# microsoft/OmniParser

Measured on AMD Instinct MI355X. Metric: screenshots/sec end-to-end (detect+caption) @1920x1080, higher is better.
Workload: dtype f32 (split-f16x3 MFMA)

## Files before the change

omniparser_amd/csrc/capi.hip:

```cpp
#include "omni_internal.h"

#include <math.h>
#include <stdarg.h>
#include <stdlib.h>
#include <string.h>
#include <vector>

static thread_local char g_err[512] = "";

void omni_set_error(const char* fmt, ...) {
  va_list ap;
  va_start(ap, fmt);
  vsnprintf(g_err, sizeof(g_err), fmt, ap);
  va_end(ap);
}

extern "C" const char* omni_last_error(void) { return g_err; }
extern "C" int omni_abi_version(void) { return OMNI_ABI_VERSION; }

static omni_ovf_reader_t g_ovf_readers[8];
static int g_ovf_n = 0;
void omni_register_overflow_reader(omni_ovf_reader_t fn) {
  if (g_ovf_n < 8) g_ovf_readers[g_ovf_n++] = fn;
}
extern "C" int omni_overflow_count(int reset, unsigned long long* count) {
  OMNI_REQUIRE(count != nullptr, "omni_overflow_count: null result pointer");
  unsigned long long total = 0;
  for (int k = 0; k < g_ovf_n; ++k) {
    unsigned int v = 0;
    if (g_ovf_readers[k](&v, reset)) {
      omni_set_error("omni_overflow_count: reading the device counter failed");
      return OMNI_E_HIP;
    }
    total += v;
  }
  *count = total;
  return OMNI_OK;
}

extern "C" int omni_device_count(void) {
  int n = 0;
  hipError_t e = hipGetDeviceCount(&n);
  if (e != hipSuccess) {
    omni_set_error("hipGetDeviceCount: %s", hipGetErrorString(e));
    return OMNI_E_NODEV;
  }
  return n;
}

static int dispatch(const omni_op_t* op, hipStream_t s) {
  switch (op->kind) {
    case OMNI_OP_CONV: return op->i[20] == 2 ? omni_launch_gemm_dma(op, s) : omni_launch_conv(op, s);
    case OMNI_OP_SPLIT_CONVERT: return omni_launch_split_convert(op, s);
    case OMNI_OP_MLP_FUSED: return omni_launch_mlp_fused(op, s);
    case OMNI_OP_GLUE: return omni_launch_glue(op, s);
    case OMNI_OP_OVERLAY: return omni_launch_overlay(op, s);
    case OMNI_OP_PNG_PACK: return omni_launch_png_pack(op, s);
    case OMNI_OP_PNG_DEFLATE: return omni_launch_png_deflate(op, s);
    case OMNI_OP_AVGPOOL2: return omni_launch_avgpool2(op, s);
    case OMNI_OP_MAXPOOL: return omni_launch_maxpool(op, s);
    case OMNI_OP_RESIZE_NEAREST: return omni_launch_resize_nearest(op, s);
    case OMNI_OP_LETTERBOX: return omni_launch_letterbox(op, s);
    case OMNI_OP_DETECT_DECODE: return omni_launch_detect_decode(op, s);
    case OMNI_OP_NMS: return omni_launch_nms(op, s);
    case OMNI_OP_DWCONV3: return omni_launch_dwconv3(op, s);
    case OMNI_OP_LAYERNORM: return omni_launch_layernorm(op, s);
    case OMNI_OP_DWCONV3_LN: return omni_launch_dwconv3_ln(op, s);
    case OMNI_OP_ATTN_ROWS: case OMNI_OP_CHAN_ATTN: case OMNI_OP_ATTN_DECODE: return omni_launch_attention(op, s);
    case OMNI_OP_PROJ_PREP: case OMNI_OP_ASSEMBLE: case OMNI_OP_EMBED_STEP: case OMNI_OP_GREEDY_STEP:
    case OMNI_OP_BEAM_STEP: case OMNI_OP_GREEDY_CTRL_STEP: case OMNI_OP_CROP_RESIZE: return omni_launch_misc(op, s);
    case OMNI_OP_GREEDY_VOCAB_STEP: return omni_launch_vocab_step(op, s);
    case OMNI_OP_VISUAL_MATCH: return omni_launch_visual_match(op, s);
    case OMNI_OP_REGION_OCR: return omni_launch_region_ocr(op, s);
    default:
      omni_set_error("unknown op kind %d", op->kind);
      return OMNI_E_ARG;
  }
}

static bool check_ptrs_enabled() {
  const char* e = getenv("OMNI_CHECK_PTRS");
  if (e && e[0] == '0') return false;
  static const int ndev = [] { int n = 0; const bool ok = hipGetDeviceCount(&n) == hipSuccess; if (!ok) (void)hipGetLastError(); return ok ? n : 0; }();
  return ndev > 0;
}

static void op_extents(const omni_op_t* op, long long ext[8]) {
  for (int k = 0; k < 8; ++k) ext[k] = 1;
  const long long esz = op->dtype == OMNI_F32 ? 4 : 2;
  const int* i = op->i;
  auto span = [&](long long rows, long long ld, long long coff, long long c) { return rows > 0 ? ((rows - 1) * ld + coff + c) * esz : 1; };
  switch (op->kind) {
    case OMNI_OP_CONV: {
      const long long B = i[0], H = i[1], W = i[2], Cin = i[3], Cout = i[12], M = B * i[10] * i[11], K = (long long)i[6] * i[7] * Cin;
      ext[0] = span(B * H * W, i[4], i[5], i[25] ? i[4] : Cin);
      ext[1] = Cout * K * (i[20] ? 4 : esz);
      ext[2] = Cout * 4;
      ext[3] = span(M, i[16], i[17], Cout);
      ext[4] = span(M, i[13], i[14], Cout);
      ext[5] = i[19] > 0 ? (long long)i[19] * 1024 : 1;
      if (i[24] > 0) ext[6] = (long long)i[24] * 4;
      if (i[20] == 2 && i[26] > 0) {
        const long long nimg = (M + i[26] - 1) / i[26];
        ext[1] += (nimg - 1) * (long long)i[27];
        ext[6] = nimg * 4;
      }
      if (i[20] == 2 && i[28] == 1) {
        ext[7] = (M / 256) * (Cout / 64) * 4096;
        ext[4] = 1;
      }
      break;
    }
    case OMNI_OP_CHAN_ATTN: {
      const long long B = i[0], N = i[1], C = i[3], G = i[4], ct = i[10] > 0 ? i[10] : (i[5] > 0 ? i[5] : 1);
      ext[0] = B * N * 3 * C * esz; ext[4] = B * N * C * esz; ext[5] = B * G * ((N + ct - 1) / ct) * 1024 * 4;
      if (i[8] == 1) { ext[1] = C * C * 4; ext[2] = ext[3] = B * C * C * 4; ext[6] = B * 4; ext[7] = B * (C / 64) * G * 4; }
      break;
    }
    case OMNI_OP_BEAM_STEP: {
      const long long rows = (long long)i[0] * i[6], T = i[3];
      ext[0] = rows > 0 ? ((rows - 1) * i[2] + i[1]) * esz : 1;
      ext[1] = (long long)i[1] * 4;
      ext[2] = ext[4] = ext[5] = rows * T * 4;
      ext[3] = rows * 4;
      ext[7] = (long long)i[0] * (3LL * i[6] + 2) * 4;
      break;
    }
    case OMNI_OP_GREEDY_STEP:
      if (op->p[5] || op->p[7]) {
        const long long rows = i[0], T = i[3];
        ext[0] = rows > 0 ? ((rows - 1) * i[2] + i[1]) * esz : 1;
        ext[1] = (long long)i[1] * 4;
        ext[2] = ext[4] = ext[7] = rows * T * 4;
        ext[5] = rows * 4;
        ext[6] = 4;
      }
      break;
    case OMNI_OP_GREEDY_CTRL_STEP: {
      const long long rows = i[0], T = i[3];
      ext[0] = rows > 0 ? ((rows - 1) * i[2] + i[1]) * esz : 1;
      ext[1] = (long long)i[1] * 4;
      ext[2] = ext[4] = rows * T * 4;
      ext[3] = rows * 4;
      ext[6] = 4;
      ext[7] = i[12];
      break;
    }
    case OMNI_OP_GREEDY_VOCAB_STEP: {
      const long long rows = i[0], T = i[3];
      ext[0] = rows > 0 ? ((rows - 1) * i[2] + i[1]) * esz : 1;
      ext[1] = (long long)i[1] * 4;
      ext[2] = ext[4] = rows * T * 4;
      ext[3] = ext[5] = rows * 4;
      ext[6] = 4;
      ext[7] = i[12];
      break;
    }
    case OMNI_OP_VISUAL_MATCH: {
      const long long D = i[3];
      if (i[0] == 0) {
        ext[0] = i[1] > 0 ? (((long long)i[1] - 1) * i[2] + D) * esz : 1; ext[4] = (long long)i[1] * D * 4; ext[5] = (long long)i[1] * 4;
      } else if (const long long part = omni_visual_match_part_bytes(op)) {
        ext[5] = part;
        if (i[0] == 1) { ext[0] = (long long)i[1] * D * 4; ext[1] = (long long)i[2] * D * 4; }
        else { ext[4] = ext[6] = (long long)i[1] * i[4] * 4; }
      }
      break;
    }
    case OMNI_OP_REGION_OCR:
      if (i[0] == 0) {
        if (i[1] > 0 && i[2] > 0 && i[3] > 0 && i[4] > 0 && i[13] > 0) {
          ext[0] = (long long)i[2] * i[3] * 3; ext[1] = (long long)i[1] * 8; ext[4] = (long long)i[1] * i[4] * i[4] * i[13] * esz; ext[7] = 1024;
        }
      } else if (i[0] == 1) {
        omni_region_ocr_extents(op, ext);
      }
      break;
    case OMNI_OP_MLP_FUSED: {
      const long long rows = (long long)i[0] * i[1], C = i[3], hid = i[12];
      ext[0] = span(rows, i[4], i[5], C); ext[1] = hid * C * 4; ext[2] = hid * 4; ext[3] = span(rows, i[16], i[17], C);
      ext[4] = span(rows, i[13], i[14], C); ext[5] = hid * C * 4; ext[6] = C * 4;
      break;
    }
    case OMNI_OP_SPLIT_CONVERT: {
      const long long rows = (long long)i[0] * i[1];
      ext[0] = span(rows, i[4], i[5], i[3]); ext[4] = span(rows, i[13], i[14], i[3]);
      break;
    }
    case OMNI_OP_AVGPOOL2: case OMNI_OP_MAXPOOL: case OMNI_OP_RESIZE_NEAREST: {
      const long long B = i[0], Ho = op->kind == OMNI_OP_AVGPOOL2 ? i[1] - 1 : i[10], Wo = op->kind == OMNI_OP_AVGPOOL2 ? i[2] - 1 : i[11];
      ext[0] = span(B * i[1] * i[2], i[4], i[5], i[3]); ext[4] = span(B * Ho * Wo, i[13], i[14], i[3]);
      if (op->kind == OMNI_OP_RESIZE_NEAREST && i[17] > 1) {
        static const int pidx[4] = {1, 2, 3, 5};
        static const int base[4][4] = {{19, 20, 21, 22}, {23, 24, 25, 26}, {27, 28, 29, 30}, {7, 12, 15, 16}};
        for (int k = 0; k + 1 < i[17] && k < 4; ++k)
          ext[pidx[k]] = span(B * i[base[k][0]] * i[base[k][1]], i[base[k][2]], i[base[k][3]], i[3]);
      }
      break;
    }
    case OMNI_OP_NMS: {
      const long long cap = i[0], md = i[1], fr = i[4] > 0 ? i[4] : 1;
      ext[0] = fr * cap * 32; ext[1] = fr * 4; ext[2] = fr * (cap + 1) * 32; ext[3] = cap * ((cap + 63) / 64) * 8;
      ext[4] = fr * md * 16; ext[5] = fr * md * 4; ext[6] = fr * md * 4; ext[7] = fr * 4;
      break;
    }
    case OMNI_OP_DETECT_DECODE: {
      for (int l = 0; l < 3; ++l) {
        const long long hw = (long long)(i[1] / (8 << l)) * (i[2] / (8 << l));
        ext[l] = span(hw, i[3 + l], i[13 + l], i[0]);
        ext[3 + l] = span(hw, i[6 + l], i[16 + l], i[12] ? 4 : 64);
      }
      ext[6] = (long long)i[9] * 32; ext[7] = 4;
      break;
    }
    case OMNI_OP_LAYERNORM: {
      const long long rows = (long long)i[0] * i[1], C = i[3];
      ext[0] = rows * C * esz; ext[1] = (long long)(i[5] > 0 ? i[5] : 1) * C * esz; ext[2] = C * 4; ext[3] = C * 4;
      ext[4] = rows * C * esz; ext[5] = rows * C * esz;
      break;
    }
    case OMNI_OP_DWCONV3: case OMNI_OP_DWCONV3_LN: {
      const long long n = (long long)i[0] * i[1] * i[2] * i[3] * esz, C = i[3];
      ext[0] = n; ext[1] = 9 * C * esz; ext[2] = C * 4; ext[4] = n;
      if (op->kind == OMNI_OP_DWCONV3_LN) { ext[3] = n; ext[5] = C * 4; ext[6] = C * 4; }
      break;
    }
    case OMNI_OP_ASSEMBLE: {
      const long long B = i[0], n_img = i[1], n_txt = i[2], C = i[3];
      ext[0] = B * n_img * C * esz; ext[1] = n_txt * C * esz; ext[2] = B * n_txt * 4; ext[3] = (long long)i[4] * C * esz;
      ext[4] = B * (n_img + n_txt) * C * esz;
      break;
    }
    case OMNI_OP_ATTN_ROWS:
      ext[7] = (long long)i[11] * 4;
      break;
    case OMNI_OP_ATTN_DECODE:
      ext[7] = i[7] > 0 ? (long long)((i[10] + (i[12] > 1 ? i[12] : 1) - 1) / (i[12] > 1 ? i[12] : 1)) * 4 : (long long)i[10] * i[8] * 4;
      break;
    case OMNI_OP_OVERLAY:
      if (op->p[3] || op->p[4] || i[3]) {
        const long long B = i[3] > 0 ? i[3] : 1;
        ext[0] = B * i[0] * i[1] * 3; ext[1] = (long long)i[2] * 32; ext[3] = B * 8; ext[4] = (B + 1) * 4;
      }
      break;
    case OMNI_OP_PNG_DEFLATE:
      if (i[5] == 2 && i[6] > 0 && i[0] > 0 && i[1] > 0) {
        const long long B = i[6], U = (long long)i[0] * (3LL * i[1] + 1), units = (U + 32767) / 32768;
        ext[0] = B * i[0] * i[1] * 3; ext[1] = B * i[2]; ext[2] = B * U; ext[3] = B * units * 33792; ext[4] = B * i[3] * 4;
        ext[5] = B * i[4] * 4; ext[6] = B * 4 * (((long long)i[2] + 2) / 3); ext[7] = B * units * 32768 * 4;
      }
      break;
    default: break;
  }
  for (int k = 0; k < 8; ++k) if (ext[k] < 1) ext[k] = 1;
}

static int check_op_ptrs(const omni_op_t* op, int index) {
  long long ext[8];
  op_extents(op, ext);
  for (int k = 0; k < 8; ++k) {
    const void* ptr = op->p[k];
    if (!ptr) continue;
    hipDeviceptr_t base = nullptr;
    size_t size = 0;
    hipError_t e = hipMemGetAddressRange(&base, &size, (hipDeviceptr_t)ptr);
    if (e != hipSuccess || !base) {
      (void)hipGetLastError();
      omni_set_error("op %d (kind %d): p[%d] = %p is not inside any device allocation (%s)", index, op->kind, k, ptr,
                     e != hipSuccess ? hipGetErrorString(e) : "no base");
      return OMNI_E_ARG;
    }
    const long long off = (const char*)ptr - (const char*)base;
    if (off < 0 || off + ext[k] > (long long)size) {
      omni_set_error("op %d (kind %d): p[%d] = %p + %lld bytes runs past its allocation [%p, +%zu)", index, op->kind, k, ptr, ext[k],
                     (void*)base, size);
      return OMNI_E_ARG;
    }
  }
  return OMNI_OK;
}

static int check_ctrl_block(const omni_op_t* op, int index) {
  if (op->kind != OMNI_OP_GREEDY_CTRL_STEP) return OMNI_OK;
  const long long bytes = op->i[12], nw = ((long long)op->i[1] + 31) >> 5, fixed = OMNI_GEN_CTRL_HEADER_BYTES + 8 * nw;
  if (!op->p[7] || op->i[1] <= 0 || bytes < fixed) {
    omni_set_error("op %d (greedy_ctrl_step): a control block of %lld bytes (i12) at p7 = %p cannot hold the header and two bitmaps over a "
                   "vocabulary of %d (%lld bytes)", index, bytes, op->p[7], op->i[1], fixed);
    return OMNI_E_ARG;
  }
  omni_gen_ctrl_t h;
  hipError_t e = hipMemcpy(&h, op->p[7], sizeof h, hipMemcpyDeviceToHost);
  if (e != hipSuccess) {
    (void)hipGetLastError();
    omni_set_error("op %d (greedy_ctrl_step): the header of the control block p7 = %p cannot be read (%s)", index, op->p[7], hipGetErrorString(e));
    return OMNI_E_ARG;
  }
  if (h.n_bad < 0 || h.n_bad > OMNI_GEN_CTRL_MAX_BAD || (h.n_bad > 0 && (h.bad_stride < 3 || h.bad_stride > OMNI_GEN_CTRL_MAX_BAD_LEN + 1))) {
    omni_set_error("op %d (greedy_ctrl_step): the control block claims %d bad-word sequences of stride %d (at most %d of 2..%d tokens)", index,
                   h.n_bad, h.bad_stride, OMNI_GEN_CTRL_MAX_BAD, OMNI_GEN_CTRL_MAX_BAD_LEN);
    return OMNI_E_ARG;
  }
  const long long need = fixed + 4LL * h.n_bad * h.bad_stride;
  if (bytes < need) {
    omni_set_error("op %d (greedy_ctrl_step): the control block's header claims %d bad-word sequences of stride %d = %lld bytes, i12 says %lld",
                   index, h.n_bad, h.bad_stride, need, bytes);
    return OMNI_E_ARG;
  }
  return OMNI_OK;
}

static int check_trie_block(const omni_op_t* op, int index) {
  if (op->kind != OMNI_OP_GREEDY_VOCAB_STEP) return OMNI_OK;
  const long long bytes = op->i[12];
  if (!op->p[7] || bytes < OMNI_VOCAB_HEADER_BYTES + 4) {
    omni_set_error("op %d (greedy_vocab_step): a trie block of %lld bytes (i12) at p7 = %p cannot hold the header and one node (%d bytes)",
                   index, bytes, op->p[7], OMNI_VOCAB_HEADER_BYTES + 4);
    return OMNI_E_ARG;
  }
  omni_vocab_trie_t h;
  hipError_t e = hipMemcpy(&h, op->p[7], sizeof h, hipMemcpyDeviceToHost);
  if (e != hipSuccess) {
    (void)hipGetLastError();
    omni_set_error("op %d (greedy_vocab_step): the header of the trie block p7 = %p cannot be read (%s)", index, op->p[7], hipGetErrorString(e));
    return OMNI_E_ARG;
  }
  if (h.n_nodes < 1 || h.n_nodes > OMNI_VOCAB_MAX_NODES || h.n_edges < 0 || h.n_edges >= h.n_nodes) {
    omni_set_error("op %d (greedy_vocab_step): the trie block claims %d nodes and %d edges (1..%d nodes, fewer edges than nodes)", index,
                   h.n_nodes, h.n_edges, OMNI_VOCAB_MAX_NODES);
    return OMNI_E_ARG;
  }
  const long long need = OMNI_VOCAB_HEADER_BYTES + 4LL * (h.n_nodes + 1 + 2LL * h.n_edges);
  if (bytes < need) {
    omni_set_error("op %d (greedy_vocab_step): the trie block's header claims %d nodes and %d edges = %lld bytes, i12 says %lld",
                   index, h.n_nodes, h.n_edges, need, bytes);
    return OMNI_E_ARG;
  }
  return OMNI_OK;
}

// ... 184 lines not shown
```

omniparser_amd/csrc/caption_ops.hip:

```cpp
#include "omni_internal.h"
#include <stdlib.h>

#pragma clang fp contract(off)

OMNI_RANGE_GUARD_TU()

namespace {

template <typename T> __device__ __forceinline__ float ldf(const T* p) { return ElemTraits<T>::to_f32(*p); }
template <typename T> __device__ __forceinline__ void stf(T* p, float v) { *p = ElemTraits<T>::from_f32(v); }

__device__ __forceinline__ float wave_sum(float v) {
#pragma unroll
  for (int o = 32; o > 0; o >>= 1) v += __shfl_xor(v, o);
  return v;
}
__device__ __forceinline__ float wave_max(float v) {
#pragma unroll
  for (int o = 32; o > 0; o >>= 1) v = fmaxf(v, __shfl_xor(v, o));
  return v;
}

struct DwArgs { const void* x; const void* w; const float* bias; void* y; int B, H, W, C; long long total; };

// ... 1335 lines not shown
}

__global__ __launch_bounds__(256) void chan_scores_mfma_kernel(ChanArgs a) {
  __shared__ float red[4][1024];
  const int chunk = blockIdx.x, g = blockIdx.y, b = blockIdx.z;
  const int lane = threadIdx.x & 63, wave = threadIdx.x >> 6;
  const int n0c = chunk * a.chunk_tokens;
  const int n1 = n0c + a.chunk_tokens < a.N ? n0c + a.chunk_tokens : a.N;
  const int per = a.chunk_tokens / 4;
  const int nw0 = n0c + wave * per, nw1 = min(nw0 + per, n1);
  const float* __restrict__ base = (const float*)a.qkv + (long long)b * a.N * 3 * a.C + g * 32 + (lane & 31);
  const long long ld = 3ll * a.C;
  f32x16 acc;
#pragma unroll
  for (int e = 0; e < 16; ++e) acc[e] = 0.0f;
  const int tsel = lane >> 5;
  int n = nw0;
  for (; n + 32 <= nw1; n += 32) {
    const float* r = base + (long long)(n + tsel) * ld;
    float qv[16], kv[16];
#pragma unroll
    for (int u = 0; u < 16; ++u) { qv[u] = r[2 * u * ld]; kv[u] = r[2 * u * ld + a.C]; }
#pragma unroll
    for (int u = 0; u < 16; ++u) acc = __builtin_amdgcn_mfma_f32_32x32x2f32(qv[u], kv[u], acc, 0, 0, 0);
  }
  for (; n < nw1; n += 2) {
    const int tok = n + tsel;
    const bool ok = tok < nw1;
    const float* r = base + (long long)(ok ? tok : nw0) * ld;
    const float qv = ok ? r[0] : 0.0f, kv = ok ? r[a.C] : 0.0f;
    acc = __builtin_amdgcn_mfma_f32_32x32x2f32(qv, kv, acc, 0, 0, 0);
  }
#pragma unroll
  for (int e = 0; e < 16; ++e) red[wave][((e & 3) + 8 * (e >> 2) + 4 * (lane >> 5)) * 32 + (lane & 31)] = acc[e];
  __syncthreads();
  float* out = a.ws + (((long long)b * a.G + g) * a.chunks + chunk) * 1024;
  for (int e = threadIdx.x; e < 1024; e += 256) out[e] = ((red[0][e] + red[1][e]) + red[2][e]) + red[3][e];
}

__global__ __launch_bounds__(256) void chan_softmax_kernel(ChanArgs a) {
  __shared__ float sa[32][33];
  const int g = blockIdx.x, b = blockIdx.y;
  float* p0 = a.ws + ((long long)b * a.G + g) * a.chunks * 1024;
  const int i = threadIdx.x >> 3, j0 = (threadIdx.x & 7) * 4;
  {
    const float* p = p0 + i * 32 + j0;
    float s[4] = {0.f, 0.f, 0.f, 0.f};
    int c = 0;
    for (; c + 8 <= a.chunks; c += 8) {
      f32x4 v[8];
#pragma unroll
      for (int u = 0; u < 8; ++u) v[u] = *reinterpret_cast<const f32x4*>(p + (long long)(c + u) * 1024);
#pragma unroll
      for (int u = 0; u < 8; ++u)
#pragma unroll
        for (int e = 0; e < 4; ++e) s[e] += v[u][e];
    }
    for (; c < a.chunks; ++c) {
      const f32x4 v = *reinterpret_cast<const f32x4*>(p + (long long)c * 1024);
#pragma unroll
      for (int e = 0; e < 4; ++e) s[e] += v[e];
    }
#pragma unroll
    for (int e = 0; e < 4; ++e) sa[i][j0 + e] = s[e] * a.scale;
  }
  __syncthreads();
  if (threadIdx.x < 32) {
    const int r = threadIdx.x;
    float mx = -INFINITY;
    for (int j = 0; j < 32; ++j) mx = fmaxf(mx, sa[r][j]);
    float sum = 0.f;
    for (int j = 0; j < 32; ++j) { float e = expf(sa[r][j] - mx); sa[r][j] = e; sum += e; }
    const float inv = 1.0f / sum;
    for (int j = 0; j < 32; ++j) sa[r][j] *= inv;
  }
  __syncthreads();
#pragma unroll
  for (int e = 0; e < 4; ++e) p0[i * 32 + j0 + e] = sa[i][j0 + e];
}

__global__ __launch_bounds__(256, 2) void chan_apply_mfma_split_kernel(ChanArgs a) {
  const int g = blockIdx.y, b = blockIdx.z;
  const int lane = threadIdx.x & 63, wave = threadIdx.x >> 6;
  const int col = lane & 31, kg = lane >> 5;
  const float inv2048 = 1.0f / 2048.0f;
  const int n00 = blockIdx.x * 256 + wave * 64;
  if (n00 >= a.N) return;
  const float* V = (const float*)a.qkv + (long long)b * a.N * 3 * a.C + 2 * a.C + g * 32 + kg * 8;
  f32x4 vraw[2][4];
#pragma unroll
  for (int t = 0; t < 2; ++t) {
    const int nl = min(n00 + t * 32 + col, a.N - 1);
    const float* vp = V + (long long)nl * 3 * a.C;
#pragma unroll
    for (int ks = 0; ks < 2; ++ks) {
      vraw[t][2 * ks] = *reinterpret_cast<const f32x4*>(vp + 16 * ks);
      vraw[t][2 * ks + 1] = *reinterpret_cast<const f32x4*>(vp + 16 * ks + 4);
    }
  }
  const float* A = a.ws + ((long long)b * a.G + g) * a.chunks * 1024 + col * 32 + kg * 8;
  h16x8 Ah[2], Al[2];
#pragma unroll
  for (int ks = 0; ks < 2; ++ks) {
    uint2 h0, l0, h1, l1;
    split4m(*reinterpret_cast<const f32x4*>(A + 16 * ks), h0, l0);
    split4m(*reinterpret_cast<const f32x4*>(A + 16 * ks + 4), h1, l1);
    Ah[ks] = __builtin_bit_cast(h16x8, u32x4{h0.x, h0.y, h1.x, h1.y});
    Al[ks] = __builtin_bit_cast(h16x8, u32x4{l0.x, l0.y, l1.x, l1.y});
  }
  float* const O = (float*)a.o + (long long)b * a.N * a.C + g * 32 + 4 * kg;
  unsigned char* const S = (unsigned char*)a.o + (long long)b * a.N * a.C * 4;
#pragma unroll
  for (int t = 0; t < 2; ++t) {
    const int n = n00 + t * 32 + col;
    if (n00 + t * 32 >= a.N) break;
    f32x16 accM, accC;
#pragma unroll
    for (int e = 0; e < 16; ++e) { accM[e] = 0.f; accC[e] = 0.f; }
#pragma unroll
    for (int ks = 0; ks < 2; ++ks) {
      uint2 h0, l0, h1, l1;
      split4m(vraw[t][2 * ks], h0, l0);
      split4m(vraw[t][2 * ks + 1], h1, l1);
      const h16x8 vh = __builtin_bit_cast(h16x8, u32x4{h0.x, h0.y, h1.x, h1.y});
      const h16x8 vl = __builtin_bit_cast(h16x8, u32x4{l0.x, l0.y, l1.x, l1.y});
      accM = __builtin_amdgcn_mfma_f32_32x32x16_f16(Ah[ks], vh, accM, 0, 0, 0);
      accC = __builtin_amdgcn_mfma_f32_32x32x16_f16(Ah[ks], vl, accC, 0, 0, 0);
      accC = __builtin_amdgcn_mfma_f32_32x32x16_f16(Al[ks], vh, accC, 0, 0, 0);
    }
    if (n < a.N) {
#pragma unroll
      for (int q = 0; q < 4; ++q) {
        const f32x4 o = f32x4{accC[4 * q], accC[4 * q + 1], accC[4 * q + 2], accC[4 * q + 3]} * inv2048 +
                        f32x4{accM[4 * q], accM[4 * q + 1], accM[4 * q + 2], accM[4 * q + 3]};
        if (a.osplit) {
          const float v[4] = {o[0], o[1], o[2], o[3]};
          uint2 hi, lo;
          omni_split4(v, hi, lo);
          unsigned char* p = S + (long long)n * a.C * 4 + omni_split_off(g * 32 + 8 * q + 4 * kg);
          *reinterpret_cast<uint2*>(p) = hi;
          *reinterpret_cast<uint2*>(p + 32) = lo;
        } else {
          *reinterpret_cast<f32x4*>(O + (long long)n * a.C + 8 * q) = o;
        }
      }
    }
  }
}


struct FoldArgs {
  const float* ws; const float* wp; float* wf; float* bmax; unsigned char* wb; float* osc;
  int C, G, chunks, nblk;
};

__global__ __launch_bounds__(256) void chan_fold_kernel(FoldArgs a) {
  __shared__ float sA[32][32];
  __shared__ float sW[64][33];
  __shared__ float smax[4];
  const int ob = blockIdx.x, g = blockIdx.y, b = blockIdx.z, tid = threadIdx.x;
  const float* A = a.ws + ((long long)b * a.G + g) * a.chunks * 1024;
  for (int e = tid; e < 1024; e += 256) sA[e >> 5][e & 31] = A[e];
  for (int e = tid; e < 64 * 32; e += 256) sW[e >> 5][e & 31] = a.wp[(long long)(ob * 64 + (e >> 5)) * a.C + g * 32 + (e & 31)];
  __syncthreads();
  const int r = tid >> 2, j0 = (tid & 3) * 8;
  float acc[8];
#pragma unroll
  for (int e = 0; e < 8; ++e) acc[e] = 0.0f;
#pragma unroll 8
  for (int i = 0; i < 32; ++i) {
    const float w = sW[r][i];
#pragma unroll
    for (int e = 0; e < 8; ++e) acc[e] = fmaf(w, sA[i][j0 + e], acc[e]);
  }
  float* out = a.wf + ((long long)b * a.C + ob * 64 + r) * a.C + g * 32 + j0;
  *reinterpret_cast<f32x4*>(out) = f32x4{acc[0], acc[1], acc[2], acc[3]};
  *reinterpret_cast<f32x4*>(out + 4) = f32x4{acc[4], acc[5], acc[6], acc[7]};
  float m = 0.0f;
#pragma unroll
  for (int e = 0; e < 8; ++e) m = fmaxf(m, fabsf(acc[e]));
#pragma unroll
  for (int o = 32; o >= 1; o >>= 1) m = fmaxf(m, __shfl_xor(m, o));
  if ((tid & 63) == 0) smax[tid >> 6] = m;
  __syncthreads();
  if (tid == 0) a.bmax[(long long)b * a.nblk + ob * a.G + g] = fmaxf(fmaxf(smax[0], smax[1]), fmaxf(smax[2], smax[3]));
}

__global__ __launch_bounds__(256) void chan_fold_pack_kernel(FoldArgs a) {
  __shared__ float red[256];
  const int b = blockIdx.y, tid = threadIdx.x;
  float m = 0.0f;
  for (int e = tid; e < a.nblk; e += 256) m = fmaxf(m, a.bmax[(long long)b * a.nblk + e]);
  red[tid] = m;
  __syncthreads();
  for (int o = 128; o >= 1; o >>= 1) {
    if (tid < o) red[tid] = fmaxf(red[tid], red[tid + o]);
    __syncthreads();
  }
  const float amax = red[0];
  int k = 0;
  if (amax > 0.0f) {
    k = 12 - ((int)((__builtin_bit_cast(unsigned, amax) >> 23) & 0xffu) - 127);
    k = max(-24, min(24, k));
  }
  const float up = __builtin_bit_cast(float, (unsigned)(127 + k) << 23);
  if (blockIdx.x == 0 && tid == 0) a.osc[b] = __builtin_bit_cast(float, (unsigned)(127 - k) << 23);
  const int gpr = a.C / 16;
  const int idx = blockIdx.x * 256 + tid;
  if (idx >= a.C * gpr) return;
  const float* src = a.wf + (long long)b * a.C * a.C + (long long)idx * 16;
  half_t h[32];
#pragma unroll
  for (int q = 0; q < 4; ++q) {
    const f32x4 v = *reinterpret_cast<const f32x4*>(src + 4 * q) * up;
#pragma unroll
    for (int e = 0; e < 4; ++e) {
      const half_t hi = (half_t)v[e];
      h[4 * q + e] = hi;
      h[16 + 4 * q + e] = (half_t)(v[e] - (float)hi);
    }
  }
  unsigned char* dst = a.wb + ((long long)b * a.C * a.C + (long long)idx * 16) * 4;
#pragma unroll
  for (int q = 0; q < 4; ++q) {
    f16x8 o;
#pragma unroll
    for (int e = 0; e < 8; ++e) o[e] = h[8 * q + e];
    *reinterpret_cast<f16x8*>(dst + 16 * q) = o;
  }
}


struct PrepArgs { const void* x; const float* pos; const float* temporal; void* y; int B, N, C; };

template <typename T>
__global__ __launch_bounds__(256) void proj_prep_kernel(PrepArgs a) {
  int c = blockIdx.x * 256 + threadIdx.x, b = blockIdx.y;
  if (c >= a.C) return;
  const T* x = (const T*)a.x + (long long)b * a.N * a.C + c;
  T* y = (T*)a.y + (long long)b * (a.N + 1) * a.C + c;
  float s = 0.f;
  for (int n = 0; n < a.N; ++n) {
    float v = (ldf(x + (long long)n * a.C) + a.pos[(long long)n * a.C + c]) + a.temporal[c];
    s += v;
    stf(y + (long long)(n + 1) * a.C, v);
  }
  stf(y, s / (float)a.N);
}

struct AsmArgs {
  const void* img; const void* txt; void* y; int B, n_img, n_txt, C;
  const void* table; const int* ids; int vocab; float scale;
};

template <typename T>
__global__ __launch_bounds__(256) void assemble_kernel(AsmArgs a) {
  long long total = (long long)a.B * (a.n_img + a.n_txt) * a.C;
  long long idx = (long long)blockIdx.x * 256 + threadIdx.x;
  if (idx >= total) return;
  int c = (int)(idx % a.C);
  long long r = idx / a.C;
  int t = (int)(r % (a.n_img + a.n_txt));
  long long b = r / (a.n_img + a.n_txt);
  if (a.ids && t >= a.n_img) {
    const int tok = min(max(a.ids[b * a.n_txt + (t - a.n_img)], 0), a.vocab - 1);
    float v = ldf((const T*)a.table + (long long)tok * a.C + c);
    if (a.scale != 1.0f) v *= a.scale;
    stf((T*)a.y + idx, v);
    return;
  }
  const T* src = t < a.n_img ? (const T*)a.img + (b * a.n_img + t) * a.C + c : (const T*)a.txt + (long long)(t - a.n_img) * a.C + c;
  ((T*)a.y)[idx] = *src;
}

struct EmbArgs { const void* table; const void* pos; const int* ids; const int* step; void* y; int B, C, T, pos_offset; float scale; };

template <typename T>
__global__ __launch_bounds__(256) void embed_step_kernel(EmbArgs a) {
  int c = blockIdx.x * 256 + threadIdx.x, b = blockIdx.y;
  if (c >= a.C) return;
  int st = *a.step;
  int tok = a.ids[b * a.T + st];
  float v = ldf((const T*)a.table + (long long)tok * a.C + c);
  if (a.scale != 1.0f) v *= a.scale;
  v += ldf((const T*)a.pos + (long long)(st + a.pos_offset) * a.C + c);
  stf((T*)a.y + (long long)b * a.C + c, v);
}

constexpr int ATTN_SELF_SPLIT_MIN_CAP = 64;
struct DecArgs {
  const void* q; const void* knew; const void* vnew; void* kc; void* vc; void* o; const int* step;
  int ldq, qoff, ldn, koff, voff, ldo;
  int heads, nk_fixed, cap, C, ldc;
  float scale;
  const int* nkeys;
};

__device__ __forceinline__ int decode_cross_keys(const DecArgs& a, int bkv) {
  return a.nkeys ? min(max(a.nkeys[bkv], 1), a.nk_fixed) : a.nk_fixed;
}

template <typename T, bool BEAM>
__device__ __forceinline__ void attn_decode_body(DecArgs a, const int* table, int kv_div) {
  OMNI_DYN_LDS(float, sp);
  const int h = blockIdx.x, b = blockIdx.y, lane = threadIdx.x;
  const int C = a.ldc;
  int nk;
  const int bkv = BEAM && a.nk_fixed > 0 ? b / kv_div : b;
  T* Kc = (T*)a.kc + (long long)bkv * a.cap * C + h * 64;
  T* Vc = (T*)a.vc + (long long)bkv * a.cap * C + h * 64;
  const int* trow = BEAM && a.nk_fixed <= 0 ? table + (long long)b * a.cap : nullptr;
  auto krow = [&](int k) -> long long {
    if constexpr (BEAM) {
      if (trow) return ((long long)(trow[k] - b) * a.cap + k) * C;
    }
    return (long long)k * C;
  };
  if (a.nk_fixed > 0) {
    nk = decode_cross_keys(a, bkv);
  } else {
    int st = *a.step;
    nk = st + 1;
    Kc[(long long)st * C + lane] = ((const T*)a.knew)[(long long)b * a.ldn + a.koff + h * 64 + lane];
    Vc[(long long)st * C + lane] = ((const T*)a.vnew)[(long long)b * a.ldn + a.voff + h * 64 + lane];
    __syncthreads();
  }
  float qd = ldf((const T*)a.q + (long long)b * a.ldq + a.qoff + h * 64 + lane);
  __shared__ float sq[64];
  sq[lane] = qd;
  __syncthreads();
  float mx = -INFINITY;
  for (int k = lane; k < nk; k += 64) {
    const T* kr = Kc + krow(k);
    float s = 0.f;
#pragma unroll 16
    for (int d = 0; d < 64; ++d) s += sq[d] * ldf(kr + d);
    s *= a.scale;
    sp[k] = s;
    mx = fmaxf(mx, s);
  }
  mx = wave_max(mx);
  float sum = 0.f;
  for (int k = lane; k < nk; k += 64) { float e = expf(sp[k] - mx); sp[k] = e; sum += e; }
  sum = wave_sum(sum);
  __syncthreads();
  float acc = 0.f;
  for (int k = 0; k < nk; ++k) acc += sp[k] * ldf(Vc + krow(k) + lane);
  stf((T*)a.o + (long long)b * a.ldo + h * 64 + lane, acc / sum);
}

template <typename T>
__global__ __launch_bounds__(64) void attn_decode_kernel(DecArgs a) { attn_decode_body<T, false>(a, nullptr, 1); }

template <typename T>
__global__ __launch_bounds__(64) void attn_decode_beam_kernel(DecArgs a, const int* table, int kv_div) {
  attn_decode_body<T, true>(a, table, kv_div);
}

template <bool BEAM>
// ... 800 lines not shown
      int kk = k[y]; s0 += s[0] * kk; s1 += s[1] * kk; s2 += s[2] * kk;
    }
    p[0] = clip8b(s0); p[1] = clip8b(s1); p[2] = clip8b(s2);
  }
  T* out = (T*)a.y + ((long long)crop * a.R * a.R + idx) * a.ldo;
#pragma unroll
  for (int c = 0; c < 3; ++c) {
    float v = a.lut[p[c]];
    stf(out + c, (v - a.mean[c]) / a.stdv[c]);
  }
  for (int c = 3; c < a.ldo; ++c) stf(out + c, 0.0f);
}

template <typename F32, typename F16>
int by_dtype(int dtype, const char* name, F32 f32, F16 f16) {
  if (dtype == OMNI_F32) f32();
  else if (dtype == OMNI_F16) f16();
  else { omni_set_error("%s: bad dtype %d", name, dtype); return OMNI_E_ARG; }
  return OMNI_OK;
}

template <typename L>
int by_dtype_scores(int dtype, bool scores, const char* name, L launch) {
  return scores ? by_dtype(dtype, name, [&] { launch(float{}, std::true_type{}); }, [&] { launch(half_t{}, std::true_type{}); })
                : by_dtype(dtype, name, [&] { launch(float{}, std::false_type{}); }, [&] { launch(half_t{}, std::false_type{}); });
}

}

int omni_launch_dwconv3(const omni_op_t* op, hipStream_t s) {
  DwArgs a{};
  a.x = op->p[0]; a.w = op->p[1]; a.bias = (const float*)op->p[2]; a.y = op->p[4];
  a.B = op->i[0]; a.H = op->i[1]; a.W = op->i[2]; a.C = op->i[3];
  OMNI_REQUIRE(a.x && a.w && a.bias && a.y && a.B > 0 && a.H > 0 && a.W > 0 && a.C > 0, "dwconv3: bad arguments");
  OMNI_REQUIRE(a.C % (op->dtype == OMNI_F32 ? 4 : 8) == 0, "dwconv3: C must be a multiple of the 16-byte vector width");
  a.total = (long long)a.B * a.H * a.W * a.C;
  const int V = op->dtype == OMNI_F32 ? 4 : 8;
  const DwStripGrid g = dwconv3_strip_grid(a, V);
  int rc;
  if (g.ok) {
    rc = by_dtype(op->dtype, "dwconv3",
        [&] { hipLaunchKernelGGL(dwconv3_strip_kernel<float>, dim3(g.gx, g.gy, g.gz), dim3(256), 0, s, a, g.cv_log2); },
        [&] { hipLaunchKernelGGL(dwconv3_strip_kernel<half_t>, dim3(g.gx, g.gy, g.gz), dim3(256), 0, s, a, g.cv_log2); });
  } else {
    long long blocks = (a.total / V + 255) / 256; if (blocks > 65536) blocks = 65536;
    rc = by_dtype(op->dtype, "dwconv3",
        [&] { hipLaunchKernelGGL(dwconv3_kernel<float>, dim3((unsigned)blocks), dim3(256), 0, s, a); },
        [&] { hipLaunchKernelGGL(dwconv3_kernel<half_t>, dim3((unsigned)blocks), dim3(256), 0, s, a); });
  }
  if (rc) return rc;
  OMNI_HIP_CHECK(hipGetLastError());
  return OMNI_OK;
}

int omni_launch_dwconv3_ln(const omni_op_t* op, hipStream_t s) {
  DwLnArgs a{};
  a.x = op->p[0]; a.w = op->p[1]; a.bias = (const float*)op->p[2]; a.h = op->p[3]; a.y1 = op->p[4];
  a.g = (const float*)op->p[5]; a.b = (const float*)op->p[6];
  a.B = op->i[0]; a.H = op->i[1]; a.W = op->i[2]; a.C = op->i[3]; a.eps = op->f[0]; a.osplit = op->i[6];
  const int V = op->dtype == OMNI_F32 ? 4 : 8;
  OMNI_REQUIRE(a.x && a.w && a.bias && a.h && a.y1 && a.g && a.b, "dwconv3_ln: null pointer");
  OMNI_REQUIRE(!a.osplit || (op->dtype == OMNI_F32 && a.C % 16 == 0), "dwconv3_ln: split output needs an f32 plan and C %% 16 == 0");
  OMNI_REQUIRE(a.B > 0 && a.H > 0 && a.W > 0 && a.C > 0 && a.C <= 1024 && a.C % V == 0, "dwconv3_ln: bad shape (C <= 1024, C %% %d == 0)", V);
  a.pixels = (long long)a.B * a.H * a.W;
  if (op->dtype == OMNI_F32 && (a.C == 128 || a.C == 256 || a.C == 512) && (long long)a.B * a.H * a.W < (1ll << 31)) {
    if (a.C == 128) launch_dwln_strip<1, 32>(a, s);
    else if (a.C == 256) launch_dwln_strip<1, 64>(a, s);
    else launch_dwln_strip<2, 64>(a, s);
    OMNI_HIP_CHECK(hipGetLastError());
    return OMNI_OK;
  }
  unsigned blocks = (unsigned)((a.pixels + 3) / 4);
  int rc = by_dtype(op->dtype, "dwconv3_ln",
      [&] { hipLaunchKernelGGL(dwconv3_ln_kernel<float>, dim3(blocks), dim3(256), 0, s, a); },
      [&] { hipLaunchKernelGGL(dwconv3_ln_kernel<half_t>, dim3(blocks), dim3(256), 0, s, a); });
  if (rc) return rc;
  OMNI_HIP_CHECK(hipGetLastError());
  return OMNI_OK;
}

int omni_launch_layernorm(const omni_op_t* op, hipStream_t s) {
  LnArgs a{};
  a.x = op->p[0]; a.add = op->p[1]; a.g = (const float*)op->p[2]; a.b = (const float*)op->p[3]; a.y = op->p[4];
  a.rows = ((long long)op->i[0]) * (op->i[1] > 0 ? op->i[1] : 1); a.C = op->i[3]; a.period = op->i[5] > 0 ? op->i[5] : 1;
  a.eps = op->f[0];
  a.omode = op->i[6]; a.y2 = op->p[5];
  OMNI_REQUIRE(a.x && a.g && a.b && a.y && a.rows > 0 && a.C > 0 && a.C <= 1024, "layernorm: bad arguments (C <= 1024)");
  OMNI_REQUIRE(a.omode >= 0 && a.omode <= 2 && (a.omode != 2 || a.y2), "layernorm: bad output mode %d", a.omode);
  OMNI_REQUIRE(a.omode == 0 || (op->dtype == OMNI_F32 && a.C % 16 == 0), "layernorm: split output needs an f32 plan and C %% 16 == 0");
  if (op->dtype == OMNI_F32 && launch_layernorm_v4(a, s)) {
    OMNI_HIP_CHECK(hipGetLastError());
    return OMNI_OK;
  }
  unsigned blocks = (unsigned)((a.rows + 3) / 4);
  int rc = by_dtype(op->dtype, "layernorm",
      [&] { launch_layernorm_typed<float>(a, blocks, s); },
      [&] { launch_layernorm_typed<half_t>(a, blocks, s); });
  if (rc) return rc;
  OMNI_HIP_CHECK(hipGetLastError());
  return OMNI_OK;
}

static int launch_attn_rows(const omni_op_t* op, hipStream_t s) {
  AttnArgs a{};
  a.q = op->p[0]; a.k = op->p[1]; a.v = op->p[2]; a.o = op->p[4];
  a.kbias = (const float*)op->p[5]; a.vbias = (const float*)op->p[6];
  a.ldq = op->i[0]; a.ldk = op->i[1]; a.ldv = op->i[2]; a.ldo = op->i[3];
  a.qoff = op->i[4]; a.koff = op->i[5]; a.voff = op->i[6]; a.ooff = op->i[7];
  a.heads = op->i[8]; a.nq = op->i[9]; a.nk = op->i[10]; a.groups = op->i[11];
  a.mode = op->i[12]; a.H = op->i[13]; a.W = op->i[14];
  int D = op->i[15];
  a.scale = op->f[0];
  a.osplit = op->i[16];
  a.nkeys = (const int*)op->p[7];
  OMNI_REQUIRE(a.q && a.k && a.v && a.o && a.heads > 0 && a.nq > 0 && a.nk > 0 && a.groups > 0, "attn_rows: bad arguments");
  OMNI_REQUIRE(!a.nkeys || a.mode == 0, "attn_rows: the per-group key count (p7) is for mode 0");
  OMNI_REQUIRE(!a.osplit || (op->dtype == OMNI_F32 && a.ldo % 16 == 0 && a.ooff % 16 == 0), "attn_rows: split output needs an f32 plan, 16-channel aligned");
  OMNI_REQUIRE(D == 32 || D == 64, "attn_rows: head_dim %d unsupported", D);
  if (a.mode == 1) {
    OMNI_REQUIRE(a.nq == 144 && a.nk == 144 && a.H > 0 && a.W > 0, "attn_rows: window mode needs 12x12 windows");
    a.wy = (a.H + 11) / 12; a.wx = (a.W + 11) / 12;
    OMNI_REQUIRE(a.groups % (a.wy * a.wx) == 0, "attn_rows: groups must be B * windows");
  } else { a.wy = a.wx = 0; }
  int rc;
  const bool aligned4 = a.ldq % 4 == 0 && a.ldk % 4 == 0 && a.ldv % 4 == 0 && a.ldo % 4 == 0 &&
                        a.qoff % 4 == 0 && a.koff % 4 == 0 && a.voff % 4 == 0 && a.ooff % 4 == 0;
  OMNI_REQUIRE(!a.osplit || (a.mode == 1 && D == 32) || (a.mode == 0 && D == 64), "attn_rows: split output exists on the MFMA kernels only");
  if (a.mode == 1 && D == 32) {
    dim3 grid(1, a.heads, a.groups);
    OMNI_REQUIRE(op->dtype != OMNI_F32 || aligned4, "attn_rows: the f32 window kernel reads 16-byte rows (pitches and channel offsets %% 4 == 0)");
    rc = by_dtype(op->dtype, "attn_rows",
      [&] { hipLaunchKernelGGL(window_attn_mfma_f32_kernel, grid, dim3(192), 0, s, a); },
      [&] { hipLaunchKernelGGL((window_attn_mfma_kernel<half_t>), grid, dim3(192), 0, s, a); });
  } else if (a.mode == 0 && D == 64) {
    dim3 grid((a.nq + 127) / 128, a.heads, a.groups);
    OMNI_REQUIRE(op->dtype != OMNI_F32 || aligned4, "attn_rows: the f32 MHA kernel reads 16-byte rows (pitches and channel offsets %% 4 == 0)");
    rc = by_dtype(op->dtype, "attn_rows",
      [&] { hipLaunchKernelGGL(mha_mfma_f32_kernel, grid, dim3(256), 0, s, a); },
      [&] { hipLaunchKernelGGL((mha_mfma_kernel<half_t>), grid, dim3(256), 0, s, a); });
  } else {
    dim3 grid((a.nq + 127) / 128, a.heads, a.groups);
    if (D == 32) rc = by_dtype(op->dtype, "attn_rows",
      [&] { hipLaunchKernelGGL((attn_rows_kernel<float, 32, 128>), grid, dim3(128), 0, s, a); },
      [&] { hipLaunchKernelGGL((attn_rows_kernel<half_t, 32, 128>), grid, dim3(128), 0, s, a); });
    else rc = by_dtype(op->dtype, "attn_rows",
      [&] { hipLaunchKernelGGL((attn_rows_kernel<float, 64, 128>), grid, dim3(128), 0, s, a); },
      [&] { hipLaunchKernelGGL((attn_rows_kernel<half_t, 64, 128>), grid, dim3(128), 0, s, a); });
  }
  if (rc) return rc;
  OMNI_HIP_CHECK(hipGetLastError());
  return OMNI_OK;
}

static int launch_chan_attn(const omni_op_t* op, hipStream_t s) {
  ChanArgs a{};
  a.qkv = op->p[0]; a.o = op->p[4]; a.ws = (float*)op->p[5];
  a.B = op->i[0]; a.N = op->i[1]; a.C = op->i[3]; a.G = op->i[4]; a.chunk_tokens = op->i[5]; a.osplit = op->i[6];
  const bool fold = op->i[8] == 1;
  OMNI_REQUIRE(a.qkv && (a.o || fold) && a.ws && a.B > 0 && a.N > 0 && a.C == a.G * 32 && a.chunk_tokens > 0, "chan_attn: bad arguments");
  OMNI_REQUIRE(op->i[8] == 0 || fold, "chan_attn: unknown mode %d", op->i[8]);
  OMNI_REQUIRE(!fold || (op->dtype == OMNI_F32 && a.chunk_tokens % 8 == 0 && a.C % 64 == 0 && op->p[1] && op->p[2] && op->p[3] && op->p[6] && op->p[7]),
               "chan_attn: fold mode needs an f32 plan, C %% 64 == 0, chunk_tokens %% 8 == 0 and p1 / p2 / p3 / p6 / p7");
  OMNI_REQUIRE(!a.osplit || op->dtype == OMNI_F32, "chan_attn: split output needs an f32 plan");
  const bool have_scores = op->i[9] == 1;
  if (op->i[10] != 0) {
    OMNI_REQUIRE(op->i[10] > 0 && op->i[10] % 8 == 0 && a.chunk_tokens % op->i[10] == 0 && op->dtype == OMNI_F32 && a.C % 4 == 0,
                 "chan_attn: i10 = %d (tokens per partial) needs an f32 plan, i10 %% 8 == 0 and i5 %% i10 == 0", op->i[10]);
    a.chunk_tokens = op->i[10];
  }
  OMNI_REQUIRE(op->i[9] == 0 || (have_scores && op->dtype == OMNI_F32 && a.chunk_tokens % 8 == 0 && a.C % 4 == 0),
               "chan_attn: i9 = %d (partials already in the workspace) needs an f32 plan and chunk_tokens %% 8 == 0", op->i[9]);
  a.chunks = (a.N + a.chunk_tokens - 1) / a.chunk_tokens;
  a.scale = 1.0f / sqrtf((float)a.N);
  if (op->f[0] != 0.0f) a.scale = op->f[0];
  dim3 g1(a.chunks, a.G, a.B), g2((a.N + 255) / 256, a.G, a.B);
  if (op->dtype == OMNI_F32 && a.chunk_tokens % 8 == 0 && a.C % 4 == 0) {
    if (!have_scores) hipLaunchKernelGGL(chan_scores_mfma_kernel, g1, dim3(256), 0, s, a);
    hipLaunchKernelGGL(chan_softmax_kernel, dim3(a.G, a.B), dim3(256), 0, s, a);
    if (fold) {
      FoldArgs f{};
      f.ws = a.ws; f.wp = (const float*)op->p[1]; f.wf = (float*)op->p[2]; f.wb = (unsigned char*)op->p[3]; f.osc = (float*)op->p[6];
      f.bmax = (float*)op->p[7];
      f.C = a.C; f.G = a.G; f.chunks = a.chunks; f.nblk = (a.C / 64) * a.G;
      hipLaunchKernelGGL(chan_fold_kernel, dim3(a.C / 64, a.G, a.B), dim3(256), 0, s, f);
      hipLaunchKernelGGL(chan_fold_pack_kernel, dim3((a.C * (a.C / 16) + 255) / 256, a.B), dim3(256), 0, s, f);
      OMNI_HIP_CHECK(hipGetLastError());
      return OMNI_OK;
    }
    hipLaunchKernelGGL(chan_apply_mfma_split_kernel, g2, dim3(256), 0, s, a);
    OMNI_HIP_CHECK(hipGetLastError());
    return OMNI_OK;
  }
  int rc = by_dtype(op->dtype, "chan_attn",
      [&] { hipLaunchKernelGGL(chan_scores_kernel<float>, g1, dim3(256), 0, s, a);
            hipLaunchKernelGGL(chan_apply_kernel<float>, g2, dim3(256), 0, s, a); },
      [&] { hipLaunchKernelGGL(chan_scores_kernel<half_t>, g1, dim3(256), 0, s, a);
            hipLaunchKernelGGL(chan_apply_kernel<half_t>, g2, dim3(256), 0, s, a); });
  if (rc) return rc;
  OMNI_HIP_CHECK(hipGetLastError());
  return OMNI_OK;
}

static int launch_attn_decode(const omni_op_t* op, hipStream_t s) {
  DecArgs a{};
  a.q = op->p[0]; a.knew = op->p[1]; a.vnew = op->p[2]; a.kc = op->p[3]; a.o = op->p[4]; a.vc = op->p[5];
  a.step = (const int*)op->p[6];
  a.ldq = op->i[0]; a.qoff = op->i[1]; a.ldn = op->i[2]; a.koff = op->i[3]; a.voff = op->i[4]; a.ldo = op->i[5];
  a.heads = op->i[6]; a.nk_fixed = op->i[7]; a.cap = op->i[8]; a.C = op->i[9]; a.ldc = op->i[11] > 0 ? op->i[11] : a.C;
  int B = op->i[10];
  a.scale = op->f[0];
  OMNI_REQUIRE(a.q && a.kc && a.vc && a.o && B > 0 && a.heads > 0 && a.C == a.heads * 64, "attn_decode: bad arguments (head_dim 64)");
  OMNI_REQUIRE(a.nk_fixed > 0 || (a.knew && a.vnew && a.step), "attn_decode: self-attention needs new k/v and the step counter");
  const int* table = a.nk_fixed > 0 ? nullptr : (const int*)op->p[7];
  a.nkeys = a.nk_fixed > 0 ? (const int*)op->p[7] : nullptr;
  const int kv_div = op->i[12] > 1 ? op->i[12] : 1;
  const bool beam = table != nullptr || kv_div > 1;
  OMNI_REQUIRE(a.nk_fixed <= 0 || a.nk_fixed <= a.cap, "attn_decode: nk_fixed beyond the cache rows");
  OMNI_REQUIRE(kv_div == 1 || a.nk_fixed > 0, "attn_decode: rows per K/V row > 1 is for cross-attention");
  int nk_max = a.nk_fixed > 0 ? a.nk_fixed : a.cap;
  if (a.nk_fixed > 0 && op->dtype == OMNI_F32 && a.ldc % 4 == 0 && a.ldq % 4 == 0 && a.qoff % 4 == 0) {
    const size_t lds = (size_t)(((a.nk_fixed + 3) & ~3) + 8 + 256) * 4;
    if (beam)
      hipLaunchKernelGGL(attn_decode_cross_kernel<true>, dim3(a.heads, B), dim3(256), lds, s, a, kv_div);
    else
      hipLaunchKernelGGL(attn_decode_cross_kernel<false>, dim3(a.heads, B), dim3(256), lds, s, a, 1);
    OMNI_HIP_CHECK(hipGetLastError());
    return OMNI_OK;
  }
  if (a.nk_fixed <= 0 && !beam && op->dtype == OMNI_F32 && a.cap > ATTN_SELF_SPLIT_MIN_CAP && a.ldc % 4 == 0 && a.ldq % 4 == 0 &&
      a.qoff % 4 == 0 && a.ldn % 4 == 0 && a.koff % 4 == 0 && a.voff % 4 == 0) {
    const size_t lds = (size_t)(((a.cap + 3) & ~3) + 8 + 256) * 4;
    OMNI_REQUIRE(lds <= 48 * 1024, "attn_decode: %d cache rows exceed the score LDS of the split-key kernel", a.cap);
    hipLaunchKernelGGL(attn_decode_self_kernel, dim3(a.heads, B), dim3(256), lds, s, a);
    OMNI_HIP_CHECK(hipGetLastError());
    return OMNI_OK;
  }
  dim3 grid(a.heads, B);
  size_t sh = (size_t)nk_max * 4;
  int rc = beam ? by_dtype(op->dtype, "attn_decode",
      [&] { hipLaunchKernelGGL(attn_decode_beam_kernel<float>, grid, dim3(64), sh, s, a, table, kv_div); },
      [&] { hipLaunchKernelGGL(attn_decode_beam_kernel<half_t>, grid, dim3(64), sh, s, a, table, kv_div); })
                : by_dtype(op->dtype, "attn_decode",
      [&] { hipLaunchKernelGGL(attn_decode_kernel<float>, grid, dim3(64), sh, s, a); },
      [&] { hipLaunchKernelGGL(attn_decode_kernel<half_t>, grid, dim3(64), sh, s, a); });
  if (rc) return rc;
  OMNI_HIP_CHECK(hipGetLastError());
  return OMNI_OK;
}

static int finish_step(const omni_op_t* op, hipStream_t s) {
  if (op->i[11]) hipLaunchKernelGGL(step_inc_kernel, dim3(1), dim3(64), 0, s, (int*)op->p[6]);
  OMNI_HIP_CHECK(hipGetLastError());
  return OMNI_OK;
}

static GreedyArgs greedy_args_from_op(const omni_op_t* op) {
  GreedyArgs a{};
  a.logits = op->p[0]; a.bias = (const float*)op->p[1]; a.ids = (int*)op->p[2]; a.finished = (int*)op->p[3];
  a.step = (const int*)op->p[6];
  a.B = op->i[0]; a.V = op->i[1]; a.ldl = op->i[2]; a.T = op->i[3]; a.max_new = op->i[4]; a.ngram = op->i[5];
  a.bos = op->i[6]; a.eos = op->i[7]; a.pad = op->i[8]; a.forced_bos = op->i[9]; a.forced_eos = op->i[10];
  a.logp = (float*)op->p[4];
  return a;
}

static int launch_score(const omni_op_t* op, hipStream_t s) {
  ScoreArgs a{};
  a.logits = op->p[0]; a.bias = (const float*)op->p[1]; a.ids = (const int*)op->p[2]; a.logp = (float*)op->p[4];
  a.tlen = (const int*)op->p[5]; a.step = (const int*)op->p[6]; a.top1 = (int*)op->p[7];
  a.B = op->i[0]; a.V = op->i[1]; a.ldl = op->i[2]; a.T = op->i[3];
  OMNI_REQUIRE(a.tlen, "greedy_step: p7 (top1) belongs to the target-score form, which p5 (target lengths) selects");
  OMNI_REQUIRE(a.logp, "greedy_step: the target-score form (p5) writes p4, which is NULL");
  OMNI_REQUIRE(a.logits && a.ids && a.step && a.B > 0 && a.V > 0 && a.ldl >= a.V && a.T >= 2, "greedy_step (target scores): bad arguments");
  OMNI_REQUIRE((unsigned long long)a.logits % (op->dtype == OMNI_F32 ? 4 : 2) == 0, "greedy_step (target scores): logits not aligned to their element");
  int rc = by_dtype(op->dtype, "greedy_step",
      [&] { hipLaunchKernelGGL(score_step_kernel<float>, dim3(a.B), dim3(256), 0, s, a); },
      [&] { hipLaunchKernelGGL(score_step_kernel<half_t>, dim3(a.B), dim3(256), 0, s, a); });
  return rc ? rc : finish_step(op, s);
}

static int launch_greedy(const omni_op_t* op, hipStream_t s) {
  if (op->p[5] || op->p[7]) return launch_score(op, s);
  GreedyArgs a = greedy_args_from_op(op);
  OMNI_REQUIRE(a.logits && a.ids && a.finished && a.step && a.B > 0 && a.V > 0 && a.T >= a.max_new + 1, "greedy_step: bad arguments");
  if (a.ngram > 0 && a.max_new - a.ngram + 1 > 32) {
    const size_t lds = ((size_t)((a.V + 31) >> 5) + (size_t)a.T) * 4;
    OMNI_REQUIRE(lds <= 48 * 1024, "greedy_step: a vocabulary of %d and %d positions exceed the ban LDS", a.V, a.T);
    int rl = by_dtype_scores(op->dtype, a.logp != nullptr, "greedy_step", [&](auto t, auto sc) {
      hipLaunchKernelGGL((greedy_step_long_kernel<decltype(t), decltype(sc)::value>), dim3(a.B), dim3(256), lds, s, a); });
    return rl ? rl : finish_step(op, s);
  }
  int rc = by_dtype_scores(op->dtype, a.logp != nullptr, "greedy_step", [&](auto t, auto sc) {
    hipLaunchKernelGGL((greedy_step_kernel<decltype(t), decltype(sc)::value>), dim3(a.B), dim3(256), 0, s, a); });
  return rc ? rc : finish_step(op, s);
}

static int launch_greedy_ctrl(const omni_op_t* op, hipStream_t s) {
  GreedyCtrlArgs c{};
  c.g = greedy_args_from_op(op);
  const GreedyArgs& a = c.g;
  c.ctrl = (const unsigned*)op->p[7]; c.ctrl_bytes = op->i[12];
  OMNI_REQUIRE(a.logits && a.ids && a.finished && a.step && a.B > 0 && a.V > 0 && a.ldl >= a.V && a.T >= a.max_new + 1 && a.max_new >= 1,
               "greedy_ctrl_step: bad arguments");
  OMNI_REQUIRE(!op->p[5], "greedy_ctrl_step: p5 (target lengths) belongs to OMNI_OP_GREEDY_STEP; the controls have no target-score form");
  OMNI_REQUIRE(c.ctrl && (unsigned long long)c.ctrl % 4 == 0, "greedy_ctrl_step: p7 (control block) is NULL or not 4-byte aligned");
  const long long nw = ((long long)a.V + 31) >> 5;
  OMNI_REQUIRE(c.ctrl_bytes >= OMNI_GEN_CTRL_HEADER_BYTES + 8 * nw, "greedy_ctrl_step: a control block of %d bytes (i12) cannot hold the header and "
               "two bitmaps over a vocabulary of %d (%lld bytes)", c.ctrl_bytes, a.V, OMNI_GEN_CTRL_HEADER_BYTES + 8 * nw);
  const size_t lds = ((size_t)2 * nw + (size_t)a.T + OMNI_GEN_CTRL_MAX_BAD) * 4;
  OMNI_REQUIRE(lds <= 48 * 1024, "greedy_ctrl_step: a vocabulary of %d and %d positions exceed the bitmap LDS", a.V, a.T);
  int rc = by_dtype_scores(op->dtype, a.logp != nullptr, "greedy_ctrl_step", [&](auto t, auto sc) {
    hipLaunchKernelGGL((greedy_ctrl_step_kernel<decltype(t), decltype(sc)::value>), dim3(a.B), dim3(256), lds, s, c); });
  return rc ? rc : finish_step(op, s);
}

static int launch_beam(const omni_op_t* op, hipStream_t s) {
  BeamArgs a{};
  a.logits = op->p[0]; a.bias = (const float*)op->p[1]; a.ids = (int*)op->p[2]; a.run_score = (float*)op->p[3];
  a.table = (int*)op->p[4]; a.fin_ids = (int*)op->p[5]; a.step = (const int*)op->p[6]; a.state = (int*)op->p[7];
  a.B = op->i[0]; a.V = op->i[1]; a.ldl = op->i[2]; a.T = op->i[3]; a.max_new = op->i[4]; a.ngram = op->i[5]; a.k = op->i[6];
  a.eos = op->i[7]; a.pad = op->i[8]; a.forced_bos = op->i[9]; a.forced_eos = op->i[10]; a.early_stopping = op->i[12];
  a.length_penalty = op->f[0];
  OMNI_REQUIRE(a.logits && a.ids && a.run_score && a.table && a.fin_ids && a.step && a.state && a.B > 0 && a.V > 0 && a.ldl >= a.V,
               "beam_step: bad arguments");
  OMNI_REQUIRE(a.k >= 2 && a.k <= BEAM_MAX, "beam_step: 2 <= beams <= %d (got %d)", BEAM_MAX, a.k);
  OMNI_REQUIRE(a.T >= a.max_new + 1 && a.max_new >= 1 && a.early_stopping >= 0 && a.early_stopping <= 2, "beam_step: bad arguments");
  const size_t lds = (size_t)3 * a.k * a.T * 4;
  OMNI_REQUIRE(lds <= 48 * 1024, "beam_step: %d beams x %d positions exceed the staging LDS", a.k, a.T);
  int rc = by_dtype(op->dtype, "beam_step",
      [&] { hipLaunchKernelGGL(beam_step_kernel<float>, dim3(a.B), dim3(256), lds, s, a); },
      [&] { hipLaunchKernelGGL(beam_step_kernel<half_t>, dim3(a.B), dim3(256), lds, s, a); });
  return rc ? rc : finish_step(op, s);
}

static int launch_crop_resize(const omni_op_t* op, hipStream_t s) {
  CropArgs a{};
  a.img = (const unsigned char*)op->p[0]; a.boxes = (const int*)op->p[1]; a.c64 = (unsigned char*)op->p[2];
// ... 71 lines not shown
```

omniparser_amd/csrc/gemm_dma.hip:

```cpp
#include "omni_internal.h"
#include "gemm_common.h"
#include <string.h>
#include <type_traits>

OMNI_RANGE_GUARD_TU()

namespace {

typedef __attribute__((address_space(3))) void lds_void;

struct GemmArgs {
  const unsigned char* x; const unsigned char* w; const float* bias; const float* res; unsigned char* y;
  int M, N, K, nk;
  int ldi, in_coff, ldo, out_coff, ldr, res_coff;
  int mtiles, ntiles, xcd_order, xcd_n;
  float oscale;
  int img_tiles; unsigned w_img_stride; const float* img_oscale;
};

constexpr int GEMM_EPI_SCORES = 3;

#if defined(__AMDGCN__)
struct RowBuf {
  __amdgpu_buffer_rsrc_t r;
  __device__ __forceinline__ RowBuf(const void* base, unsigned bytes) : r(__builtin_amdgcn_make_buffer_rsrc((void*)base, 0, (int)bytes, 0x00020000)) {}
  __device__ __forceinline__ void store16(unsigned off, f32x4 v) const { __builtin_amdgcn_raw_buffer_store_b128(__builtin_bit_cast(u32x4, v), r, (int)off, 0, 0); }
  __device__ __forceinline__ f32x4 load16(unsigned off) const { return __builtin_bit_cast(f32x4, __builtin_amdgcn_raw_buffer_load_b128(r, (int)off, 0, 0)); }
};
#else
struct RowBuf {
  unsigned char* base; unsigned bytes;
  RowBuf(const void* b, unsigned n) : base((unsigned char*)b), bytes(n) {}
  void store16(unsigned off, f32x4 v) const { if (off + 16u <= bytes) *reinterpret_cast<f32x4*>(base + off) = v; }
  f32x4 load16(unsigned off) const { return off + 16u <= bytes ? *reinterpret_cast<const f32x4*>(base + off) : f32x4{0.f, 0.f, 0.f, 0.f}; }
};
#endif

template <int BM, int BN, int WM, int WN, int TM, int TN, int LDS_BYTES, int ACT, bool OSPLIT, bool RES>
__device__ __forceinline__ void gemm_epilogue(f32x16 (&acc)[TM][TN], const GemmArgs& a, unsigned char* lds, int m0, int n0, int wave, int lane, float osc) {
  constexpr int NW = WM * WN;
  const int wm = wave / WN, wn = wave % WN;
  const int hsel = lane >> 5;
  static_assert(TN % 2 == 0, "epilogue stages 64 channels (256 bytes per row) of a wave at a time");
  constexpr int EP = 272;
  static_assert(NW * 32 * EP <= LDS_BYTES, "epilogue staging must fit the LDS ring");
  __syncthreads();
  unsigned char* stg = lds + wave * (32 * EP);
  float amax = 0.0f;
  const int rrow = lane >> 4, chunk = lane & 15;
  const int trows = min(a.M - m0, BM), wc0 = n0 + wn * (BN / WN);
  const RowBuf ybuf(a.y + ((long long)m0 * a.ldo + a.out_coff + wc0) * 4, (unsigned)(trows - 1) * (unsigned)(a.ldo * 4) + (BN / WN) * 4);
  const RowBuf rbuf(RES ? reinterpret_cast<const unsigned char*>(a.res) + ((long long)m0 * a.ldr + a.res_coff + wc0) * 4 : a.y,
                    RES ? (unsigned)(trows - 1) * (unsigned)(a.ldr * 4) + (BN / WN) * 4 : 0u);
  const unsigned yoff = (unsigned)(wm * (BM / WM) + rrow) * (unsigned)(a.ldo * 4) + chunk * 16;
  const unsigned roff = (unsigned)(wm * (BM / WM) + rrow) * (unsigned)(a.ldr * 4) + chunk * 16;
  static_assert(!(RES && OSPLIT), "residual + format-B output is not a layer of this model");
#pragma unroll
  for (int jh = 0; jh < TN / 2; ++jh) {
    const int nw0 = n0 + wn * (BN / WN) + jh * 64;
    f32x4 bq[2][4];
#pragma unroll
    for (int j = 0; j < 2; ++j)
#pragma unroll
      for (int q = 0; q < 4; ++q)
        bq[j][q] = a.bias ? *reinterpret_cast<const f32x4*>(a.bias + nw0 + 4 * hsel + j * 32 + q * 8) : f32x4{0.f, 0.f, 0.f, 0.f};
    f32x4 rres[8];
    auto load_res = [&](int i) {
#pragma unroll
      for (int it = 0; it < 8; ++it) rres[it] = rbuf.load16(roff + (unsigned)(i * 32 + it * 4) * (unsigned)(a.ldr * 4) + jh * 256);
    };
    if constexpr (RES) load_res(0);
#pragma unroll
    for (int i = 0; i < TM; ++i) {
      unsigned char* wr = stg + (lane & 31) * EP;
#pragma unroll
      for (int j = 0; j < 2; ++j)
#pragma unroll
        for (int q = 0; q < 4; ++q) {
          const f32x16& ac = acc[i][jh * 2 + j];
          float v[4];
          if constexpr (ACT == OMNI_ACT_GELU) {
#pragma unroll
            for (int c = 0; c < 4; c += 2) {
              const f32x2 g = omni_gelu2(__builtin_elementwise_fma(f32x2{ac[q * 4 + c], ac[q * 4 + c + 1]}, (f32x2)osc, f32x2{bq[j][q][c], bq[j][q][c + 1]}));
              v[c] = g[0]; v[c + 1] = g[1];
            }
          } else {
#pragma unroll
            for (int c = 0; c < 4; c += 2) {
              f32x2 t = __builtin_elementwise_fma(f32x2{ac[q * 4 + c], ac[q * 4 + c + 1]}, (f32x2)osc, f32x2{bq[j][q][c], bq[j][q][c + 1]});
              if constexpr (ACT == OMNI_ACT_SILU) t = f32x2{t[0] / (1.0f + expf(-t[0])), t[1] / (1.0f + expf(-t[1]))};
              v[c] = t[0]; v[c + 1] = t[1];
            }
          }
          const int cl = j * 32 + q * 8 + 4 * hsel;
          if constexpr (OSPLIT) {
            uint2 hi, lo;
            omni_split4(v, hi, lo, amax);
            *reinterpret_cast<uint2*>(wr + omni_split_off(cl)) = hi;
            *reinterpret_cast<uint2*>(wr + omni_split_off(cl) + 32) = lo;
          } else {
            *reinterpret_cast<f32x4*>(wr + cl * 4) = f32x4{v[0], v[1], v[2], v[3]};
          }
        }
      OMNI_WAVE_SYNC();
      f32x4 ov[8];
#pragma unroll
      for (int it = 0; it < 8; ++it) {
        ov[it] = *reinterpret_cast<const f32x4*>(stg + (it * 4 + rrow) * EP + chunk * 16);
        if constexpr (RES) ov[it] += rres[it];
      }
      if constexpr (RES) { if (i + 1 < TM) load_res(i + 1); }
#pragma unroll
      for (int it = 0; it < 8; ++it) ybuf.store16(yoff + (unsigned)(i * 32 + it * 4) * (unsigned)(a.ldo * 4) + jh * 256, ov[it]);
      OMNI_WAVE_SYNC();
      __builtin_amdgcn_sched_barrier(0);
    }
  }
  if constexpr (OSPLIT) omni_report_range(amax);
}

template <int BM, int BN, int WM, int WN, int TM, int TN, int LDS_BYTES>
__device__ __forceinline__ void gemm_scores_epilogue(f32x16 (&acc)[TM][TN], const GemmArgs& a, unsigned char* lds, int img, int chunk, int n0, int wave,
                                                     int lane, float osc) {
  static_assert(BM == 256 && BN == 256 && WM == 2 && WN == 4 && TM == 4 && TN == 2, "scores epilogue: 256x256 tile, a wave owns 128 tokens x 64 channels");
  constexpr int NW = WM * WN, EP = 272, HAND = NW * 32 * EP;
  static_assert(HAND + WN * 2 * 4096 <= LDS_BYTES, "hand-over matrices must fit the LDS ring behind the staging slices");
  const int wm = wave / WN, wn = wave % WN;
  const int hsel = lane >> 5;
  __syncthreads();
  unsigned char* stg = lds + wave * (32 * EP);
  const int nw0 = n0 + wn * 64;
  f32x4 bq[2][4];
#pragma unroll
  for (int j = 0; j < 2; ++j)
#pragma unroll
    for (int q = 0; q < 4; ++q)
      bq[j][q] = a.bias ? *reinterpret_cast<const f32x4*>(a.bias + nw0 + 4 * hsel + j * 32 + q * 8) : f32x4{0.f, 0.f, 0.f, 0.f};
  f32x16 sc[2];
#pragma unroll
  for (int e = 0; e < 16; ++e) { sc[0][e] = 0.0f; sc[1][e] = 0.0f; }
#pragma unroll
  for (int i = 0; i < TM; ++i) {
    unsigned char* wr = stg + (lane & 31) * EP;
#pragma unroll
    for (int j = 0; j < 2; ++j)
#pragma unroll
      for (int q = 0; q < 4; ++q) {
        const f32x16& ac = acc[i][j];
        float v[4];
#pragma unroll
        for (int c = 0; c < 4; c += 2) {
          const f32x2 t = __builtin_elementwise_fma(f32x2{ac[q * 4 + c], ac[q * 4 + c + 1]}, (f32x2)osc, f32x2{bq[j][q][c], bq[j][q][c + 1]});
          v[c] = t[0]; v[c + 1] = t[1];
        }
        *reinterpret_cast<f32x4*>(wr + (j * 32 + q * 8 + 4 * hsel) * 4) = f32x4{v[0], v[1], v[2], v[3]};
      }
    OMNI_WAVE_SYNC();
    const unsigned char* rd = stg + hsel * EP + (lane & 31) * 4;
    float qv[16], kv[16];
#pragma unroll
    for (int u = 0; u < 16; ++u) {
      qv[u] = *reinterpret_cast<const float*>(rd + 2 * u * EP);
      kv[u] = *reinterpret_cast<const float*>(rd + 2 * u * EP + 128);
    }
#pragma unroll
    for (int u = 0; u < 16; ++u) sc[i >> 1] = __builtin_amdgcn_mfma_f32_32x32x2f32(qv[u], kv[u], sc[i >> 1], 0, 0, 0);
    OMNI_WAVE_SYNC();
    __builtin_amdgcn_sched_barrier(0);
  }
  float* hand = reinterpret_cast<float*>(lds + HAND) + wn * 2048;
  if (wm == 1) {
#pragma unroll
    for (int r = 0; r < 2; ++r)
#pragma unroll
      for (int e = 0; e < 16; ++e) hand[(r * 16 + e) * 64 + lane] = sc[r][e];
  }
  __syncthreads();
  if (wm == 0) {
    float* out = reinterpret_cast<float*>(a.y) + ((((long long)img * (a.N / 64) + (n0 / 64 + wn)) * a.img_tiles + chunk) * 1024 + (lane & 31));
#pragma unroll
    for (int e = 0; e < 16; ++e)
      out[((e & 3) + 8 * (e >> 2) + 4 * hsel) * 32] = ((sc[0][e] + sc[1][e]) + hand[e * 64 + lane]) + hand[(16 + e) * 64 + lane];
  }
}

template <int BM, int BN, int WM, int WN, int NSTAGE, int ACT, bool OSPLIT, bool RES, int SCHED = 0>
__global__ __launch_bounds__(WM * WN * 64, 2) void gemm_dma_kernel(GemmArgs a) {
#if defined(__HIP_DEVICE_COMPILE__)
  constexpr int NW = WM * WN;
  constexpr int TM = BM / (32 * WM), TN = BN / (32 * WN);
  constexpr int A_DMA = BM / (8 * NW), B_DMA = BN / (8 * NW);
  constexpr int DPS = A_DMA + B_DMA;
  constexpr int STAGE = (BM + BN) * 128;
  constexpr int NP = TM / 2;
  constexpr int NU = 2 * NP;
  constexpr int NM = 6 * TN;
  static_assert(TM % 2 == 0 && TN >= 1 && A_DMA >= 1 && B_DMA >= 1 && NSTAGE >= 2 && NSTAGE <= 4, "tile / wave grid mismatch");
  static_assert(BM * 128 + (TN - 1) * 4096 < 65536 && (TM - 1) * 4096 < 65536, "ds_read immediate offsets");
  __shared__ __attribute__((aligned(16))) unsigned char lds[NSTAGE * STAGE];

  const int tid = threadIdx.x, lane = tid & 63;
  const int wave = __builtin_amdgcn_readfirstlane(tid >> 6);
  const int wm = wave / WN, wn = wave % WN;
  int mt, nt;
  if (!tile_of_block(blockIdx.x, a.mtiles, a.ntiles, a.xcd_order, a.xcd_n, mt, nt)) return;
  const int m0 = __builtin_amdgcn_readfirstlane(mt) * BM, n0 = __builtin_amdgcn_readfirstlane(nt) * BN;
  const int img = a.img_tiles ? __builtin_amdgcn_readfirstlane(mt / a.img_tiles) : 0;
  const float osc = a.img_oscale ? a.img_oscale[img] : a.oscale;

  const int rsub = lane >> 3, slot = lane & 7;
  unsigned voffA[A_DMA], voffB[B_DMA];
  auto pieceA = [&](int i) { return SCHED == 2 ? wave + NW * i : wave * A_DMA + i; };
#pragma unroll
  for (int i = 0; i < A_DMA; ++i) {
    const int rl = pieceA(i) * 8 + rsub;
    const int rr = min(rl, a.M - 1 - m0);
    voffA[i] = (unsigned)rr * (unsigned)(a.ldi * 4) + (unsigned)((slot ^ ((rl >> 1) & 7)) * 16);
// ... 21 lines not shown
    for (int i = 0; i < DPS; ++i) issue_piece(kt, stage, i);
  };

  const int swz = (lane >> 1) & 7, hsel = lane >> 5;
  int offA[4], offW[4];
#pragma unroll
  for (int gp = 0; gp < 4; ++gp) {
    const int c = ((((gp >> 1) * 4 + (gp & 1) * 2 + hsel) ^ swz)) * 16;
    offA[gp] = (wm * (BM / WM) + (lane & 31)) * 128 + c;
    offW[gp] = BM * 128 + (wn * (BN / WN) + (lane & 31)) * 128 + c;
  }
  struct AF { f16x8 h[2], l[2]; };
  struct WF { f16x8 h[TN], l[TN]; };
  auto loadA = [&](const unsigned char* st, int g, int ip, AF& f) {
#pragma unroll
    for (int t = 0; t < 2; ++t) {
      f.h[t] = *reinterpret_cast<const f16x8*>(st + offA[g * 2 + 0] + (ip * 2 + t) * 4096);
      f.l[t] = *reinterpret_cast<const f16x8*>(st + offA[g * 2 + 1] + (ip * 2 + t) * 4096);
    }
  };
  auto loadW = [&](const unsigned char* st, int g, WF& f) {
#pragma unroll
    for (int j = 0; j < TN; ++j) {
      f.h[j] = *reinterpret_cast<const f16x8*>(st + offW[g * 2 + 0] + j * 4096);
      f.l[j] = *reinterpret_cast<const f16x8*>(st + offW[g * 2 + 1] + j * 4096);
    }
  };

  f32x16 acc[TM][TN];
#pragma unroll
  for (int i = 0; i < TM; ++i)
#pragma unroll
    for (int j = 0; j < TN; ++j)
#pragma unroll
      for (int e = 0; e < 16; ++e) acc[i][j][e] = 0.0f;

  auto mma = [&](const AF& af, const WF& wf, int ip) {
#pragma unroll
    for (int t = 0; t < 2; ++t)
#pragma unroll
      for (int j = 0; j < TN; ++j)
        acc[ip * 2 + t][j] = __builtin_amdgcn_mfma_f32_32x32x16_f16(wf.h[j], af.h[t], acc[ip * 2 + t][j], 0, 0, 0);
#pragma unroll
    for (int t = 0; t < 2; ++t)
#pragma unroll
      for (int j = 0; j < TN; ++j)
        acc[ip * 2 + t][j] = __builtin_amdgcn_mfma_f32_32x32x16_f16(wf.l[j], af.h[t], acc[ip * 2 + t][j], 0, 0, 0);
#pragma unroll
    for (int t = 0; t < 2; ++t)
#pragma unroll
      for (int j = 0; j < TN; ++j)
        acc[ip * 2 + t][j] = __builtin_amdgcn_mfma_f32_32x32x16_f16(wf.h[j], af.l[t], acc[ip * 2 + t][j], 0, 0, 0);
  };

  const int nk = a.nk;
#pragma unroll
  for (int s = 0; s < NSTAGE - 1; ++s)
    if (s < nk) issue(s, s);
  int stage = 0, nstage = NSTAGE - 1;
  constexpr int IU = SCHED == 1 ? (NU + 1) / 2 : NU;
  constexpr int PPU = (DPS + IU - 1) / IU;
  AF af[2];
  WF wf[2];
  auto slice = [&](int kt, auto more_tag) {
    constexpr bool MORE = decltype(more_tag)::value;
    if constexpr (NSTAGE > 2 && MORE) OMNI_WAIT_VMCNT((NSTAGE - 2) * DPS);
    else OMNI_WAIT_VMCNT(0);
    __builtin_amdgcn_s_barrier();
    const unsigned char* st = lds + stage * STAGE;
    loadW(st, 0, wf[0]);
    loadA(st, 0, 0, af[0]);
#pragma unroll
    for (int u = 0; u < NU; ++u) {
      const int g = u / NP, ip = u % NP;
      int nds = 0;
      if (u + 1 < NU) {
        const int g2 = (u + 1) / NP, ip2 = (u + 1) % NP;
        if (g2 != g) { loadW(st, g2, wf[g2 & 1]); nds += 2 * TN; }
        loadA(st, g2, ip2, af[(u + 1) & 1]);
        nds += 4;
      }
      if constexpr (MORE) {
#pragma unroll
        for (int i = u * PPU; i < (u + 1) * PPU && i < DPS; ++i) issue_piece(kt + NSTAGE - 1, nstage, i);
      }
      mma(af[u & 1], wf[g & 1], ip);
      {
        const int npc = (MORE && u < IU) ? PPU : 0;
#pragma unroll
        for (int k = 0; k < NM; ++k) {
          __builtin_amdgcn_sched_group_barrier(0x8, 1, 0);
          if (k < nds) __builtin_amdgcn_sched_group_barrier(0x100, 1, 0);
          else if (k < nds + npc) __builtin_amdgcn_sched_group_barrier(0x20, 1, 0);
        }
      }
      __builtin_amdgcn_sched_barrier(0);
    }
    stage = stage + 1 == NSTAGE ? 0 : stage + 1;
    nstage = nstage + 1 == NSTAGE ? 0 : nstage + 1;
  };
  if constexpr (SCHED == 2) {
    static_assert(BM == 256 && BN == 256 && WM == 2 && WN == 4 && NSTAGE == 2 && TM == 4 && TN == 2 && A_DMA == 4 && B_DMA == 4, "ping-pong: 256x256 tile, 8 waves");
    OMNI_WAIT_VMCNT(0);
    __builtin_amdgcn_s_barrier();
    if (wm == 1) __builtin_amdgcn_s_barrier();
    auto phase_barrier = [&]() {
      __builtin_amdgcn_sched_barrier(0);
      __builtin_amdgcn_s_barrier();
      __builtin_amdgcn_sched_barrier(0);
    };
    {
      AF afp;
      auto slice_pp = [&](int kt, auto more_tag) {
        constexpr bool MORE = decltype(more_tag)::value;
        const unsigned char* st = lds + stage * STAGE;
#pragma unroll
        for (int u = 0; u < 4; ++u) {
          const int g = u & 1, ip = u >> 1;
          if (u < 2) loadW(st, g, wf[g]);
          loadA(st, g, ip, afp);
          if constexpr (MORE) {
            if (u == 0) { issue_piece(kt + 1, nstage, 0); issue_piece(kt + 1, nstage, 2); }
            if (u == 1) { issue_piece(kt + 1, nstage, A_DMA + 0); issue_piece(kt + 1, nstage, A_DMA + 1); }
            if (u == 2) { issue_piece(kt + 1, nstage, A_DMA + 2); issue_piece(kt + 1, nstage, A_DMA + 3); }
            if (u == 3) { issue_piece(kt + 1, nstage, 1); issue_piece(kt + 1, nstage, 3); }
            if (u == 1) OMNI_WAIT_VMCNT(4);
            if (u == 3) OMNI_WAIT_VMCNT(2);
          } else {
            if (u == 1) OMNI_WAIT_VMCNT(0);
          }
          phase_barrier();
          __builtin_amdgcn_s_setprio(1);
          mma(afp, wf[g], ip);
          __builtin_amdgcn_s_setprio(0);
          phase_barrier();
        }
        stage ^= 1;
        nstage ^= 1;
      };
      int ktp = 0;
      for (; ktp + 1 < nk; ++ktp) slice_pp(ktp, std::true_type{});
      for (; ktp < nk; ++ktp) slice_pp(ktp, std::false_type{});
    }
    if (wm == 0) __builtin_amdgcn_s_barrier();
  } else {
  int kt = 0;
  for (; kt + NSTAGE - 1 < nk; ++kt) slice(kt, std::true_type{});
  for (; kt < nk; ++kt) slice(kt, std::false_type{});
  }

  if constexpr (ACT == GEMM_EPI_SCORES)
    gemm_scores_epilogue<BM, BN, WM, WN, TM, TN, NSTAGE * STAGE>(acc, a, lds, img, __builtin_amdgcn_readfirstlane(mt) - img * a.img_tiles, n0, wave, lane, osc);
  else
    gemm_epilogue<BM, BN, WM, WN, TM, TN, NSTAGE * STAGE, ACT, OSPLIT, RES>(acc, a, lds, m0, n0, wave, lane, osc);
#endif
}

__global__ __launch_bounds__(256) void split_convert_kernel(const float* __restrict__ x, unsigned char* __restrict__ y, long long rows,
                                                            int C, int ldi, int in_coff, int ldo, int out_coff) {
  const int gpr = C / 16;
  const long long idx = (long long)blockIdx.x * blockDim.x + threadIdx.x;
  if (idx >= rows * gpr) return;
  const long long r = idx / gpr;
  const int g = (int)(idx - r * gpr);
  const float* src = x + r * ldi + in_coff + g * 16;
  f32x4 v[4];
#pragma unroll
  for (int q = 0; q < 4; ++q) v[q] = *reinterpret_cast<const f32x4*>(src + q * 4);
  uint2 hi[4], lo[4];
#pragma unroll
  for (int q = 0; q < 4; ++q) {
    float t[4] = {v[q][0], v[q][1], v[q][2], v[q][3]};
    omni_split4(t, hi[q], lo[q]);
  }
  unsigned char* dst = y + (r * ldo + out_coff + g * 16) * 4;
  *reinterpret_cast<u32x4*>(dst) = u32x4{hi[0].x, hi[0].y, hi[1].x, hi[1].y};
  *reinterpret_cast<u32x4*>(dst + 16) = u32x4{hi[2].x, hi[2].y, hi[3].x, hi[3].y};
  *reinterpret_cast<u32x4*>(dst + 32) = u32x4{lo[0].x, lo[0].y, lo[1].x, lo[1].y};
  *reinterpret_cast<u32x4*>(dst + 48) = u32x4{lo[2].x, lo[2].y, lo[3].x, lo[3].y};
}

struct MlpArgs {
  const unsigned char* x; const unsigned char* w1; const unsigned char* w2; const float* b1;
  GemmArgs ep{};
  int ldi, in_coff;
  float osc1;
};

template <int C, int HID>
__global__ __launch_bounds__(256, 2) void mlp_fused_kernel(MlpArgs a) {
#if defined(__HIP_DEVICE_COMPILE__)
  static_assert(C == 128 && HID % 32 == 0, "written for the C = 128 stage: 8 K groups in registers, 4 output tiles");
  constexpr int NW = 4, KG = C / 16, OB = C / 32, NCH = HID / 32;
  constexpr int W1B = 32 * C * 4, W2B = C * 128, STAGE = W1B + W2B;
  constexpr int P1 = W1B / 1024 / NW, P2 = W2B / 1024 / NW;
  __shared__ __attribute__((aligned(16))) unsigned char lds[2 * STAGE + HID * 4];
  float* lb1 = reinterpret_cast<float*>(lds + 2 * STAGE);

  const int tid = threadIdx.x, lane = tid & 63;
  const int wave = __builtin_amdgcn_readfirstlane(tid >> 6);
  const int m0 = blockIdx.x * (NW * 32);
  const int hsel = lane >> 5, swz = (lane >> 1) & 7;

  for (int e = tid * 4; e < HID; e += 256 * 4) *reinterpret_cast<f32x4*>(lb1 + e) = *reinterpret_cast<const f32x4*>(a.b1 + e);

  const int rsub = lane >> 3, slot = lane & 7;
  unsigned voff1[P1], voff2[P2];
#pragma unroll
  for (int i = 0; i < P1; ++i) {
    const int pc = wave * P1 + i, rl = (pc & 3) * 8 + rsub, sl = pc >> 2;
    voff1[i] = (unsigned)rl * (unsigned)(C * 4) + (unsigned)(sl * 128) + (unsigned)((slot ^ ((rl >> 1) & 7)) * 16);
  }
#pragma unroll
  for (int i = 0; i < P2; ++i) {
    const int rl = (wave * P2 + i) * 8 + rsub;
    voff2[i] = (unsigned)rl * (unsigned)(HID * 4) + (unsigned)((slot ^ ((rl >> 1) & 7)) * 16);
  }
  const __amdgpu_buffer_rsrc_t rsrc1 = __builtin_amdgcn_make_buffer_rsrc((void*)a.w1, 0, 0x7fffffff, 0x00020000);
  const __amdgpu_buffer_rsrc_t rsrc2 = __builtin_amdgcn_make_buffer_rsrc((void*)a.w2, 0, 0x7fffffff, 0x00020000);
  auto issue = [&](int c, int stage) {
#pragma unroll
    for (int i = 0; i < P1; ++i)
      __builtin_amdgcn_raw_ptr_buffer_load_lds(rsrc1, (lds_void*)(lds + stage * STAGE + (wave * P1 + i) * 1024), 16, voff1[i], c * (32 * C * 4), 0, 0);
#pragma unroll
    for (int i = 0; i < P2; ++i)
      __builtin_amdgcn_raw_ptr_buffer_load_lds(rsrc2, (lds_void*)(lds + stage * STAGE + W1B + (wave * P2 + i) * 1024), 16, voff2[i], c * 128, 0, 0);
  };
  issue(0, 0);

  f16x8 xh[KG], xl[KG];
  {
    const int m = min(m0 + wave * 32 + (lane & 31), a.ep.M - 1);
    const unsigned char* xrow = a.x + ((long long)m * a.ldi + a.in_coff) * 4 + hsel * 16;
#pragma unroll
    for (int g = 0; g < KG; ++g) {
      xh[g] = *reinterpret_cast<const f16x8*>(xrow + g * 64);
      xl[g] = *reinterpret_cast<const f16x8*>(xrow + g * 64 + 32);
    }
  }
  int fo[2][2];
#pragma unroll
  for (int gg = 0; gg < 2; ++gg)
#pragma unroll
    for (int pt = 0; pt < 2; ++pt) fo[gg][pt] = (lane & 31) * 128 + (((gg * 4 + pt * 2 + hsel) ^ swz) * 16);

  f32x16 acc2[1][OB];
#pragma unroll
  for (int j = 0; j < OB; ++j)
#pragma unroll
    for (int e = 0; e < 16; ++e) acc2[0][j][e] = 0.0f;
  const float osc1 = a.osc1;
  float amax = 0.0f;
  __syncthreads();

  for (int c = 0; c < NCH; ++c) {
    const int stage = c & 1;
    OMNI_WAIT_VMCNT(0);
    __builtin_amdgcn_s_barrier();
    if (c + 1 < NCH) issue(c + 1, stage ^ 1);
    const unsigned char* st = lds + stage * STAGE;
    f32x16 a1[2];
#pragma unroll
    for (int e = 0; e < 16; ++e) { a1[0][e] = 0.0f; a1[1][e] = 0.0f; }
#pragma unroll
    for (int g = 0; g < KG; g += 2) {
      const unsigned char* sl = st + (g >> 1) * 4096;
      const f16x8 wh0 = *reinterpret_cast<const f16x8*>(sl + fo[0][0]), wl0 = *reinterpret_cast<const f16x8*>(sl + fo[0][1]);
      const f16x8 wh1 = *reinterpret_cast<const f16x8*>(sl + fo[1][0]), wl1 = *reinterpret_cast<const f16x8*>(sl + fo[1][1]);
      a1[0] = __builtin_amdgcn_mfma_f32_32x32x16_f16(wh0, xh[g], a1[0], 0, 0, 0);
      a1[1] = __builtin_amdgcn_mfma_f32_32x32x16_f16(wh1, xh[g + 1], a1[1], 0, 0, 0);
      a1[0] = __builtin_amdgcn_mfma_f32_32x32x16_f16(wl0, xh[g], a1[0], 0, 0, 0);
      a1[1] = __builtin_amdgcn_mfma_f32_32x32x16_f16(wl1, xh[g + 1], a1[1], 0, 0, 0);
      a1[0] = __builtin_amdgcn_mfma_f32_32x32x16_f16(wh0, xl[g], a1[0], 0, 0, 0);
      a1[1] = __builtin_amdgcn_mfma_f32_32x32x16_f16(wh1, xl[g + 1], a1[1], 0, 0, 0);
    }
    f16x8 gh[2], gl[2];
#pragma unroll
    for (int kg = 0; kg < 2; ++kg) {
      uint2 hq[2], lq[2];
#pragma unroll
      for (int qq = 0; qq < 2; ++qq) {
        const int q = kg * 2 + qq;
        const f32x4 bq = *reinterpret_cast<const f32x4*>(lb1 + c * 32 + 8 * q + 4 * hsel);
        float v[4];
#pragma unroll
        for (int r = 0; r < 4; r += 2) {
          const f32x2 t = omni_gelu2(__builtin_elementwise_fma(f32x2{a1[0][q * 4 + r], a1[0][q * 4 + r + 1]} + f32x2{a1[1][q * 4 + r], a1[1][q * 4 + r + 1]},
                                                               (f32x2)osc1, f32x2{bq[r], bq[r + 1]}));
          v[r] = t[0]; v[r + 1] = t[1];
        }
        omni_split4(v, hq[qq], lq[qq], amax);
      }
      gh[kg] = __builtin_bit_cast(f16x8, u32x4{hq[0].x, hq[0].y, hq[1].x, hq[1].y});
      gl[kg] = __builtin_bit_cast(f16x8, u32x4{lq[0].x, lq[0].y, lq[1].x, lq[1].y});
    }
#pragma unroll
    for (int kg = 0; kg < 2; ++kg)
#pragma unroll
      for (int j = 0; j < OB; j += 2) {
        const unsigned char* sw = st + W1B + j * 4096;
        const f16x8 wh0 = *reinterpret_cast<const f16x8*>(sw + fo[kg][0]), wl0 = *reinterpret_cast<const f16x8*>(sw + fo[kg][1]);
        const f16x8 wh1 = *reinterpret_cast<const f16x8*>(sw + 4096 + fo[kg][0]), wl1 = *reinterpret_cast<const f16x8*>(sw + 4096 + fo[kg][1]);
        acc2[0][j] = __builtin_amdgcn_mfma_f32_32x32x16_f16(wh0, gh[kg], acc2[0][j], 0, 0, 0);
        acc2[0][j + 1] = __builtin_amdgcn_mfma_f32_32x32x16_f16(wh1, gh[kg], acc2[0][j + 1], 0, 0, 0);
        acc2[0][j] = __builtin_amdgcn_mfma_f32_32x32x16_f16(wl0, gh[kg], acc2[0][j], 0, 0, 0);
        acc2[0][j + 1] = __builtin_amdgcn_mfma_f32_32x32x16_f16(wl1, gh[kg], acc2[0][j + 1], 0, 0, 0);
        acc2[0][j] = __builtin_amdgcn_mfma_f32_32x32x16_f16(wh0, gl[kg], acc2[0][j], 0, 0, 0);
        acc2[0][j + 1] = __builtin_amdgcn_mfma_f32_32x32x16_f16(wh1, gl[kg], acc2[0][j + 1], 0, 0, 0);
      }
  }
  omni_report_range(amax);
  gemm_epilogue<NW * 32, C, NW, 1, 1, OB, 2 * STAGE, OMNI_ACT_NONE, false, true>(acc2, a.ep, lds, m0, 0, wave, lane, a.ep.oscale);
#endif
}

template <int BM, int BN, int WM, int WN, int NSTAGE>
int launch_tile(GemmArgs& a, int rows_per_img, int act, int osplit, bool scores, hipStream_t s) {
  if (rows_per_img % BM != 0) {
    omni_set_error("gemm_dma: per-image weights need whole %d-row tiles per image (rows per image %d)", BM, rows_per_img);
    return OMNI_E_ARG;
  }
  a.img_tiles = rows_per_img / BM;
  a.mtiles = (a.M + BM - 1) / BM;
  a.ntiles = a.N / BN;
  a.xcd_order = (a.mtiles >= 64 && a.ntiles > 1) ? 1 : 0;
  a.xcd_n = a.xcd_order ? choose_xcd_n(a.ntiles, 4ll * a.N * a.K) : 1;
  dim3 grid(tile_grid(a.mtiles, a.ntiles, a.xcd_order, a.xcd_n)), block(WM * WN * 64);
  const bool res = a.res != nullptr;
  constexpr int SCHED1 = (BM == 256 && BN == 256) ? 1 : 0;
  const char* sched_e = getenv("OMNI_GEMM_SCHED");
  const bool lockstep = sched_e && atoi(sched_e) == 1;
#define OMNI_GD(ACT_, OS_, RES_)                                                                                                   \
  do {                                                                                                                             \
    if constexpr (BM == 256 && BN == 256) {                                                                                        \
      if (!lockstep) { hipLaunchKernelGGL((gemm_dma_kernel<BM, BN, WM, WN, NSTAGE, ACT_, OS_, RES_, 2>), grid, block, 0, s, a); break; }  \
    }                                                                                                                              \
    hipLaunchKernelGGL((gemm_dma_kernel<BM, BN, WM, WN, NSTAGE, ACT_, OS_, RES_, SCHED1>), grid, block, 0, s, a);                  \
  } while (0)
  if (scores) {
    if constexpr (BM == 256 && BN == 256) OMNI_GD(GEMM_EPI_SCORES, false, false);
    else { omni_set_error("gemm_dma: the scores epilogue is built for the 256x256 tile"); return OMNI_E_ARG; }
  }
  else if (act == OMNI_ACT_NONE && !osplit && !res) OMNI_GD(OMNI_ACT_NONE, false, false);
  else if (act == OMNI_ACT_NONE && !osplit && res) OMNI_GD(OMNI_ACT_NONE, false, true);
  else if (act == OMNI_ACT_NONE && osplit && !res) OMNI_GD(OMNI_ACT_NONE, true, false);
  else if (act == OMNI_ACT_GELU && osplit && !res) OMNI_GD(OMNI_ACT_GELU, true, false);
  else if (act == OMNI_ACT_GELU && !osplit && !res) OMNI_GD(OMNI_ACT_GELU, false, false);
#undef OMNI_GD
  else {
    omni_set_error("gemm_dma: unsupported epilogue (act %d, split out %d, residual %d)", act, osplit, (int)res);
    return OMNI_E_ARG;
  }
  return OMNI_OK;
}

}

int omni_launch_gemm_dma(const omni_op_t* op, hipStream_t s) {
  GemmArgs a{};
  a.x = (const unsigned char*)op->p[0]; a.w = (const unsigned char*)op->p[1]; a.bias = (const float*)op->p[2];
  a.res = (const float*)op->p[3]; a.y = (unsigned char*)op->p[4];
  const int B = op->i[0], H = op->i[1], W = op->i[2];
  a.K = op->i[3]; a.ldi = op->i[4]; a.in_coff = op->i[5];
  a.N = op->i[12]; a.ldo = op->i[13]; a.out_coff = op->i[14];
  const int act = op->i[15];
  a.ldr = op->i[16]; a.res_coff = op->i[17];
  const int osplit = op->i[21];
  a.oscale = op->f[1] != 0.0f ? op->f[1] : 1.0f;
  OMNI_REQUIRE(op->dtype == OMNI_F32, "gemm_dma: f32 plans only");
  OMNI_REQUIRE(op->i[28] == 0 || op->i[28] == 1, "gemm_dma: unknown epilogue mode %d (i28)", op->i[28]);
  const bool scores = op->i[28] == 1;
  OMNI_REQUIRE(a.x && a.w && (a.y || scores), "gemm_dma: null pointer");
  if (scores) a.y = (unsigned char*)op->p[7];
  OMNI_REQUIRE(op->i[6] == 1 && op->i[7] == 1 && op->i[8] == 1 && op->i[9] == 0 && op->i[10] == H && op->i[11] == W,
               "gemm_dma: pointwise layers only");
  OMNI_REQUIRE(op->f[0] == 0.0f, "gemm_dma: output scale is not supported");
  const long long M = (long long)B * H * W;
  OMNI_REQUIRE(M > 0 && M < (1ll << 31), "gemm_dma: bad M");
  a.M = (int)M;
  OMNI_REQUIRE(a.K >= 32 && a.K % 32 == 0 && a.N % 128 == 0, "gemm_dma: needs K %% 32 == 0 and N %% 128 == 0 (K %d, N %d)", a.K, a.N);
  OMNI_REQUIRE(a.ldi % 16 == 0 && a.in_coff % 16 == 0, "gemm_dma: split input needs 16-channel aligned ld / offset (%d, %d)", a.ldi, a.in_coff);
  OMNI_REQUIRE(a.ldo % 4 == 0 && a.out_coff % 4 == 0 && (!osplit || (a.ldo % 16 == 0 && a.out_coff % 16 == 0)), "gemm_dma: output alignment");
  OMNI_REQUIRE(!a.res || (a.ldr % 4 == 0 && a.res_coff % 4 == 0), "gemm_dma: residual alignment");
  OMNI_REQUIRE((long long)a.ldi * 4 * 256 < (1ll << 31) && (long long)a.K * 4 * 256 < (1ll << 31) && (long long)a.ldo * 4 * 256 < (1ll << 31) &&
               (long long)a.ldr * 4 * 256 < (1ll << 31), "gemm_dma: row stride too large");
  a.nk = a.K / 32;
  const int rows_per_img = op->i[26];
  OMNI_REQUIRE(rows_per_img >= 0 && op->i[27] >= 0, "gemm_dma: bad per-image weight arguments (%d rows, stride %d)", rows_per_img, op->i[27]);
  if (rows_per_img > 0) {
    OMNI_REQUIRE(a.M % rows_per_img == 0, "gemm_dma: %d rows are no whole number of images of %d rows", a.M, rows_per_img);
    OMNI_REQUIRE(op->i[27] % 16 == 0 && (op->i[27] == 0 || op->i[27] >= a.N * a.K * 4), "gemm_dma: per-image weight stride %d (N %d, K %d)", op->i[27], a.N, a.K);
    a.w_img_stride = (unsigned)op->i[27];
    a.img_oscale = (const float*)op->p[6];
  }
  if (scores) {
    OMNI_REQUIRE(a.y, "gemm_dma: the scores epilogue needs its workspace (p7)");
    OMNI_REQUIRE(rows_per_img > 0 && rows_per_img % 256 == 0, "gemm_dma: the scores epilogue needs whole 256-row chunks per image (i26 = %d)", rows_per_img);
    OMNI_REQUIRE(a.N % 256 == 0, "gemm_dma: the scores epilogue needs N %% 256 == 0 (N %d)", a.N);
    OMNI_REQUIRE(act == OMNI_ACT_NONE && !a.res && !osplit, "gemm_dma: the scores epilogue takes no activation, residual or format-B output");
  }
  int tile = (a.N % 256 == 0) ? 0 : 1;
  {
    const long long mt256 = (a.M + 255) / 256;
    if (mt256 * (a.N / (tile == 0 ? 256 : 128)) < 256) tile = (tile == 0 && mt256 * (a.N / 128) >= 256) ? 1 : 2;
  }
  if (const char* e = getenv("OMNI_GEMM_TILE")) {
    if (!strcmp(e, "256x128")) tile = 1;
    else if (!strcmp(e, "128x128")) tile = 2;
    else if (!strcmp(e, "256x256") && a.N % 256 == 0) tile = 0;
  }
  if (scores) tile = 0;
  int rc;
  if (tile == 0) rc = launch_tile<256, 256, 2, 4, 2>(a, rows_per_img, act, osplit, scores, s);
  else if (tile == 1) rc = launch_tile<256, 128, 4, 2, 3>(a, rows_per_img, act, osplit, false, s);
  else rc = launch_tile<128, 128, 2, 2, 2>(a, rows_per_img, act, osplit, false, s);
  if (rc) return rc;
  OMNI_HIP_CHECK(hipGetLastError());
  return OMNI_OK;
}

int omni_launch_split_convert(const omni_op_t* op, hipStream_t s) {
  const long long rows = (long long)op->i[0] * (op->i[1] > 0 ? op->i[1] : 1);
  const int C = op->i[3], ldi = op->i[4], in_coff = op->i[5], ldo = op->i[13], out_coff = op->i[14];
  OMNI_REQUIRE(op->dtype == OMNI_F32 && op->p[0] && op->p[4], "split_convert: f32 plans, non-null pointers");
  OMNI_REQUIRE(rows > 0 && C > 0 && C % 16 == 0 && ldi % 16 == 0 && in_coff % 16 == 0 && ldo % 16 == 0 && out_coff % 16 == 0,
               "split_convert: 16-channel alignment (C %d, ld %d/%d, off %d/%d)", C, ldi, ldo, in_coff, out_coff);
  const long long total = rows * (C / 16);
  hipLaunchKernelGGL(split_convert_kernel, dim3((unsigned)((total + 255) / 256)), dim3(256), 0, s, (const float*)op->p[0],
                     (unsigned char*)op->p[4], rows, C, ldi, in_coff, ldo, out_coff);
  OMNI_HIP_CHECK(hipGetLastError());
  return OMNI_OK;
}

int omni_launch_mlp_fused(const omni_op_t* op, hipStream_t s) {
  MlpArgs a{};
  a.x = (const unsigned char*)op->p[0]; a.w1 = (const unsigned char*)op->p[1]; a.b1 = (const float*)op->p[2];
  a.w2 = (const unsigned char*)op->p[5];
  a.ep.x = nullptr; a.ep.w = nullptr; a.ep.bias = (const float*)op->p[6]; a.ep.res = (const float*)op->p[3]; a.ep.y = (unsigned char*)op->p[4];
  const long long M = (long long)op->i[0] * (op->i[1] > 0 ? op->i[1] : 1);
  const int C = op->i[3], HID = op->i[12];
  a.ldi = op->i[4]; a.in_coff = op->i[5];
  a.ep.ldo = op->i[13]; a.ep.out_coff = op->i[14]; a.ep.ldr = op->i[16]; a.ep.res_coff = op->i[17];
  a.osc1 = op->f[1] != 0.0f ? op->f[1] : 1.0f;
  a.ep.oscale = op->f[2] != 0.0f ? op->f[2] : 1.0f;
  OMNI_REQUIRE(op->dtype == OMNI_F32, "mlp_fused: f32 plans only");
  OMNI_REQUIRE(a.x && a.w1 && a.w2 && a.b1 && a.ep.bias && a.ep.res && a.ep.y, "mlp_fused: null pointer (both biases and the residual are required)");
  OMNI_REQUIRE(C == 128 && HID == 512, "mlp_fused: built for C = 128, hidden = 512 (got %d, %d)", C, HID);
  OMNI_REQUIRE(M > 0 && M < (1ll << 31), "mlp_fused: bad row count");
  OMNI_REQUIRE(a.ldi % 16 == 0 && a.in_coff % 16 == 0, "mlp_fused: split input needs 16-channel aligned ld / offset");
  OMNI_REQUIRE(a.ep.ldo % 4 == 0 && a.ep.out_coff % 4 == 0 && a.ep.ldr % 4 == 0 && a.ep.res_coff % 4 == 0, "mlp_fused: output / residual alignment");
  OMNI_REQUIRE((long long)a.ep.ldo * 4 * 128 < (1ll << 31) && (long long)a.ep.ldr * 4 * 128 < (1ll << 31), "mlp_fused: row stride too large");
  a.ep.M = (int)M; a.ep.N = C; a.ep.K = HID; a.ep.nk = 0; a.ep.ldi = 0; a.ep.in_coff = 0;
  a.ep.mtiles = a.ep.ntiles = a.ep.xcd_order = a.ep.xcd_n = 0;
  hipLaunchKernelGGL((mlp_fused_kernel<128, 512>), dim3((unsigned)((M + 127) / 128)), dim3(256), 0, s, a);
  OMNI_HIP_CHECK(hipGetLastError());
  return OMNI_OK;
}
```

omniparser_amd/csrc/omni_internal.h:

```cpp
#pragma once
#include <hip/hip_runtime.h>
#include <hip/hip_fp16.h>
#include <stdint.h>
#include <stdio.h>
#include <string>
#include "../../include/omni_amd.h"

void omni_set_error(const char* fmt, ...);

#define OMNI_HIP_CHECK(expr)                                                        \
  do {                                                                              \
    hipError_t _e = (expr);                                                         \
    if (_e != hipSuccess) {                                                         \
      omni_set_error("%s failed: %s (%s:%d)", #expr, hipGetErrorString(_e), __FILE__, __LINE__); \
      return OMNI_E_HIP;                                                            \
    }                                                                               \
  } while (0)

#define OMNI_REQUIRE(cond, ...)                 \
  do {                                          \
    if (!(cond)) {                              \
      omni_set_error(__VA_ARGS__);              \
      return OMNI_E_ARG;                        \
    }                                           \
  } while (0)

#ifndef OMNI_WAIT_VMCNT
#define OMNI_WAIT_VMCNT(n) asm volatile("s_waitcnt vmcnt(%0)" ::"n"(n) : "memory")
#endif

#ifndef OMNI_WAIT_LGKM0
#define OMNI_WAIT_LGKM0() asm volatile("s_waitcnt lgkmcnt(0)" ::: "memory")
#endif

#ifndef OMNI_DYN_LDS
#define OMNI_DYN_LDS(type, name) extern __shared__ type name[]
#endif

#ifndef OMNI_WAVE_SYNC
#define OMNI_WAVE_SYNC() __builtin_amdgcn_wave_barrier()
#endif

typedef _Float16 half_t;
typedef float f32x4 __attribute__((ext_vector_type(4)));
typedef float f32x16 __attribute__((ext_vector_type(16)));
typedef _Float16 f16x8 __attribute__((ext_vector_type(8)));
typedef _Float16 f16x4 __attribute__((ext_vector_type(4)));
typedef uint32_t u32x4 __attribute__((ext_vector_type(4)));

template <typename T> struct ElemTraits;
template <> struct ElemTraits<float> {
  static constexpr int kVec = 4;
  static __host__ __device__ __forceinline__ float to_f32(float v) { return v; }
  static __host__ __device__ __forceinline__ float from_f32(float v) { return v; }
};
template <> struct ElemTraits<half_t> {
  static constexpr int kVec = 8;
  static __host__ __device__ __forceinline__ float to_f32(half_t v) { return (float)v; }
  static __host__ __device__ __forceinline__ half_t from_f32(float v) { return (half_t)v; }
};

static __device__ unsigned int omni_ovf_count_tu;
#define OMNI_F16_MAX 65504.0f
__device__ __forceinline__ float omni_amax4(const float* v, float amax) {
  amax = __builtin_fmaxf(__builtin_fmaxf(__builtin_fabsf(v[0]), __builtin_fabsf(v[1])), amax);
  return __builtin_fmaxf(__builtin_fmaxf(__builtin_fabsf(v[2]), __builtin_fabsf(v[3])), amax);
}
__device__ __forceinline__ void omni_report_range(float amax) {
  if (__builtin_expect(amax > OMNI_F16_MAX, 0)) atomicAdd(&omni_ovf_count_tu, 1u);
}
typedef int (*omni_ovf_reader_t)(unsigned int* count, int reset);
void omni_register_overflow_reader(omni_ovf_reader_t fn);
#define OMNI_RANGE_GUARD_TU()                                                                                               \
  namespace {                                                                                                               \
  int omni_ovf_read_tu(unsigned int* count, int reset) {                                                                    \
    unsigned int v = 0;                                                                                                     \
    if (hipMemcpyFromSymbol(&v, HIP_SYMBOL(omni_ovf_count_tu), sizeof v, 0, hipMemcpyDeviceToHost) != hipSuccess) return 1; \
    if (reset && v) {                                                                                                       \
      const unsigned int z = 0;                                                                                             \
      if (hipMemcpyToSymbol(HIP_SYMBOL(omni_ovf_count_tu), &z, sizeof z, 0, hipMemcpyHostToDevice) != hipSuccess) return 1; \
    }                                                                                                                       \
    *count = v;                                                                                                             \
    return 0;                                                                                                               \
  }                                                                                                                         \
  struct OmniOvfReg { OmniOvfReg() { omni_register_overflow_reader(&omni_ovf_read_tu); } } omni_ovf_reg;                   \
  }

__device__ __forceinline__ void omni_split4_raw(const float* v, uint2& hi, uint2& lo) {
  typedef __fp16 hv2 __attribute__((ext_vector_type(2)));
  float c[4];
#pragma unroll
  for (int e = 0; e < 4; ++e) c[e] = __builtin_fminf(__builtin_fmaxf(v[e], -OMNI_F16_MAX), OMNI_F16_MAX);
  hv2 h01 = __builtin_amdgcn_cvt_pkrtz(c[0], c[1]);
  hv2 h23 = __builtin_amdgcn_cvt_pkrtz(c[2], c[3]);
  float m1 = -1.0f;
  asm("" : "+r"(m1));
  hv2 l01 = __builtin_amdgcn_cvt_pkrtz(__builtin_fmaf((float)h01[0], m1, c[0]), __builtin_fmaf((float)h01[1], m1, c[1]));
  hv2 l23 = __builtin_amdgcn_cvt_pkrtz(__builtin_fmaf((float)h23[0], m1, c[2]), __builtin_fmaf((float)h23[1], m1, c[3]));
  hi.x = __builtin_bit_cast(unsigned, h01); hi.y = __builtin_bit_cast(unsigned, h23);
  lo.x = __builtin_bit_cast(unsigned, l01); lo.y = __builtin_bit_cast(unsigned, l23);
}
__device__ __forceinline__ void omni_split4(const float* v, uint2& hi, uint2& lo, float& amax) {
  amax = omni_amax4(v, amax);
  omni_split4_raw(v, hi, lo);
}
__device__ __forceinline__ void omni_split4(const float* v, uint2& hi, uint2& lo) {
  omni_report_range(omni_amax4(v, 0.0f));
  omni_split4_raw(v, hi, lo);
}
__device__ __forceinline__ void omni_split1(float v, unsigned short& hi, unsigned short& lo) {
  typedef __fp16 hv2 __attribute__((ext_vector_type(2)));
  omni_report_range(__builtin_fabsf(v));
  v = __builtin_fminf(__builtin_fmaxf(v, -OMNI_F16_MAX), OMNI_F16_MAX);
  hv2 h = __builtin_amdgcn_cvt_pkrtz(v, 0.0f);
  hv2 l = __builtin_amdgcn_cvt_pkrtz(v - (float)h[0], 0.0f);
  hi = (unsigned short)(__builtin_bit_cast(unsigned, h) & 0xffffu);
  lo = (unsigned short)(__builtin_bit_cast(unsigned, l) & 0xffffu);
}
__device__ __forceinline__ int omni_split_half_index(int c) { return (c >> 4) * 32 + (c & 15); }
__device__ __forceinline__ int omni_split_off(int c) { return (c >> 4) * 64 + (c & 15) * 2; }

__device__ __forceinline__ float omni_erff(float a) {
  const float t = __builtin_fminf(__builtin_fabsf(a), 6.0f), s = t * t;
  float r = __builtin_fmaf(-1.72853470e-5f, t, 3.83197126e-4f);
  const float u = __builtin_fmaf(-3.88396438e-3f, t, 2.42546219e-2f);
  r = __builtin_fmaf(r, s, u);
  r = __builtin_fmaf(r, t, -1.06777847e-1f);
  r = __builtin_fmaf(r, t, -6.34846687e-1f);
  r = __builtin_fmaf(r, t, -1.28717512e-1f);
  r = __builtin_fmaf(r, t, -t);
  const float big = __builtin_copysignf(1.0f - __expf(r), a);
  float q = -5.96761703e-4f;
  q = __builtin_fmaf(q, s, 4.99119423e-3f);
  q = __builtin_fmaf(q, s, -2.67681349e-2f);
  q = __builtin_fmaf(q, s, 1.12819925e-1f);
  q = __builtin_fmaf(q, s, -3.76125336e-1f);
  q = __builtin_fmaf(q, s, 1.28379166e-1f);
  const float small = __builtin_fmaf(q, a, a);
  return t > 0.927734375f ? big : small;
}
__device__ __forceinline__ float omni_gelu(float v) { return 0.5f * v * (1.0f + omni_erff(v * 0.70710678118654752440f)); }
typedef float f32x2 __attribute__((ext_vector_type(2)));
#if defined(__AMDGCN__)
#define OMNI_EXP2(x) __builtin_amdgcn_exp2f(x)
#else
#define OMNI_EXP2(x) __builtin_exp2f(x)
#endif
__device__ __forceinline__ f32x2 omni_gelu2(f32x2 v) {
  const f32x2 t = __builtin_elementwise_min(__builtin_elementwise_abs(v), (f32x2)8.48528137423857f);
  f32x2 p = __builtin_elementwise_fma((f32x2)1.137868688e-09f, t, (f32x2)-5.171069262e-08f);
  p = __builtin_elementwise_fma(p, t, (f32x2)1.014483701e-06f);
  p = __builtin_elementwise_fma(p, t, (f32x2)-1.117507963e-05f);
  p = __builtin_elementwise_fma(p, t, (f32x2)7.388171798e-05f);
  p = __builtin_elementwise_fma(p, t, (f32x2)-2.645340865e-04f);
  p = __builtin_elementwise_fma(p, t, (f32x2)-3.723767077e-05f);
  p = __builtin_elementwise_fma(p, t, (f32x2)6.994847674e-03f);
  p = __builtin_elementwise_fma(p, t, (f32x2)-5.247364566e-02f);
  p = __builtin_elementwise_fma(p, t, (f32x2)-4.592104554e-01f);
  p = __builtin_elementwise_fma(p, t, (f32x2)-1.151105404e+00f);
  p = __builtin_elementwise_fma(p, t, (f32x2)1.941864447e-08f);
  const f32x2 E = {OMNI_EXP2(p[0]), OMNI_EXP2(p[1])};
  const f32x2 c1 = __builtin_elementwise_copysign((f32x2)0.5f, v);
  return v * __builtin_elementwise_fma(-c1, E, 0.5f + c1);
}

int omni_launch_conv(const omni_op_t* op, hipStream_t s);
int omni_launch_gemm_dma(const omni_op_t* op, hipStream_t s);
int omni_launch_split_convert(const omni_op_t* op, hipStream_t s);
int omni_launch_mlp_fused(const omni_op_t* op, hipStream_t s);
int omni_launch_avgpool2(const omni_op_t* op, hipStream_t s);
int omni_launch_maxpool(const omni_op_t* op, hipStream_t s);
int omni_launch_resize_nearest(const omni_op_t* op, hipStream_t s);
int omni_launch_letterbox(const omni_op_t* op, hipStream_t s);
int omni_launch_detect_decode(const omni_op_t* op, hipStream_t s);
int omni_launch_nms(const omni_op_t* op, hipStream_t s);
int omni_launch_dwconv3(const omni_op_t* op, hipStream_t s);
int omni_launch_layernorm(const omni_op_t* op, hipStream_t s);
int omni_launch_dwconv3_ln(const omni_op_t* op, hipStream_t s);
int omni_launch_attention(const omni_op_t* op, hipStream_t s);
int omni_launch_misc(const omni_op_t* op, hipStream_t s);
int omni_launch_vocab_step(const omni_op_t* op, hipStream_t s);
int omni_launch_visual_match(const omni_op_t* op, hipStream_t s);
long long omni_visual_match_part_bytes(const omni_op_t* op);
int omni_launch_region_ocr(const omni_op_t* op, hipStream_t s);
bool omni_region_ocr_extents(const omni_op_t* op, long long ext[8]);
int omni_launch_glue(const omni_op_t* op, hipStream_t s);
int omni_launch_overlay(const omni_op_t* op, hipStream_t s);
int omni_launch_png_pack(const omni_op_t* op, hipStream_t s);
int omni_launch_png_deflate(const omni_op_t* op, hipStream_t s);
```

omniparser_amd/florence.py:

```python
import contextlib
import json
import math
import os
from pathlib import Path
from types import SimpleNamespace
from typing import Dict, List, Optional

import numpy as np
import torch

from . import _lib as L
from .planner import PlanBuilder, View, torch_dtype

PROMPT_IDS = [0, 2264, 473, 5, 2274, 6190, 116, 2]
TEXT_CAPACITIES = (8, 16, 32, 64)


def text_capacity(n_tokens: int) -> int:
    for c in TEXT_CAPACITIES:
        if n_tokens <= c:
            return c
    raise ValueError(f"a prompt of {n_tokens} tokens exceeds the captioner's limit of {TEXT_CAPACITIES[-1]} prompt tokens "
                     "(bos and eos included)")

# ... 863 lines not shown
        if cap.use_graph:
            self.reset()
            for p in plans:
                p.run(cap.stream)
            cap.stream.synchronize()
            for p in plans:
                p.capture(cap.stream)
            cap.stream.synchronize()


class _DecodePlans(_StepPlans):

    def __init__(self, cap: "Florence2Captioner", B: int, R: int, max_new: int, beam=None, n_txt=None, scores=False, vocab=False):
        w, dev, dt = cap.w, cap.device, cap.dtype
        self.B, self.R = B, R
        S = (R // 32) ** 2 + 1 + (len(PROMPT_IDS) if n_txt is None else n_txt)
        self.S = S
        self.n_txt = n_txt
        pk = PlanBuilder(dev, dt)
        self.nkeys = None
        if n_txt is not None:
            self.nkeys = pk.raw((B,), torch.int32)
            self.nkeys.fill_(S)
        self.cross_kv = [pk.alloc(B, S, 1, 2 * w.d_model, zero=True) for _ in range(w.dec_layers)]
        self._keep = pk.keep
        self._build_step(cap, B, max_new, S, self.cross_kv, beam=beam, nkeys=self.nkeys, scores=scores, vocab=vocab)
        self.free_evt = None
        self._warm_up_and_capture(cap, self.step_plan)


class _CaptionPlans(_StepPlans):

    def __init__(self, cap: "Florence2Captioner", B: int, R: int, max_new: int, arena: Optional["_CaptionPlans"] = None, stream=None,
                 beam=None, n_txt=None, scores=False, force=None, controls=False, vocab=False, embed=False):
        w, dev, dt = cap.w, cap.device, cap.dtype
        if arena is not None:
            n_txt = arena.n_txt
        self.embed = bool(embed)
        self.n_txt = n_txt
        sd = w.sd
        self.B, self.R, self.T = B, R, max_new + 1
        pb = PlanBuilder(dev, dt)
        pb.reuse = bool(cap.reuse_activations)
        if arena is not None:
            assert arena.R == R and arena.B >= B and arena.arena is None
            pb.arena = iter(arena.pb.alloc_log)
        self.arena = arena
        self._row_plans = {}
        self.pb = pb
        V = pb.V
        W = _Weights(cap, pb)

        use_dma = dt == L.F32 and pb.split and os.environ.get("OMNI_GEMM_DMA", "1") != "0"
        self.use_dma = use_dma
        grp = {"dma": use_dma}

        def tokens(v: View) -> View:
            return View(v.t.view(v.B, v.H * v.W, 1, v.ld), v.coff, v.C, v.fmt)

        def linear(key, x: View, out: View, act=L.ACT_NONE, res=None, bias=True, keys=None, out_split=False):
            keys = keys or [key]
            n_out, k_in = out.C, x.C
            dma = grp["dma"] and n_out % 128 == 0 and k_in % 32 == 0 and x.ld % 16 == 0 and x.coff % 16 == 0
            assert dma or x.fmt != "split", f"{keys}: split input for a layer that cannot take the LDS-DMA GEMM"
            wp, bp = W.linear(keys, bias, dma)
            if dma and x.fmt != "split":
                pb.split_convert(x)
            xt, ot = tokens(x), tokens(out)
            pb.conv(xt, wp, bp, ot, 1, act=act, res=tokens(res) if res is not None else None, out_split=dma and out_split)
            out.fmt = ot.fmt
            return out

        def layernorm(key, x: View, out: View, add=None, period=0, eps=1e-5, split=None):
            rows = x.B * x.H * x.W
            omode, y2 = 0, None
            if grp["dma"] and split is not None and x.C % 16 == 0:
                omode, y2 = (1, None) if split is out else (2, split)
            pb.add_op(W.layernorm(key, x.ptr, out.ptr, rows, x.C, add=add.data_ptr() if add is not None else None,
                                  y2=y2.ptr if y2 is not None else None, period=period, omode=omode, eps=eps))
            out.fmt = "split" if omode == 1 else "f32"
            if y2 is not None:
                y2.fmt = "split"
            return out

        def dwconv(key, x: View, out: View):
            wp, bp = W.dwconv(key)
            pb.keep += [wp, bp]
            pb.add_op(L.make_op(L.OP_DWCONV3, dt, p=[x.ptr, wp.data_ptr(), bp.data_ptr(), None, out.ptr],
                                i={0: x.B, 1: x.H, 2: x.W, 3: x.C}))
            return out

        fuse_env = cap.fuse_dwln
        attn_split = use_dma and cap.attn_split_out

        def dwconv_ln(conv_key, norm_key, x: View, y1: View, hout: View):
            if not (fuse_env and dt == L.F32 and x.C in (128, 256, 512)):
                dwconv(conv_key, x, y1)
                return layernorm(norm_key, y1, hout, split=hout)
            wp, bp = W.dwconv(conv_key)
            pb.keep += [wp, bp]
            pb.add_op(L.make_op(L.OP_DWCONV3_LN, dt,
                                p=[x.ptr, wp.data_ptr(), bp.data_ptr(), hout.ptr, y1.ptr,
                                   W.f32(norm_key + ".weight").data_ptr(), W.f32(norm_key + ".bias").data_ptr()],
                                i={0: x.B, 1: x.H, 2: x.W, 3: x.C, 6: 1 if grp["dma"] else 0}, f={0: 1e-5}))
            hout.fmt = "split" if grp["dma"] else "f32"
            return hout

        self.x_in = pb.alloc(B, R, R, V, zero=True)
        x = self.x_in
        vt = "model.vision_tower."
        self.chan_ws = None
        self.fold_stages = []
        self.stage_out = []
        for s in range(4):
            C = w.embed_dim[s]
            grp["dma"] = use_dma and C % 128 == 0
            k, st, pd = w.patch[s]
            Ho = (x.H + 2 * pd - k) // st + 1
            conv_key = f"{vt}convs.{s}.conv"
            if w.prenorm[s]:
                xn = pb.alloc(B, x.H, x.W, x.C)
                layernorm(f"{vt}convs.{s}.norm", x, xn)
                cur = pb.alloc(B, Ho, Ho, C)
                wp, bp = W.packed(conv_key, lambda: (sd[conv_key + ".weight"], sd[conv_key + ".bias"]))
                pb.conv(xn, wp, bp, cur, k, st, pd)
                pb.release(xn, *([] if x is self.x_in else [x]))
            else:
                t0 = pb.alloc(B, Ho, Ho, C)
                if cap.patch_rows and dt == L.F32 and pb.split and V == 4 and k <= 8 and x is self.x_in:
                    wp, bp = W.cached((conv_key, dt, "patch"), lambda: (pb.pack_weight_patch(sd[conv_key + ".weight"], V),
                                                                         pb.upload(sd[conv_key + ".bias"].float())))
                    pb.conv_patch(x, wp, bp, t0, k, st, pd)
                else:
                    wp, bp = W.cached((conv_key, dt, "pad"), lambda: (pb.pack_weight(sd[conv_key + ".weight"], cin_pad=V),
                                                                       pb.upload(sd[conv_key + ".bias"].float())))
                    pb.conv(x, wp, bp, t0, k, st, pd)
                cur = pb.alloc(B, Ho, Ho, C)
                layernorm(f"{vt}convs.{s}.norm", t0, cur)
                pb.release(t0)
            H = Ho
            N = H * H
            A_, B_ = cur, pb.alloc(B, H, H, C)
            hbuf = pb.alloc(B, H, H, C)
            qkv = pb.alloc(B, H, H, 3 * C)
            att = pb.alloc(B, H, H, C)
            mlp_one = grp["dma"] and cap.fuse_mlp and C == 128 and sd[f"{vt}blocks.{s}.0.spatial_block.ffn.fc1.weight"].shape[0] == 512
            ffn = None if mlp_one else pb.alloc(B, H, H, 4 * C)
            fold = bool(cap.fold_chan_proj) and grp["dma"] and dt == L.F32 and C % 128 == 0 and N % 256 == 0 and N >= 4 * C
            chunk_tokens = 1024
            partial_tokens = 256 if fold else 0
            chunks = (N + (partial_tokens or chunk_tokens) - 1) // (partial_tokens or chunk_tokens)
            cws = pb.raw((B * w.groups[s] * chunks * 1024,), torch.float32, zero=False)
            scores_in_gemm = fold and bool(cap.chan_scores_in_gemm)
            fold_wf = fold_wb = fold_sc = fold_mx = None
            if fold:
                fold_wf = pb.raw((B * C * C,), torch.float32, zero=False)
                fold_wb = pb.raw((B * C * C,), torch.float32, zero=False)
                fold_sc = pb.raw((B,), torch.float32, zero=False)
                fold_mx = pb.raw((B * (C // 64) * w.groups[s],), torch.float32, zero=False)
            if fold:
                self.fold_stages.append(s)
            for blk in range(w.depths[s]):
                for kind in ("spatial_block", "channel_block"):
                    pre = f"{vt}blocks.{s}.{blk}.{kind}."
                    dwconv_ln(pre + "conv1", pre + "norm1", A_, B_, hbuf)
                    if kind == "spatial_block":
                        linear(pre + "window_attn.qkv", hbuf, qkv)
                        qb = W.f32(pre + "window_attn.qkv.bias")
                        nw = ((H + 11) // 12) ** 2
                        pb.add_op(L.make_op(
                            L.OP_ATTN_ROWS, dt,
                            p=[qkv.ptr, qkv.ptr, qkv.ptr, None, att.ptr, qb.data_ptr() + 4 * C, qb.data_ptr() + 8 * C],
                            i={0: 3 * C, 1: 3 * C, 2: 3 * C, 3: C, 4: 0, 5: C, 6: 2 * C, 7: 0, 8: w.heads[s], 9: 144, 10: 144,
                               11: B * nw, 12: 1, 13: H, 14: H, 15: C // w.heads[s], 16: 1 if (attn_split and grp["dma"]) else 0},
                            f={0: (C // w.heads[s]) ** -0.5}))
                        att.fmt = "split" if (attn_split and grp["dma"]) else "f32"
                        linear(pre + "window_attn.proj", att, B_, res=B_)
                    elif fold:
                        key = pre + "channel_attn.qkv"
                        wp, _ = W.linear([key], dma=True)
                        wqk, bqk, wv, bv = W.cached((key, dt, "dma-qk|v"), lambda: (
                            pb.weight_rows(wp, 0, 2 * C), pb.upload(sd[key + ".bias"][:2 * C].float()),
                            pb.weight_rows(wp, 2 * C, C), pb.upload(sd[key + ".bias"][2 * C:].float())))
                        assert hbuf.fmt == "split"
                        if scores_in_gemm:
                            wqs, bqs = W.cached((key, dt, "dma-qk-groups"), lambda: (
                                pb.pack_weight_qk_groups(wqk), pb.upload(sd[key + ".bias"][:2 * C].float()[pb.qk_group_rows(C)])))
                            pb.conv_scores(tokens(hbuf), wqs, bqs, cws, N)
                        else:
                            pb.conv(tokens(hbuf), wqk, bqk, tokens(qkv.slice(0, 2 * C)), 1)
                        vs = tokens(qkv.slice(2 * C, C))
                        pb.conv(tokens(hbuf), wv, bv, vs, 1, out_split=True)
                        pkey = pre + "channel_attn.proj"
                        wplain, bproj = W.f32(pkey + ".weight"), W.f32(pkey + ".bias")
                        pb.keep += [wplain, bproj]
                        pb.add_op(L.make_op(L.OP_CHAN_ATTN, dt,
                                            p=[qkv.ptr, wplain.data_ptr(), fold_wf.data_ptr(), fold_wb.data_ptr(), None, cws.data_ptr(),
                                               fold_sc.data_ptr(), fold_mx.data_ptr()],
                                            i={0: B, 1: N, 3: C, 4: w.groups[s], 5: chunk_tokens, 6: 1 if (attn_split and grp["dma"]) else 0, 8: 1,
                                               9: 1 if scores_in_gemm else 0, 10: partial_tokens}))
                        pb.conv_per_image(vs, fold_wb, fold_sc, bproj, tokens(B_), tokens(B_), N)
                    else:
                        linear(pre + "channel_attn.qkv", hbuf, qkv)
                        pb.add_op(L.make_op(L.OP_CHAN_ATTN, dt, p=[qkv.ptr, None, None, None, att.ptr, cws.data_ptr()],
                                            i={0: B, 1: N, 3: C, 4: w.groups[s], 5: chunk_tokens, 6: 1 if (attn_split and grp["dma"]) else 0}))
                        att.fmt = "split" if (attn_split and grp["dma"]) else "f32"
                        linear(pre + "channel_attn.proj", att, B_, res=B_)
                    dwconv_ln(pre + "conv2", pre + "norm2", B_, A_, hbuf)
                    if mlp_one:
                        k1, k2 = pre + "ffn.fc1", pre + "ffn.fc2"
                        w1p, b1p = W.linear([k1], dma=True)
                        w2p, b2p = W.cached((k2, dt, "dma-kperm"), lambda: (pb.pack_weight_dma(sd[k2 + ".weight"], kperm=True),
                                                                             pb.upload(sd[k2 + ".bias"].float())))
                        pb.mlp_fused(tokens(hbuf), w1p, b1p, w2p, b2p, tokens(A_), tokens(A_))
                        continue
                    linear(pre + "ffn.fc1", hbuf, ffn, act=L.ACT_GELU, out_split=True)
                    linear(pre + "ffn.fc2", ffn, A_, res=A_)
            x = A_
            self.stage_out.append(A_)
            pb.release(B_, hbuf, qkv, att, ffn, cws, fold_wf, fold_wb, fold_sc, fold_mx)
        self.vision_out = x
        grp["dma"] = use_dma
        mp = "model.multi_modal_projector."
        h = x.H
        Cv = x.C

        def pos_tables():
            col = sd[mp + "image_position_embed.column_embeddings.weight"][:h]
            row = sd[mp + "image_position_embed.row_embeddings.weight"][:h]
            pos = torch.cat([col.unsqueeze(0).repeat(h, 1, 1), row.unsqueeze(1).repeat(1, h, 1)], -1).reshape(h * h, Cv)
            return pb.upload(pos.float()), pb.upload(sd[mp + "visual_temporal_embed.pos_idx_to_embed"][0].float())
        pos2d, temporal = W.cached(("pos2d", h), pos_tables)
        pb.keep += [pos2d, temporal]
        n_img = h * h + 1
        self.n_img = n_img
        pp = pb.alloc(B, n_img, 1, Cv)
        pb.add_op(L.make_op(L.OP_PROJ_PREP, dt, p=[x.ptr, pos2d.data_ptr(), temporal.data_ptr(), None, pp.ptr],
                            i={0: B, 1: h * h, 3: Cv}))
        D = w.d_model
        pj = pb.alloc(B, n_img, 1, D)
        linear(mp + "image_projection", pp, pj, bias=False)
        img_feat = pb.alloc(B, n_img, 1, D)
        layernorm(mp + "image_proj_norm", pj, img_feat)
        self.img_feat = img_feat
        if embed:
            assert arena is None and not (beam or force or controls or vocab or scores) and n_txt is None
            self.emb = pb.raw((B, D), torch.float32)
            self.emb_norm = pb.raw((B,), torch.float32)
            pb.add_op(embed_op(dt, img_feat.ptr, n_img * D, self.emb, self.emb_norm, B, D))
            self.S = self.prompt_ids = self.nkeys = self.step_plan = self.free_evt = None
            self.cross_kv = []
            self.n_encode_ops = len(pb.ops)
            self.encode_flops = pb.flops
            self.encode_plan = pb.build()
            if dev.type == "cuda":
                torch.cuda.synchronize(dev)
            if cap.use_graph:
                self.encode_plan.run(cap.stream)
                cap.stream.synchronize()
                self.encode_plan.capture(cap.stream)
                cap.stream.synchronize()
            return
        lm = "model.language_model."
        S = n_img + (len(PROMPT_IDS) if n_txt is None else n_txt)
        self.S = S
        self.prompt_ids = self.nkeys = None
        if n_txt is None:
            txt = W.cached(("prompt", dt), lambda: pb.upload((sd[lm + "shared.weight"][torch.tensor(PROMPT_IDS)] * w.embed_scale).to(torch_dtype(dt))))
            pb.keep.append(txt)
            enc = pb.alloc(B, S, 1, D)
            pb.add_op(L.make_op(L.OP_ASSEMBLE, dt, p=[img_feat.ptr, txt.data_ptr(), None, None, enc.ptr],
                                i={0: B, 1: n_img, 2: len(PROMPT_IDS), 3: D}))
        else:
            table, _ = W.token_tables()
            pb.keep.append(table)
            self.prompt_ids = pb.raw((B, n_txt), torch.int32)
            self.nkeys = pb.raw((B,), torch.int32)
            if arena is None:
                self.prompt_ids.fill_(w.pad)
                self.nkeys.fill_(S)
            enc = pb.alloc(B, S, 1, D)
            pb.add_op(L.make_op(L.OP_ASSEMBLE, dt, p=[img_feat.ptr, None, self.prompt_ids.data_ptr(), table.data_ptr(), enc.ptr],
                                i={0: B, 1: n_img, 2: n_txt, 3: D, 4: table.shape[0]}, f={0: w.embed_scale}))
        encpos = W.cached(("encpos", S, dt), lambda: pb.upload(sd[lm + "encoder.embed_positions.weight"][2:2 + S].to(torch_dtype(dt))))
        pb.keep.append(encpos)
        xa = pb.alloc(B, S, 1, D)
        dma_enc = grp["dma"] = use_dma and D % 128 == 0
        xs = pb.alloc(B, S, 1, D) if dma_enc else None
        layernorm(lm + "encoder.layernorm_embedding", enc, xa, add=encpos, period=S, split=xs)
        xin = xs if dma_enc else xa
        qkv = pb.alloc(B, S, 1, 3 * D)
        att = pb.alloc(B, S, 1, D)
        tmp = pb.alloc(B, S, 1, D)
        ffn = pb.alloc(B, S, 1, sd[lm + "encoder.layers.0.fc1.weight"].shape[0])
        nh = w.n_heads
        for l in range(w.enc_layers):
            pre = f"{lm}encoder.layers.{l}."
            linear(None, xin, qkv, keys=[pre + "self_attn.q_proj", pre + "self_attn.k_proj", pre + "self_attn.v_proj"])
            pb.add_op(L.make_op(L.OP_ATTN_ROWS, dt, p=[qkv.ptr, qkv.ptr, qkv.ptr, None, att.ptr]
                                + ([None, None, self.nkeys.data_ptr()] if self.nkeys is not None else []),
                                i={0: 3 * D, 1: 3 * D, 2: 3 * D, 3: D, 4: 0, 5: D, 6: 2 * D, 7: 0, 8: nh, 9: S, 10: S, 11: B,
                                   12: 0, 15: 64, 16: 1 if (attn_split and dma_enc) else 0}, f={0: 64 ** -0.5}))
            att.fmt = "split" if (attn_split and dma_enc) else "f32"
            linear(pre + "self_attn.out_proj", att, tmp, res=xa)
            layernorm(pre + "self_attn_layer_norm", tmp, xa, split=xs)
            linear(pre + "fc1", xin, ffn, act=L.ACT_GELU, out_split=True)
            linear(pre + "fc2", ffn, tmp, res=xa)
            layernorm(pre + "final_layer_norm", tmp, xa, split=xs)
        self.enc_out = xa
        self.cross_kv = []
        for l in range(w.dec_layers):
            pre = f"{lm}decoder.layers.{l}.encoder_attn."
            kv = pb.alloc(B, S, 1, 2 * D)
            linear(None, xin, kv, keys=[pre + "k_proj", pre + "v_proj"])
            self.cross_kv.append(kv)
        self.free_evt = None
        self.n_encode_ops = len(pb.ops)
        self.encode_flops = pb.flops
        self.encode_plan = pb.build()
        if arena is not None:
            assert len(pb.alloc_log) == len(arena.pb.alloc_log) and self.n_encode_ops == arena.n_encode_ops, \
                "arena replay: the two builds made different allocation / op sequences"
            if cap.use_graph:
                self.encode_plan.capture(stream or cap.stream)
            return
        self._build_step(cap, B, max_new, S, self.cross_kv, pb.ws, beam=beam, nkeys=self.nkeys, scores=scores, force=force, controls=controls,
                         vocab=vocab)
        self._warm_up_and_capture(cap, self.encode_plan, self.step_plan)

    def set_prompt(self, ids: torch.Tensor, nkeys: torch.Tensor, n: int):
        assert self.prompt_ids is not None and ids.shape[-1] == self.n_txt and n <= self.B
        self.prompt_ids[:n].copy_(ids.expand(n, -1), non_blocking=True)
        self.nkeys[:n].copy_(nkeys.expand(n), non_blocking=True)

    def rows_for(self, cap: "Florence2Captioner", n: int) -> int:
        last, cap._last_remainder = getattr(cap, "_last_remainder", None), n
        if n in self._row_plans or n == last:
            return n
        return min(cap.bucket(n), self.B)

    def encode_rows(self, cap: "Florence2Captioner", n: int, stream=None) -> "_CaptionPlans":
        assert self.arena is None and 1 <= n <= self.B
        if n == self.B:
            return self
        cp = self._row_plans.pop(n, None)
        if cp is None:
            while len(self._row_plans) >= max(1, int(cap.row_graphs)):
                if dev_sync := (cap.device.type == "cuda"):
                    torch.cuda.synchronize(cap.device)
                self._row_plans.pop(next(iter(self._row_plans)))
            cp = _CaptionPlans(cap, n, self.R, self.T - 1, arena=self, stream=stream)
            cap.row_graph_builds = getattr(cap, "row_graph_builds", 0) + 1
        self._row_plans[n] = cp
        return cp


class _Config(SimpleNamespace):
    pass


class Florence2Captioner:
    fuse_dwln = True
    attn_split_out = True
    fold_chan_proj = True
    chan_scores_in_gemm = True
    fuse_mlp = True
    exact_rows = os.environ.get("OMNI_EXACT_ROWS", "1") != "0"
    row_graphs = int(os.environ.get("OMNI_CAPTION_ROW_GRAPHS", "24"))
    patch_rows = os.environ.get("OMNI_PATCH_ROWS", "1") != "0"
    reuse_activations = True

    long_kv_budget_bytes = 2 ** 30

    def __init__(self, model_dir, device=None, precision: Optional[str] = None, resolution: Optional[int] = None):
        device = L.require_device(device, "Florence2Captioner")
        L.lib()
        self.device = device
        precision = precision or os.environ.get("OMNI_PRECISION", "f32")
        self.dtype = L.F32 if precision == "f32" else L.F16
        self.resolution = int(resolution or os.environ.get("OMNI_CAPTION_RES", "768"))
        self.w = FlorenceWeights(model_dir)
        self.config = _Config(name_or_path=str(model_dir) if "florence" in str(model_dir).lower() else f"florence:{model_dir}",
                              model_type="florence2")
        self.use_graph = os.environ.get("OMNI_HIPGRAPH", "1") != "0"
        self.stream = self._lane_stream(0)
        self._wcache = {}
        self._plans = {}
        self.max_new_tokens = 20
        self.early_exit_every = 5
        self.num_beams = 1
        self.token_scores = False
        self.last_steps = 0
        self._lut, self._bic = None, {}
        self._lock = L.DeviceLock(self.device, reentrant=True)

    def to(self, *a, **k):
        return self

    def eval(self):
        return self

    @staticmethod
    def bucket(n: int) -> int:
        for b in _BUCKETS:
            if n <= b:
                return b
        return _BUCKETS[-1]

    def max_new_limit(self) -> int:
        return int(self.w.sd["model.language_model.decoder.embed_positions.weight"].shape[0]) - 2

    def check_max_new(self, max_new_tokens, beam=None) -> int:
        lim, why = self.max_new_limit(), "the decoder's position table has no row beyond that"
        if beam and beam_max_new(beam[0]) < lim:
            lim, why = beam_max_new(beam[0]), f"beam search with num_beams={beam[0]} stages every position of its beams in LDS"
        n = max_new_tokens
        if isinstance(n, bool) or not isinstance(n, int) or n < 1 or n > lim:
            raise ValueError(f"max_new_tokens must be an integer in 1..{lim} ({why}), got {n!r}")
        return n

    def long_plan_rows(self, max_new_tokens: int, k: int = 1) -> int:
        per_row = (int(max_new_tokens) + 1) * self.w.d_model * 4 * 2 * self.w.dec_layers * max(int(k), 1)
        fit = [b for b in _BUCKETS if b * per_row <= self.long_kv_budget_bytes]
        return fit[-1] if fit else _BUCKETS[0]

    @staticmethod
    def decode_bucket(n: int) -> int:
        return max(128, (n + 31) // 32 * 32)

    def begin_batch(self):
        self._epoch = getattr(self, "_epoch", 0) + 1

    def _wcache_bytes(self) -> int:
        n = 0
        for v in self.__dict__.get("_wcache", {}).values():
            for t in (v if isinstance(v, (tuple, list)) else (v,)):
                if isinstance(t, torch.Tensor):
                    n += t.numel() * t.element_size()
        return n

    def plan_cache_bytes(self) -> int:
        return sum(m[0] for k, m in self.__dict__.get("_plan_meta", {}).items() if k in self._plans)

    def clear_plans(self):
        self._plans.clear()
        self.__dict__.get("_plan_meta", {}).clear()

    def _cached_plan(self, key, build):
        meta = self.__dict__.setdefault("_plan_meta", {})
        epoch = getattr(self, "_epoch", 0)
        if key in self._plans:
            self._plans[key] = self._plans.pop(key)
            meta.setdefault(key, [0, epoch])[1] = epoch
            return self._plans[key]
        max_bytes = int(float(os.environ.get("OMNI_CAPTION_PLAN_GB", "200")) * 2 ** 30)
        max_plans = int(os.environ.get("OMNI_MAX_CAPTION_PLANS", "16"))
        base = key[:4] if key[0] == "dec" else key[:3]
        sizes = self.__dict__.setdefault("_plan_sizes", {})
        est = sizes.get(base, 0)
        if not est and sizes:
            same = [(b, v) for b, v in sizes.items() if (b[0] == "dec") == (base[0] == "dec") and b[-2] == base[-2] and v]
            if same:
                b0, v0 = max(same, key=lambda bv: bv[1])
                rows0, rows = (b0[1] if b0[0] == "dec" else b0[0]), (base[1] if base[0] == "dec" else base[0])
                est = int(v0 * rows / max(rows0, 1))
        def over():
            return len(self._plans) >= max_plans or (self._plans and self.plan_cache_bytes() + est > max_bytes)
        while over():
            victim = next((k for k in self._plans if meta.get(k, [0, None])[1] != epoch), None)
            if victim is None:
                break
            torch.cuda.synchronize(self.device)
            self._plans.pop(victim)
            meta.pop(victim, None)
            self.plan_evictions = getattr(self, "plan_evictions", 0) + 1
            L.gc_after_eviction()
        on_gpu = self.device.type == "cuda" and torch.cuda.is_available()
        before = torch.cuda.memory_allocated(self.device) if on_gpu else 0
        w_before = self._wcache_bytes()
        import contextlib
        with (torch.cuda.device(self.device) if self.device.type == "cuda" else contextlib.nullcontext()):
            obj = build()
        self._plans[key] = obj
        grown = (torch.cuda.memory_allocated(self.device) if on_gpu else 0) - before - (self._wcache_bytes() - w_before)
        meta[key] = [max(0, grown), epoch]
        sizes[base] = meta[key][0]
        return obj

    def beam_config(self, num_beams=None, length_penalty=None, early_stopping=None):
        k = self.num_beams if num_beams is None else num_beams
        if isinstance(k, bool) or not isinstance(k, int) or k < 1 or k > BEAM_MAX:
            raise ValueError(f"num_beams must be an integer in 1..{BEAM_MAX} (got {k!r})")
        if k == 1:
            return None
        lp = float(self.w.length_penalty if length_penalty is None else length_penalty)
        es = check_early_stopping(self.w.early_stopping if early_stopping is None else early_stopping)
        return (k, lp, es)

    @torch.inference_mode()
    def decode_plans(self, B, R, max_new, slot=0, beam=None, n_txt=None, scores=False, vocab=False) -> _DecodePlans:
        self.check_max_new(max_new, beam)
        if vocab and beam:
            raise ValueError("a closed vocabulary is applied by greedy decoding only (no beam search)")
        key = ("dec", B, R, max_new) if slot == 0 else ("dec", B, R, max_new, slot)
        if beam or n_txt is not None:
            key = ("dec", B, R, max_new, slot, beam) + (() if n_txt is None else (("txt", n_txt),))
        if scores:
            key = ("dec", B, R, max_new, slot, beam) + (() if n_txt is None else (("txt", n_txt),)) + ("scores",)
        if vocab:
            key = ("dec", B, R, max_new, slot, None) + (() if n_txt is None else (("txt", n_txt),)) + (("scores",) if scores else ()) + ("vocab",)
            return self._cached_plan(key, lambda: _DecodePlans(self, B, R, max_new, n_txt=n_txt, scores=scores, vocab=True))
        return self._cached_plan(key, lambda: _DecodePlans(self, B, R, max_new, beam=beam, n_txt=n_txt, scores=scores))

    @torch.inference_mode()
    def plans(self, B, R, max_new, slot=0, beam=None, n_txt=None, scores=False, force=None, controls=False, vocab=False) -> _CaptionPlans:
        self.check_max_new(max_new, beam)
        if vocab and (beam or force or controls):
# ... 526 lines not shown
```

omniparser_amd/opwork.py:

```python

NAMES = {1: "conv_igemm/conv_split", 2: "avgpool2", 3: "maxpool", 4: "resize_nearest", 5: "letterbox", 6: "detect_decode", 7: "nms",
         8: "dwconv3", 9: "layernorm", 10: "attn_rows (window / MHA)", 11: "chan_attn", 12: "proj_prep", 13: "assemble", 14: "embed_step",
         15: "attn_decode", 16: "greedy_step", 17: "crop_resize", 18: "dwconv3_ln", 19: "split_convert", 20: "hand_off", 21: "overlay",
         22: "png_pack", 23: "png_deflate", 24: "mlp_fused", 26: "greedy_ctrl_step", 28: "visual_match", 29: "region_ocr"}

MFMA_KINDS = (1, 24, 10)


def op_work(op, esz=4):
    i = op.i
    k = op.kind
    if k == 1:
        M, N, K = i[0] * i[10] * i[11], i[12], i[6] * i[7] * i[3]
        if i[25]:
            K = i[6] * i[6] * i[4]
            return 2 * M * N * K, esz * (i[0] * i[1] * i[2] * i[4] + N * K + M * N)
        if i[20] == 2 and i[28] == 1:
            return 2 * M * N * K + 2 * M * N * 16, esz * (M * K + N * K + (M // 256) * (N // 64) * 1024)
        nw = M // i[26] if (i[20] == 2 and i[26] > 0) else 1
        return 2 * M * N * K, esz * (i[0] * i[1] * i[2] * i[3] + nw * N * K + M * N * (2 if op.p[3] else 1))
    if k == 24:
        rows, C, hid = i[0] * max(i[1], 1), i[3], i[12]
        return 4 * rows * C * hid, esz * (3 * rows * C + 2 * C * hid)
    if k in (2, 3, 4):
        return 0, esz * (i[0] * i[1] * i[2] * i[3] + i[0] * max(i[10], 1) * max(i[11], 1) * i[3])
    if k in (8, 18):
        n = i[0] * i[1] * i[2] * i[3]
        return 18 * n, esz * n * (2 if k == 8 else 3)
    if k == 9:
        n = i[0] * max(i[1], 1) * i[3]
        return 8 * n, esz * 2 * n
    if k == 10:
        heads, nq, nk, groups, D = i[8], i[9], i[10], i[11], i[15]
        return 4 * groups * heads * nq * nk * D, esz * groups * (nq + 2 * nk + nq) * heads * D
    if k == 11:
        B, N, C = i[0], i[1], i[3]
        if i[8] == 1 and i[9] == 1:
            ct = i[10] or i[5]
            chunks = (N + ct - 1) // ct
            return 2 * B * C * C * 32, esz * (B * (C // 32) * chunks * 1024 + C * C + B * C * C)
        if i[8] == 1:
            return 2 * B * N * C * 32 + 2 * B * C * C * 32, esz * (B * N * C * 2 + C * C + B * C * C)
        return 4 * B * N * C * 32, esz * B * N * C * 4
    if k == 15:
        B, heads, nk = i[10], i[6], (i[7] if i[7] > 0 else i[8])
        return 4 * B * heads * nk * 64, esz * B * nk * i[9] * 2
    if k in (16, 26):
        return 0, esz * i[0] * i[1]
    if k == 28:
        if i[0] == 0:
            n, D = i[1], i[3]
            return 3 * n * D, n * D * (esz + 4) + 4 * n
        m, n, D, kk = i[1], i[2], i[3], i[4]
        ln = i[5] if i[5] > 0 else None
        splits = (n + ln - 1) // ln if ln else 1
        if i[0] == 1:
            return 2 * m * n * D, 4 * (m + n) * D + 8 * m * splits * kk
        return 0, 8 * m * splits * kk + 8 * m * kk
    if k == 29:
        if i[0] == 0:
            n, R, ldo = i[1], i[4], i[13]
            return 2 * 3 * n * R * R, n * R * R * (3 + ldo * esz)
        n, T, M = i[1], i[2], i[3]
        return 0, n * (4 * T + (4 * (T - 1) if op.p[2] else 0) + 68 * M + 16 + 24)
    return 0, 0


def op_shape(op):
    i, k = op.i, op.kind
    if k in (1, 19):
        return (i[0] * max(i[10], 1) * max(i[11], 1) if k == 1 else i[0] * max(i[1], 1), i[12] if k == 1 else i[3], i[6] * i[7] * i[3] if k == 1 else 0)
    if k == 24:
        return (i[0] * max(i[1], 1), i[3], i[12])
    if k in (8, 18):
        return (i[0] * i[1] * i[2], i[3], 0)
    if k == 9:
        return (i[0] * max(i[1], 1), i[3], i[6])
    if k == 10:
        return (i[11] * i[9], i[8] * i[15], i[12])
    if k == 11:
        return (i[0] * i[1], i[3], (2 if i[9] == 1 else 1) if i[8] == 1 else 0)
    if k == 15:
        return (i[10], i[9], i[7] if i[7] > 0 else i[8])
    if k == 28:
        return (i[1], i[3], 0 if i[0] == 0 else i[2])
    if k == 29:
        return (i[1], i[4] if i[0] == 0 else i[2], 0)
    return (i[0], i[3], 0)


def op_kernel(op):
    if op.kind == 1:
        if op.i[20] == 2 and op.i[28] == 1:
            return "gemm_dma (scores epilogue)"
        if op.i[20] == 2 and op.i[26] > 0:
            return "gemm_dma (per-image weights)"
        return "gemm_dma" if op.i[20] == 2 else ("conv_split" if op.i[20] else "conv_igemm")
    if op.kind == 11 and op.i[8] == 1:
        return "chan_attn (fold)" if op.i[9] == 1 else "chan_attn (scores + fold)"
    if op.kind == 28:
        return ("visual_match (embed)", "visual_match (partial top-k)", "visual_match (merge)")[op.i[0]] if 0 <= op.i[0] <= 2 else "visual_match"
    if op.kind == 29:
        return ("region_ocr (tile cut)", "region_ocr (parse)")[op.i[0]] if 0 <= op.i[0] <= 1 else "region_ocr"
    return NAMES.get(op.kind, str(op.kind))
```

omniparser_amd/planner.py:

```python
import math
import os
from dataclasses import dataclass
from typing import Optional

import torch

from . import _lib as L


def vec_width(dtype: int) -> int:
    return 4 if dtype == L.F32 else 8


def torch_dtype(dtype: int):
    return torch.float32 if dtype == L.F32 else torch.float16


@dataclass
class View:
    t: torch.Tensor
    coff: int
    C: int
    fmt: str = "f32"

# ... 111 lines not shown
        if need > have or not src.is_contiguous():
            raise RuntimeError(f"arena replay: tensor of shape {tuple(shape)} ({need} B) does not fit the arena's {tuple(src.shape)} ({have} B)")
        t = src.view(-1).view(torch.uint8)[:need].view(dtype).view(shape)
        self.alloc_log.append(t)
        return t

    def release(self, *tensors):
        if not self.reuse or self.arena is not None:
            return
        for t in tensors:
            t = t.t if isinstance(t, View) else t
            if t is None or id(t) in self._released or t.numel() == 0:
                continue
            self._released.add(id(t))
            self._pins.append(t)
            nbytes = t.numel() * t.element_size() // 256 * 256
            if nbytes:
                self._free.append((t.view(-1).view(torch.uint8)[:nbytes], nbytes))

    def _from_free(self, shape, dtype):
        if not self.reuse or not self._free:
            return None
        need = math.prod(shape) * torch.empty((), dtype=dtype).element_size()
        cand = [(nb, k) for k, (_, nb) in enumerate(self._free) if nb >= need]
        if not cand or need == 0:
            return None
        nb, k = min(cand)
        block, _ = self._free.pop(k)
        rest = (nb - need) // 256 * 256
        if rest:
            self._free.append((block[nb - rest:], rest))
        self.reused_bytes += need
        return block[:need].view(dtype).view(shape)

    def upload(self, host_tensor: torch.Tensor) -> torch.Tensor:
        t = host_tensor.contiguous().to(self.device)
        self.keep.append(_register(t, "const"))
        return t

    @staticmethod
    def split_f16(w2d: torch.Tensor) -> torch.Tensor:
        cout, K = w2d.shape
        assert K % 16 == 0
        w2d = w2d.float().clamp(-65504.0, 65504.0)
        hi = w2d.to(torch.float16)
        lo = ((w2d - hi.float()) * 2048.0).to(torch.float16)
        return torch.cat([hi.view(cout, K // 16, 16), lo.view(cout, K // 16, 16)], -1).contiguous()

    @staticmethod
    def split_f16_b(w2d: torch.Tensor):
        cout, K = w2d.shape
        assert K % 16 == 0
        w2d = w2d.double()
        amax = float(w2d.abs().max())
        k = 0 if amax == 0.0 else 12 - math.floor(math.log2(amax))
        k = max(-24, min(24, k))
        ws = (w2d * (2.0 ** k)).float()
        hi = ws.to(torch.float16)
        lo = (ws - hi.float()).to(torch.float16)
        return torch.cat([hi.view(cout, K // 16, 16), lo.view(cout, K // 16, 16)], -1).contiguous(), 2.0 ** -k

    KPERM16 = (0, 1, 2, 3, 8, 9, 10, 11, 4, 5, 6, 7, 12, 13, 14, 15)

    def pack_weight_dma(self, w: torch.Tensor, kperm: bool = False) -> torch.Tensor:
        w2d = w.detach().float().reshape(w.shape[0], -1)
        if kperm:
            cout, K = w2d.shape
            assert K % 16 == 0
            w2d = w2d.view(cout, K // 16, 16)[:, :, list(self.KPERM16)].reshape(cout, K).contiguous()
        t, oscale = self.split_f16_b(w2d)
        t = self.upload(t)
        t.omni_fmt, t.omni_oscale = 2, oscale
        return t

    def pack_weight(self, w: torch.Tensor, cin_pad: Optional[int] = None) -> torch.Tensor:
        w = w.detach().float()
        cout, cin, kh, kw = w.shape
        if cin_pad and cin_pad > cin:
            w = torch.cat([w, w.new_zeros(cout, cin_pad - cin, kh, kw)], 1)
        w = w.permute(0, 2, 3, 1).reshape(cout, -1)
        cin_eff = max(cin, cin_pad or 0)
        if self.split and self.dtype == L.F32 and cin_eff % 32 == 0 and cin_eff * kh * kw >= 128:
            t = self.upload(self.split_f16(w))
            t.omni_fmt = 1
            return t
        return self.upload(w.to(torch_dtype(self.dtype)))

    def conv(self, x: View, w_packed: torch.Tensor, bias: Optional[torch.Tensor], out: View, k: int, s: int = 1,
             p: Optional[int] = None, act: int = L.ACT_NONE, res: Optional[View] = None, scale: float = 0.0,
             out_split: bool = False):
        p = k // 2 if p is None else p
        Ho = (x.H + 2 * p - k) // s + 1
        Wo = (x.W + 2 * p - k) // s + 1
        assert (out.B, out.H, out.W) == (x.B, Ho, Wo), ((out.B, out.H, out.W), (x.B, Ho, Wo))
        cout = out.C
        wfmt = getattr(w_packed, "omni_fmt", 0) if self.dtype == L.F32 else 0
        if wfmt:
            assert w_packed.dtype == torch.float16 and w_packed.numel() == 2 * cout * k * k * x.C and x.C % 32 == 0, \
                (tuple(w_packed.shape), cout, k, x.C)
        else:
            assert tuple(w_packed.shape) == (cout, k * k * x.C), (tuple(w_packed.shape), cout, k, x.C)
        if wfmt == 2:
            assert k == 1 and s == 1 and p == 0 and scale == 0.0 and cout % 128 == 0, "format-B weights: pointwise layers, Cout % 128 == 0"
            assert x.fmt == "split", "the LDS-DMA GEMM reads a pre-split input: its producer must emit format B (or insert split_convert)"
            assert x.ld % 16 == 0 and x.coff % 16 == 0 and not (out_split and (res is not None or out.ld % 16 or out.coff % 16))
        else:
            assert x.fmt == "f32" and not out_split, "register-staged conv kernels read and write f32"
        if res is not None:
            assert (res.B, res.H, res.W, res.C) == (out.B, out.H, out.W, out.C) and res.fmt == "f32"
        b = None
        if bias is not None:
            b = bias if bias.device == self.device and bias.dtype == torch.float32 else self.upload(bias.detach().float())
            ent = _TENSORS.get(b.data_ptr())
            if ent is None or ent[0]() is not b:
                _register(b, "const")
            self.keep.append(b)
            assert b.numel() == cout
        if self.ws is None and (self.device.type == "cuda" or self.workspace_on_host):
            self.ws = self.raw((self.ws_kib * 256,), torch.float32, zero=False)
        if self.cnt is None and self.ws is not None and self.n_cnt and wfmt == 1:
            self.cnt = self.raw((self.n_cnt,), torch.int32, zero=True)
        cnt = self.cnt if (wfmt == 1 and self.cnt is not None) else None
        tune = (0, 0)
        if wfmt == 1 and self.conv_tuning:
            tune = tuple(self.conv_tuning.get(conv_key(x.B * Ho * Wo, cout, k * k * x.C, k, s), (0, 0)))
        op = L.make_op(
            L.OP_CONV, self.dtype,
            p=[x.ptr, w_packed.data_ptr(), b.data_ptr() if b is not None else None,
               res.ptr if res is not None else None, out.ptr, self.ws.data_ptr() if self.ws is not None else None,
               cnt.data_ptr() if cnt is not None else None],
            i={0: x.B, 1: x.H, 2: x.W, 3: x.C, 4: x.ld, 5: x.coff, 6: k, 7: k, 8: s, 9: p, 10: Ho, 11: Wo,
               12: cout, 13: out.ld, 14: out.coff, 15: act,
               16: res.ld if res is not None else 0, 17: res.coff if res is not None else 0,
               19: self.ws_kib if self.ws is not None else 0, 20: wfmt, 21: 1 if out_split else 0,
               22: tune[0], 23: tune[1], 24: cnt.numel() if cnt is not None else 0},
            f={0: scale, 1: getattr(w_packed, "omni_oscale", 0.0) if wfmt == 2 else 0.0})
        self.ops.append(op)
        self.keep.append(w_packed)
        out.fmt = "split" if out_split else "f32"
        M = x.B * Ho * Wo
        esz = 4 if self.dtype == L.F32 else 2
        self.flops += 2 * M * cout * k * k * x.C
        self.bytes += esz * (x.B * x.H * x.W * x.C + w_packed.numel() // (2 if wfmt else 1) + M * cout * (2 if res is not None else 1))
        return out

    @staticmethod
    def weight_rows(w_packed: torch.Tensor, row0: int, rows: int) -> torch.Tensor:
        assert getattr(w_packed, "omni_fmt", 0) == 2 and 0 <= row0 and row0 + rows <= w_packed.shape[0]
        t = w_packed[row0:row0 + rows]
        t.omni_fmt, t.omni_oscale = 2, w_packed.omni_oscale
        return t

    def conv_per_image(self, x: View, w_img: torch.Tensor, scales: torch.Tensor, bias: Optional[torch.Tensor], out: View,
                       res: Optional[View], rows_per_img: int):
        cout, K = out.C, x.C
        M = x.B * x.H * x.W
        assert self.dtype == L.F32 and x.fmt == "split" and x.ld % 16 == 0 and x.coff % 16 == 0 and cout % 128 == 0 and K % 32 == 0
        assert (out.B, out.H, out.W) == (x.B, x.H, x.W) and M % rows_per_img == 0
        nimg = M // rows_per_img
        assert w_img.numel() * w_img.element_size() >= nimg * cout * K * 4 and scales.dtype == torch.float32 and scales.numel() >= nimg
        assert bias is None or (bias.dtype == torch.float32 and bias.numel() == cout and bias.device.type == self.device.type)
        if res is not None:
            assert (res.B, res.H, res.W, res.C) == (out.B, out.H, out.W, out.C) and res.fmt == "f32"
        self.ops.append(L.make_op(
            L.OP_CONV, self.dtype,
            p=[x.ptr, w_img.data_ptr(), bias.data_ptr() if bias is not None else None, res.ptr if res is not None else None, out.ptr,
               None, scales.data_ptr()],
            i={0: x.B, 1: x.H, 2: x.W, 3: K, 4: x.ld, 5: x.coff, 6: 1, 7: 1, 8: 1, 9: 0, 10: x.H, 11: x.W, 12: cout, 13: out.ld, 14: out.coff,
               15: L.ACT_NONE, 16: res.ld if res is not None else 0, 17: res.coff if res is not None else 0, 20: 2,
               26: rows_per_img, 27: cout * K * 4}))
        self.keep += [w_img, scales] + ([bias] if bias is not None else [])
        out.fmt = "f32"
        self.flops += 2 * M * cout * K
        self.bytes += 4 * (M * K + nimg * cout * K + M * cout * (2 if res is not None else 1))
        return out

    @staticmethod
    def qk_group_rows(C: int):
        assert C % 32 == 0
        return [part * C + g * 32 + r for g in range(C // 32) for part in (0, 1) for r in range(32)]

    def pack_weight_qk_groups(self, w_qk: torch.Tensor) -> torch.Tensor:
        assert getattr(w_qk, "omni_fmt", 0) == 2 and w_qk.shape[0] % 64 == 0
        idx = torch.tensor(self.qk_group_rows(w_qk.shape[0] // 2), device=w_qk.device)
        t = self.upload(w_qk[idx])
        t.omni_fmt, t.omni_oscale = 2, w_qk.omni_oscale
        return t

    def conv_scores(self, x: View, w_qk: torch.Tensor, bias: Optional[torch.Tensor], ws: torch.Tensor, rows_per_img: int):
        cout, K = w_qk.shape[0], x.C
        M = x.B * x.H * x.W
        assert self.dtype == L.F32 and x.fmt == "split" and x.ld % 16 == 0 and x.coff % 16 == 0 and K % 32 == 0
        assert getattr(w_qk, "omni_fmt", 0) == 2 and w_qk.numel() == 2 * cout * K and cout % 256 == 0
        assert rows_per_img > 0 and rows_per_img % 256 == 0 and M % rows_per_img == 0
        assert ws.dtype == torch.float32 and ws.numel() >= (M // 256) * (cout // 64) * 1024
        assert bias is None or (bias.dtype == torch.float32 and bias.numel() == cout and bias.device.type == self.device.type)
        self.ops.append(L.make_op(
            L.OP_CONV, self.dtype,
            p=[x.ptr, w_qk.data_ptr(), bias.data_ptr() if bias is not None else None, None, None, None, None, ws.data_ptr()],
            i={0: x.B, 1: x.H, 2: x.W, 3: K, 4: x.ld, 5: x.coff, 6: 1, 7: 1, 8: 1, 9: 0, 10: x.H, 11: x.W, 12: cout, 13: cout, 14: 0,
               15: L.ACT_NONE, 20: 2, 26: rows_per_img, 27: 0, 28: 1},
            f={1: w_qk.omni_oscale}))
        self.keep += [w_qk, ws] + ([bias] if bias is not None else [])
        self.flops += 2 * M * cout * K + 2 * M * cout * 16
        self.bytes += 4 * (M * K + cout * K + (M // 256) * (cout // 64) * 1024)

    def pack_weight_patch(self, w: torch.Tensor, ld: int = 4) -> torch.Tensor:
        w = w.detach().float()
        cout, cin, kh, kw = w.shape
        assert kh == kw and kh <= 8 and cin <= ld == 4
        full = w.new_zeros(cout, kh, 8, ld)
        full[:, :, :kw, :cin] = w.permute(0, 2, 3, 1)
        t = self.upload(self.split_f16(full.reshape(cout, kh * 8 * ld)))
        t.omni_fmt = 1
        return t

    def conv_patch(self, x: View, w_patch: torch.Tensor, bias: torch.Tensor, out: View, k: int, s: int, p: int, act: int = L.ACT_NONE):
        assert self.dtype == L.F32 and x.fmt == "f32" and x.ld == 4 and x.coff == 0 and x.C == 4 and k <= 8
        Ho = (x.H + 2 * p - k) // s + 1
        Wo = (x.W + 2 * p - k) // s + 1
        cout = out.C
        assert (out.B, out.H, out.W) == (x.B, Ho, Wo) and w_patch.numel() == 2 * cout * k * 32 and getattr(w_patch, "omni_fmt", 0) == 1
        assert bias.device.type == self.device.type and bias.dtype == torch.float32 and bias.numel() == cout
        if self.ws is None and (self.device.type == "cuda" or self.workspace_on_host):
            self.ws = self.raw((self.ws_kib * 256,), torch.float32, zero=False)
        self.ops.append(L.make_op(
            L.OP_CONV, self.dtype,
            p=[x.ptr, w_patch.data_ptr(), bias.data_ptr(), None, out.ptr, self.ws.data_ptr() if self.ws is not None else None],
            i={0: x.B, 1: x.H, 2: x.W, 3: 32, 4: 4, 5: 0, 6: k, 7: 1, 8: s, 9: p, 10: Ho, 11: Wo, 12: cout, 13: out.ld, 14: out.coff,
               15: act, 19: self.ws_kib if self.ws is not None else 0, 20: 1, 25: 1}))
        self.keep += [w_patch, bias]
        out.fmt = "f32"
        M = x.B * Ho * Wo
        self.flops += 2 * M * cout * k * k * x.C
        self.bytes += 4 * (x.B * x.H * x.W * x.C + cout * k * k * x.C + M * cout)
        return out

    def mlp_fused(self, x: View, w1: torch.Tensor, b1: torch.Tensor, w2: torch.Tensor, b2: torch.Tensor, res: View, out: View):
        C, hid = x.C, b1.numel()
        assert self.dtype == L.F32 and x.fmt == "split" and res.fmt == "f32" and (C, hid) == (128, 512), (x.fmt, res.fmt, C, hid)
        assert getattr(w1, "omni_fmt", 0) == 2 and getattr(w2, "omni_fmt", 0) == 2 and w1.numel() == 2 * hid * C == w2.numel()
        assert (out.B, out.H, out.W, out.C) == (x.B, x.H, x.W, C) == (res.B, res.H, res.W, res.C) and b2.numel() == C
        rows = x.B * x.H * x.W
        self.ops.append(L.make_op(L.OP_MLP_FUSED, self.dtype,
                                  p=[x.ptr, w1.data_ptr(), b1.data_ptr(), res.ptr, out.ptr, w2.data_ptr(), b2.data_ptr()],
                                  i={0: rows, 1: 1, 3: C, 4: x.ld, 5: x.coff, 12: hid, 13: out.ld, 14: out.coff, 16: res.ld, 17: res.coff},
                                  f={1: w1.omni_oscale, 2: w2.omni_oscale}))
        self.keep += [w1, w2, b1, b2]
        out.fmt = "f32"
        self.flops += 2 * rows * C * hid * 2
        self.bytes += 4 * (rows * C * 3 + 2 * C * hid)
        return out

    def split_convert(self, x: View, out: Optional[View] = None) -> View:
        out = out or x
        assert self.dtype == L.F32 and x.fmt == "f32" and x.C % 16 == 0 and (out.B, out.H, out.W, out.C) == (x.B, x.H, x.W, x.C)
        self.ops.append(L.make_op(L.OP_SPLIT_CONVERT, self.dtype, p=[x.ptr, None, None, None, out.ptr],
                                  i={0: x.B * x.H * x.W, 1: 1, 3: x.C, 4: x.ld, 5: x.coff, 13: out.ld, 14: out.coff}))
        self.bytes += 8 * x.B * x.H * x.W * x.C
        out.fmt = "split"
        return out

    def _pool(self, kind, x: View, out: View, k=0, s=1, p=0, accumulate=0):
        assert x.C == out.C and x.B == out.B
        op = L.make_op(
            kind, self.dtype, p=[x.ptr, None, None, None, out.ptr],
            i={0: x.B, 1: x.H, 2: x.W, 3: x.C, 4: x.ld, 5: x.coff, 6: k, 8: s, 9: p, 10: out.H, 11: out.W,
               13: out.ld, 14: out.coff, 18: accumulate})
        self.ops.append(op)
        esz = 4 if self.dtype == L.F32 else 2
        self.bytes += esz * (x.B * x.H * x.W * x.C + out.B * out.H * out.W * out.C * (2 if accumulate else 1))
        return out

    def avgpool2(self, x: View, out: View):
        assert (out.H, out.W) == (x.H - 1, x.W - 1)
        return self._pool(L.OP_AVGPOOL2, x, out)

    def maxpool(self, x: View, out: View, k, s, p):
        assert (out.H, out.W) == ((x.H + 2 * p - k) // s + 1, (x.W + 2 * p - k) // s + 1)
        return self._pool(L.OP_MAXPOOL, x, out, k, s, p)

    def resize_nearest(self, x: View, out: View, accumulate=False):
        return self._pool(L.OP_RESIZE_NEAREST, x, out, accumulate=1 if accumulate else 0)

    def resize_sum(self, srcs, out: View):
        assert 1 <= len(srcs) <= 5 and all(s.C == out.C and s.B == out.B for s in srcs)
        if len(srcs) == 1:
            return self.resize_nearest(srcs[0], out)
        x = srcs[0]
        slots = ((19, 20, 21, 22), (23, 24, 25, 26), (27, 28, 29, 30), (7, 12, 15, 16))
        pidx = (1, 2, 3, 5)
        p = [x.ptr, None, None, None, out.ptr, None]
        i = {0: x.B, 1: x.H, 2: x.W, 3: x.C, 4: x.ld, 5: x.coff, 10: out.H, 11: out.W, 13: out.ld, 14: out.coff, 17: len(srcs)}
        for k, sv in enumerate(srcs[1:]):
            p[pidx[k]] = sv.ptr
            i.update({slots[k][0]: sv.H, slots[k][1]: sv.W, slots[k][2]: sv.ld, slots[k][3]: sv.coff})
        self.ops.append(L.make_op(L.OP_RESIZE_NEAREST, self.dtype, p=p, i=i))
        esz = 4 if self.dtype == L.F32 else 2
        self.bytes += esz * (sum(s.B * s.H * s.W * s.C for s in srcs) + out.B * out.H * out.W * out.C)
        return out

    def add_op(self, op):
        self.ops.append(op)

    def build(self) -> "L.Plan":
        plan = L.Plan(self.ops)
        plan._keep = self.keep
        return plan
```

Baseline: 13.35.

## Fold V projection into per-image channel-attention weight and bias

When tokens far outnumber channels, the channel-attention V projection is no longer computed as its own GEMM over all tokens. Instead, the per-image folded projection weight W' is multiplied by Wv in a small C×C GEMM, then re-packed to split format. A folded bias (W'·bv + bp) is computed per image, and the final per-image GEMM reads the hidden tokens directly with that per-image bias. This removes one full-token GEMM and its split-format V buffer per channel-attention layer. In exchange it adds a few small kernels per image and changes rounding, since the composed weights are quantized to split format again.

```diff
diff --git a/omniparser_amd/csrc/capi.hip b/omniparser_amd/csrc/capi.hip
--- a/omniparser_amd/csrc/capi.hip
+++ b/omniparser_amd/csrc/capi.hip
@@ -104,6 +104,7 @@
         const long long nimg = (M + i[26] - 1) / i[26];
         ext[1] += (nimg - 1) * (long long)i[27];
         ext[6] = nimg * 4;
+        if (i[29] == 1) ext[2] = nimg * Cout * 4;
       }
       if (i[20] == 2 && i[28] == 1) {
         ext[7] = (M / 256) * (Cout / 64) * 4096;
@@ -115,6 +116,7 @@
       const long long B = i[0], N = i[1], C = i[3], G = i[4], ct = i[10] > 0 ? i[10] : (i[5] > 0 ? i[5] : 1);
       ext[0] = B * N * 3 * C * esz; ext[4] = B * N * C * esz; ext[5] = B * G * ((N + ct - 1) / ct) * 1024 * 4;
       if (i[8] == 1) { ext[1] = C * C * 4; ext[2] = ext[3] = B * C * C * 4; ext[6] = B * 4; ext[7] = B * (C / 64) * G * 4; }
+      if (i[8] == 1 && i[11] == 1) { ext[1] += 2 * C * 4; ext[2] += B * C * 4; }
       break;
     }
     case OMNI_OP_BEAM_STEP: {
@@ -185,6 +187,7 @@
     case OMNI_OP_SPLIT_CONVERT: {
       const long long rows = (long long)i[0] * i[1];
       ext[0] = span(rows, i[4], i[5], i[3]); ext[4] = span(rows, i[13], i[14], i[3]);
+      if (i[6] == 1) { ext[5] = (long long)i[0] * (i[3] / 64) * (i[3] / 32) * 4; ext[6] = (long long)i[0] * 4; }
       break;
     }
     case OMNI_OP_AVGPOOL2: case OMNI_OP_MAXPOOL: case OMNI_OP_RESIZE_NEAREST: {
diff --git a/omniparser_amd/csrc/caption_ops.hip b/omniparser_amd/csrc/caption_ops.hip
--- a/omniparser_amd/csrc/caption_ops.hip
+++ b/omniparser_amd/csrc/caption_ops.hip
@@ -1511,7 +1511,49 @@
 struct FoldArgs {
   const float* ws; const float* wp; float* wf; float* bmax; unsigned char* wb; float* osc;
   int C, G, chunks, nblk;
+  float oscmul;
+  const float* bv; const float* bp; float* bias;
 };
+
+__global__ __launch_bounds__(256) void chan_fold_bias_kernel(FoldArgs a) {
+  constexpr int TC = 128, PITCH = TC + 1;
+  __shared__ float sW[64 * PITCH];
+  __shared__ float sB[TC];
+  const int ob = blockIdx.x, b = blockIdx.y, tid = threadIdx.x;
+  const float* W = a.wf + ((long long)b * a.C + ob * 64) * a.C;
+  float acc = 0.0f;
+  for (int c0 = 0; c0 < a.C; c0 += TC) {
+    __syncthreads();
+    for (int e = tid; e < 64 * (TC / 4); e += 256) {
+      const int r = e / (TC / 4), q = e % (TC / 4);
+      const f32x4 v = *reinterpret_cast<const f32x4*>(W + (long long)r * a.C + c0 + 4 * q);
+      float* d = sW + r * PITCH + 4 * q;
+      d[0] = v[0]; d[1] = v[1]; d[2] = v[2]; d[3] = v[3];
+    }
+    if (tid < TC) sB[tid] = a.bv[c0 + tid];
+    __syncthreads();
+    if (tid < 64) {
+#pragma unroll 8
+      for (int i = 0; i < TC; ++i) acc = fmaf(sW[tid * PITCH + i], sB[i], acc);
+    }
+  }
+  if (tid < 64) a.bias[(long long)b * a.C + ob * 64 + tid] = acc + a.bp[ob * 64 + tid];
+}
+
+__global__ __launch_bounds__(256) void chan_fold_max_kernel(FoldArgs a) {
+  __shared__ float smax[4];
+  const int e = blockIdx.x, b = blockIdx.y, tid = threadIdx.x;
+  const float* src = a.wf + (long long)b * a.C * a.C + (long long)e * 2048 + tid * 8;
+  const f32x4 v0 = *reinterpret_cast<const f32x4*>(src), v1 = *reinterpret_cast<const f32x4*>(src + 4);
+  float m = 0.0f;
+#pragma unroll
+  for (int q = 0; q < 4; ++q) m = fmaxf(m, fmaxf(fabsf(v0[q]), fabsf(v1[q])));
+#pragma unroll
+  for (int o = 32; o >= 1; o >>= 1) m = fmaxf(m, __shfl_xor(m, o));
+  if ((tid & 63) == 0) smax[tid >> 6] = m;
+  __syncthreads();
+  if (tid == 0) a.bmax[(long long)b * a.nblk + e] = fmaxf(fmaxf(smax[0], smax[1]), fmaxf(smax[2], smax[3]));
+}
 
 __global__ __launch_bounds__(256) void chan_fold_kernel(FoldArgs a) {
   __shared__ float sA[32][32];
@@ -1563,7 +1605,7 @@
     k = max(-24, min(24, k));
   }
   const float up = __builtin_bit_cast(float, (unsigned)(127 + k) << 23);
-  if (blockIdx.x == 0 && tid == 0) a.osc[b] = __builtin_bit_cast(float, (unsigned)(127 - k) << 23);
+  if (blockIdx.x == 0 && tid == 0) a.osc[b] = __builtin_bit_cast(float, (unsigned)(127 - k) << 23) * a.oscmul;
   const int gpr = a.C / 16;
   const int idx = blockIdx.x * 256 + tid;
   if (idx >= a.C * gpr) return;
@@ -2670,6 +2712,20 @@
   return OMNI_OK;
 }
 
+int omni_launch_chan_repack(const omni_op_t* op, hipStream_t s) {
+  FoldArgs f{};
+  const int B = op->i[0], C = op->i[3];
+  f.wf = (float*)op->p[0]; f.wb = (unsigned char*)op->p[4]; f.bmax = (float*)op->p[5]; f.osc = (float*)op->p[6];
+  OMNI_REQUIRE(op->dtype == OMNI_F32 && f.wf && f.wb && f.bmax && f.osc, "split_convert (i6 = 1): f32 plans, p0 / p4 / p5 / p6");
+  OMNI_REQUIRE(B > 0 && C > 0 && C % 64 == 0 && op->i[1] == C && op->i[4] == C && op->i[5] == 0 && op->i[13] == C && op->i[14] == 0,
+               "split_convert (i6 = 1): i0 square matrices of i1 = i3 = i4 = i13 = C, C %% 64 == 0, no channel offsets (C %d)", C);
+  f.C = C; f.G = C / 32; f.nblk = (C / 64) * (C / 32); f.oscmul = 1.0f;
+  hipLaunchKernelGGL(chan_fold_max_kernel, dim3(f.nblk, B), dim3(256), 0, s, f);
+  hipLaunchKernelGGL(chan_fold_pack_kernel, dim3((C * (C / 16) + 255) / 256, B), dim3(256), 0, s, f);
+  OMNI_HIP_CHECK(hipGetLastError());
+  return OMNI_OK;
+}
+
 static int launch_chan_attn(const omni_op_t* op, hipStream_t s) {
   ChanArgs a{};
   a.qkv = op->p[0]; a.o = op->p[4]; a.ws = (float*)op->p[5];
@@ -2680,6 +2736,8 @@
   OMNI_REQUIRE(!fold || (op->dtype == OMNI_F32 && a.chunk_tokens % 8 == 0 && a.C % 64 == 0 && op->p[1] && op->p[2] && op->p[3] && op->p[6] && op->p[7]),
                "chan_attn: fold mode needs an f32 plan, C %% 64 == 0, chunk_tokens %% 8 == 0 and p1 / p2 / p3 / p6 / p7");
   OMNI_REQUIRE(!a.osplit || op->dtype == OMNI_F32, "chan_attn: split output needs an f32 plan");
+  const int vfold = op->i[11];
+  OMNI_REQUIRE(vfold == 0 || (vfold == 1 && fold && a.C % 128 == 0), "chan_attn: i11 = %d needs fold mode (i8 = 1) and C %% 128 == 0, and is 0 or 1", vfold);
   const bool have_scores = op->i[9] == 1;
   if (op->i[10] != 0) {
     OMNI_REQUIRE(op->i[10] > 0 && op->i[10] % 8 == 0 && a.chunk_tokens % op->i[10] == 0 && op->dtype == OMNI_F32 && a.C % 4 == 0,
@@ -2700,7 +2758,12 @@
       f.ws = a.ws; f.wp = (const float*)op->p[1]; f.wf = (float*)op->p[2]; f.wb = (unsigned char*)op->p[3]; f.osc = (float*)op->p[6];
       f.bmax = (float*)op->p[7];
       f.C = a.C; f.G = a.G; f.chunks = a.chunks; f.nblk = (a.C / 64) * a.G;
+      f.oscmul = (vfold == 1 && op->f[1] != 0.0f) ? op->f[1] : 1.0f;
       hipLaunchKernelGGL(chan_fold_kernel, dim3(a.C / 64, a.G, a.B), dim3(256), 0, s, f);
+      if (vfold == 1) {
+        f.bv = f.wp + (long long)a.C * a.C; f.bp = f.bv + a.C; f.bias = f.wf + (long long)a.B * a.C * a.C;
+        hipLaunchKernelGGL(chan_fold_bias_kernel, dim3(a.C / 64, a.B), dim3(256), 0, s, f);
+      }
       hipLaunchKernelGGL(chan_fold_pack_kernel, dim3((a.C * (a.C / 16) + 255) / 256, a.B), dim3(256), 0, s, f);
       OMNI_HIP_CHECK(hipGetLastError());
       return OMNI_OK;
diff --git a/omniparser_amd/csrc/gemm_dma.hip b/omniparser_amd/csrc/gemm_dma.hip
--- a/omniparser_amd/csrc/gemm_dma.hip
+++ b/omniparser_amd/csrc/gemm_dma.hip
@@ -16,6 +16,7 @@
   int mtiles, ntiles, xcd_order, xcd_n;
   float oscale;
   int img_tiles; unsigned w_img_stride; const float* img_oscale;
+  int bias_img_stride;
 };
 
 constexpr int GEMM_EPI_SCORES = 3;
@@ -37,7 +38,8 @@
 #endif
 
 template <int BM, int BN, int WM, int WN, int TM, int TN, int LDS_BYTES, int ACT, bool OSPLIT, bool RES>
-__device__ __forceinline__ void gemm_epilogue(f32x16 (&acc)[TM][TN], const GemmArgs& a, unsigned char* lds, int m0, int n0, int wave, int lane, float osc) {
+__device__ __forceinline__ void gemm_epilogue(f32x16 (&acc)[TM][TN], const GemmArgs& a, const float* bias, unsigned char* lds, int m0, int n0, int wave,
+                                              int lane, float osc) {
   constexpr int NW = WM * WN;
   const int wm = wave / WN, wn = wave % WN;
   const int hsel = lane >> 5;
@@ -63,7 +65,7 @@
     for (int j = 0; j < 2; ++j)
 #pragma unroll
       for (int q = 0; q < 4; ++q)
-        bq[j][q] = a.bias ? *reinterpret_cast<const f32x4*>(a.bias + nw0 + 4 * hsel + j * 32 + q * 8) : f32x4{0.f, 0.f, 0.f, 0.f};
+        bq[j][q] = bias ? *reinterpret_cast<const f32x4*>(bias + nw0 + 4 * hsel + j * 32 + q * 8) : f32x4{0.f, 0.f, 0.f, 0.f};
     f32x4 rres[8];
     auto load_res = [&](int i) {
 #pragma unroll
@@ -391,7 +393,8 @@
   if constexpr (ACT == GEMM_EPI_SCORES)
     gemm_scores_epilogue<BM, BN, WM, WN, TM, TN, NSTAGE * STAGE>(acc, a, lds, img, __builtin_amdgcn_readfirstlane(mt) - img * a.img_tiles, n0, wave, lane, osc);
   else
-    gemm_epilogue<BM, BN, WM, WN, TM, TN, NSTAGE * STAGE, ACT, OSPLIT, RES>(acc, a, lds, m0, n0, wave, lane, osc);
+    gemm_epilogue<BM, BN, WM, WN, TM, TN, NSTAGE * STAGE, ACT, OSPLIT, RES>(acc, a, a.bias + (long long)img * a.bias_img_stride, lds, m0, n0, wave,
+                                                                            lane, osc);
 #endif
 }
 
@@ -549,7 +552,7 @@
       }
   }
   omni_report_range(amax);
-  gemm_epilogue<NW * 32, C, NW, 1, 1, OB, 2 * STAGE, OMNI_ACT_NONE, false, true>(acc2, a.ep, lds, m0, 0, wave, lane, a.ep.oscale);
+  gemm_epilogue<NW * 32, C, NW, 1, 1, OB, 2 * STAGE, OMNI_ACT_NONE, false, true>(acc2, a.ep, a.ep.bias, lds, m0, 0, wave, lane, a.ep.oscale);
 #endif
 }
 
@@ -632,6 +635,12 @@
     a.w_img_stride = (unsigned)op->i[27];
     a.img_oscale = (const float*)op->p[6];
   }
+  OMNI_REQUIRE(op->i[29] == 0 || op->i[29] == 1, "gemm_dma: unknown bias mode %d (i29)", op->i[29]);
+  if (op->i[29] == 1) {
+    OMNI_REQUIRE(rows_per_img > 0 && op->i[28] == 0, "gemm_dma: a per-image bias (i29) needs per-image mode (i26 > 0) and no scores epilogue");
+    OMNI_REQUIRE(a.bias && (uintptr_t)a.bias % 16 == 0, "gemm_dma: the per-image bias table (p2) must be a 16-byte aligned pointer");
+    a.bias_img_stride = a.N;
+  }
   if (scores) {
     OMNI_REQUIRE(a.y, "gemm_dma: the scores epilogue needs its workspace (p7)");
     OMNI_REQUIRE(rows_per_img > 0 && rows_per_img % 256 == 0, "gemm_dma: the scores epilogue needs whole 256-row chunks per image (i26 = %d)", rows_per_img);
@@ -643,6 +652,7 @@
     const long long mt256 = (a.M + 255) / 256;
     if (mt256 * (a.N / (tile == 0 ? 256 : 128)) < 256) tile = (tile == 0 && mt256 * (a.N / 128) >= 256) ? 1 : 2;
   }
+  if (rows_per_img > 0 && rows_per_img % 256 != 0) tile = 2;
   if (const char* e = getenv("OMNI_GEMM_TILE")) {
     if (!strcmp(e, "256x128")) tile = 1;
     else if (!strcmp(e, "128x128")) tile = 2;
@@ -659,6 +669,8 @@
 }
 
 int omni_launch_split_convert(const omni_op_t* op, hipStream_t s) {
+  OMNI_REQUIRE(op->i[6] == 0 || op->i[6] == 1, "split_convert: unknown mode %d (i6)", op->i[6]);
+  if (op->i[6] == 1) return omni_launch_chan_repack(op, s);
   const long long rows = (long long)op->i[0] * (op->i[1] > 0 ? op->i[1] : 1);
   const int C = op->i[3], ldi = op->i[4], in_coff = op->i[5], ldo = op->i[13], out_coff = op->i[14];
   OMNI_REQUIRE(op->dtype == OMNI_F32 && op->p[0] && op->p[4], "split_convert: f32 plans, non-null pointers");
diff --git a/omniparser_amd/csrc/omni_internal.h b/omniparser_amd/csrc/omni_internal.h
--- a/omniparser_amd/csrc/omni_internal.h
+++ b/omniparser_amd/csrc/omni_internal.h
@@ -167,6 +167,7 @@
 int omni_launch_conv(const omni_op_t* op, hipStream_t s);
 int omni_launch_gemm_dma(const omni_op_t* op, hipStream_t s);
 int omni_launch_split_convert(const omni_op_t* op, hipStream_t s);
+int omni_launch_chan_repack(const omni_op_t* op, hipStream_t s);
 int omni_launch_mlp_fused(const omni_op_t* op, hipStream_t s);
 int omni_launch_avgpool2(const omni_op_t* op, hipStream_t s);
 int omni_launch_maxpool(const omni_op_t* op, hipStream_t s);
diff --git a/omniparser_amd/florence.py b/omniparser_amd/florence.py
--- a/omniparser_amd/florence.py
+++ b/omniparser_amd/florence.py
@@ -1039,9 +1039,11 @@
             chunks = (N + (partial_tokens or chunk_tokens) - 1) // (partial_tokens or chunk_tokens)
             cws = pb.raw((B * w.groups[s] * chunks * 1024,), torch.float32, zero=False)
             scores_in_gemm = fold and bool(cap.chan_scores_in_gemm)
-            fold_wf = fold_wb = fold_sc = fold_mx = None
+            fold_v = fold and bool(cap.fold_chan_v) and N >= 4 * C
+            fold_wf = fold_wb = fold_sc = fold_mx = fold_bias = None
             if fold:
-                fold_wf = pb.raw((B * C * C,), torch.float32, zero=False)
+                fold_wf = pb.raw((B * C * C + (B * C if fold_v else 0),), torch.float32, zero=False)
+                fold_bias = fold_wf[B * C * C:] if fold_v else None
                 fold_wb = pb.raw((B * C * C,), torch.float32, zero=False)
                 fold_sc = pb.raw((B,), torch.float32, zero=False)
                 fold_mx = pb.raw((B * (C // 64) * w.groups[s],), torch.float32, zero=False)
@@ -1076,17 +1078,30 @@
                             pb.conv_scores(tokens(hbuf), wqs, bqs, cws, N)
                         else:
                             pb.conv(tokens(hbuf), wqk, bqk, tokens(qkv.slice(0, 2 * C)), 1)
-                        vs = tokens(qkv.slice(2 * C, C))
-                        pb.conv(tokens(hbuf), wv, bv, vs, 1, out_split=True)
                         pkey = pre + "channel_attn.proj"
-                        wplain, bproj = W.f32(pkey + ".weight"), W.f32(pkey + ".bias")
-                        pb.keep += [wplain, bproj]
-                        pb.add_op(L.make_op(L.OP_CHAN_ATTN, dt,
-                                            p=[qkv.ptr, wplain.data_ptr(), fold_wf.data_ptr(), fold_wb.data_ptr(), None, cws.data_ptr(),
-                                               fold_sc.data_ptr(), fold_mx.data_ptr()],
-                                            i={0: B, 1: N, 3: C, 4: w.groups[s], 5: chunk_tokens, 6: 1 if (attn_split and grp["dma"]) else 0, 8: 1,
-                                               9: 1 if scores_in_gemm else 0, 10: partial_tokens}))
-                        pb.conv_per_image(vs, fold_wb, fold_sc, bproj, tokens(B_), tokens(B_), N)
+                        chan_p = [qkv.ptr, None, fold_wf.data_ptr(), fold_wb.data_ptr(), None, cws.data_ptr(), fold_sc.data_ptr(), fold_mx.data_ptr()]
+                        chan_i = {0: B, 1: N, 3: C, 4: w.groups[s], 5: chunk_tokens, 6: 1 if (attn_split and grp["dma"]) else 0, 8: 1,
+                                  9: 1 if scores_in_gemm else 0, 10: partial_tokens}
+                        if fold_v:
+                            wvt, wpb = W.cached((key, dt, "dma-vT|wp|bv|bp"), lambda: (
+                                pb.pack_weight_dma(sd[key + ".weight"][2 * C:].float().t().contiguous()),
+                                pb.upload(torch.cat([sd[pkey + ".weight"].float().reshape(-1), sd[key + ".bias"][2 * C:].float(),
+                                                     sd[pkey + ".bias"].float()]))))
+                            pb.keep += [wvt, wpb]
+                            chan_p[1] = wpb.data_ptr()
+                            pb.add_op(L.make_op(L.OP_CHAN_ATTN, dt, p=chan_p, i={**chan_i, 11: 1}, f={1: wvt.omni_oscale}))
+                            pb.fold_gemm(fold_wb, fold_sc, wvt, fold_wf, B, C)
+                            pb.repack_per_image(fold_wf, fold_wb, fold_sc, fold_mx, B, C)
+                            pb.conv_per_image(tokens(hbuf), fold_wb, fold_sc, fold_bias, tokens(B_), tokens(B_), N, bias_per_image=True)
+                            pb.flops += 2 * B * N * C * C
+                        else:
+                            vs = tokens(qkv.slice(2 * C, C))
+                            pb.conv(tokens(hbuf), wv, bv, vs, 1, out_split=True)
+                            wplain, bproj = W.f32(pkey + ".weight"), W.f32(pkey + ".bias")
+                            pb.keep += [wplain, bproj]
+                            chan_p[1] = wplain.data_ptr()
+                            pb.add_op(L.make_op(L.OP_CHAN_ATTN, dt, p=chan_p, i=chan_i))
+                            pb.conv_per_image(vs, fold_wb, fold_sc, bproj, tokens(B_), tokens(B_), N)
                     else:
                         linear(pre + "channel_attn.qkv", hbuf, qkv)
                         pb.add_op(L.make_op(L.OP_CHAN_ATTN, dt, p=[qkv.ptr, None, None, None, att.ptr, cws.data_ptr()],
@@ -1250,6 +1265,7 @@
     fuse_dwln = True
     attn_split_out = True
     fold_chan_proj = True
+    fold_chan_v = True
     chan_scores_in_gemm = True
     fuse_mlp = True
     exact_rows = os.environ.get("OMNI_EXACT_ROWS", "1") != "0"
diff --git a/omniparser_amd/opwork.py b/omniparser_amd/opwork.py
--- a/omniparser_amd/opwork.py
+++ b/omniparser_amd/opwork.py
@@ -18,10 +18,16 @@
         if i[20] == 2 and i[28] == 1:
             return 2 * M * N * K + 2 * M * N * 16, esz * (M * K + N * K + (M // 256) * (N // 64) * 1024)
         nw = M // i[26] if (i[20] == 2 and i[26] > 0) else 1
+        if i[20] == 2 and i[26] > 0 and i[27] == 0:
+            return 0, esz * (M * K + N * K + M * N)
+        if i[20] == 2 and i[29] == 1:
+            return 4 * M * N * K, esz * (i[0] * i[1] * i[2] * i[3] + nw * N * K + nw * N + M * N * (2 if op.p[3] else 1))
         return 2 * M * N * K, esz * (i[0] * i[1] * i[2] * i[3] + nw * N * K + M * N * (2 if op.p[3] else 1))
     if k == 24:
         rows, C, hid = i[0] * max(i[1], 1), i[3], i[12]
         return 4 * rows * C * hid, esz * (3 * rows * C + 2 * C * hid)
+    if k == 19 and i[6] == 1:
+        return 0, esz * 2 * i[0] * i[3] * i[3]
     if k in (2, 3, 4):
         return 0, esz * (i[0] * i[1] * i[2] * i[3] + i[0] * max(i[10], 1) * max(i[11], 1) * i[3])
     if k in (8, 18):
@@ -93,9 +99,13 @@
     if op.kind == 1:
         if op.i[20] == 2 and op.i[28] == 1:
             return "gemm_dma (scores epilogue)"
+        if op.i[20] == 2 and op.i[26] > 0 and op.i[27] == 0:
+            return "gemm_dma (fold W' . Wv)"
         if op.i[20] == 2 and op.i[26] > 0:
-            return "gemm_dma (per-image weights)"
+            return "gemm_dma (per-image weights + bias)" if op.i[29] == 1 else "gemm_dma (per-image weights)"
         return "gemm_dma" if op.i[20] == 2 else ("conv_split" if op.i[20] else "conv_igemm")
+    if op.kind == 19 and op.i[6] == 1:
+        return "split_convert (re-pack W'')"
     if op.kind == 11 and op.i[8] == 1:
         return "chan_attn (fold)" if op.i[9] == 1 else "chan_attn (scores + fold)"
     if op.kind == 28:
diff --git a/omniparser_amd/planner.py b/omniparser_amd/planner.py
--- a/omniparser_amd/planner.py
+++ b/omniparser_amd/planner.py
@@ -287,14 +287,17 @@
         return t
 
     def conv_per_image(self, x: View, w_img: torch.Tensor, scales: torch.Tensor, bias: Optional[torch.Tensor], out: View,
-                       res: Optional[View], rows_per_img: int):
+                       res: Optional[View], rows_per_img: int, bias_per_image: bool = False):
         cout, K = out.C, x.C
         M = x.B * x.H * x.W
         assert self.dtype == L.F32 and x.fmt == "split" and x.ld % 16 == 0 and x.coff % 16 == 0 and cout % 128 == 0 and K % 32 == 0
         assert (out.B, out.H, out.W) == (x.B, x.H, x.W) and M % rows_per_img == 0
         nimg = M // rows_per_img
         assert w_img.numel() * w_img.element_size() >= nimg * cout * K * 4 and scales.dtype == torch.float32 and scales.numel() >= nimg
-        assert bias is None or (bias.dtype == torch.float32 and bias.numel() == cout and bias.device.type == self.device.type)
+        if bias_per_image:
+            assert bias is not None and bias.dtype == torch.float32 and bias.numel() >= nimg * cout and bias.device.type == self.device.type
+        else:
+            assert bias is None or (bias.dtype == torch.float32 and bias.numel() == cout and bias.device.type == self.device.type)
         if res is not None:
             assert (res.B, res.H, res.W, res.C) == (out.B, out.H, out.W, out.C) and res.fmt == "f32"
         self.ops.append(L.make_op(
@@ -303,12 +306,31 @@
                None, scales.data_ptr()],
             i={0: x.B, 1: x.H, 2: x.W, 3: K, 4: x.ld, 5: x.coff, 6: 1, 7: 1, 8: 1, 9: 0, 10: x.H, 11: x.W, 12: cout, 13: out.ld, 14: out.coff,
                15: L.ACT_NONE, 16: res.ld if res is not None else 0, 17: res.coff if res is not None else 0, 20: 2,
-               26: rows_per_img, 27: cout * K * 4}))
+               26: rows_per_img, 27: cout * K * 4, **({29: 1} if bias_per_image else {})}))
         self.keep += [w_img, scales] + ([bias] if bias is not None else [])
         out.fmt = "f32"
         self.flops += 2 * M * cout * K
         self.bytes += 4 * (M * K + nimg * cout * K + M * cout * (2 if res is not None else 1))
         return out
+
+    def fold_gemm(self, w_img: torch.Tensor, scales: torch.Tensor, wvt: torch.Tensor, out: torch.Tensor, nimg: int, C: int):
+        assert self.dtype == L.F32 and C % 128 == 0 and getattr(wvt, "omni_fmt", 0) == 2 and wvt.numel() == 2 * C * C
+        assert w_img.numel() * w_img.element_size() >= nimg * C * C * 4 and out.numel() >= nimg * C * C and out.dtype == torch.float32
+        assert scales.dtype == torch.float32 and scales.numel() >= nimg
+        self.ops.append(L.make_op(
+            L.OP_CONV, self.dtype,
+            p=[w_img.data_ptr(), wvt.data_ptr(), None, None, out.data_ptr(), None, scales.data_ptr()],
+            i={0: nimg, 1: C, 2: 1, 3: C, 4: C, 5: 0, 6: 1, 7: 1, 8: 1, 9: 0, 10: C, 11: 1, 12: C, 13: C, 14: 0, 15: L.ACT_NONE, 20: 2,
+               26: C, 27: 0}))
+        self.keep += [w_img, scales, wvt, out]
+
+    def repack_per_image(self, wf: torch.Tensor, w_img: torch.Tensor, scales: torch.Tensor, maxima: torch.Tensor, nimg: int, C: int):
+        assert self.dtype == L.F32 and C % 64 == 0 and wf.numel() >= nimg * C * C and w_img.numel() * w_img.element_size() >= nimg * C * C * 4
+        assert scales.numel() >= nimg and maxima.numel() >= nimg * (C // 64) * (C // 32)
+        self.ops.append(L.make_op(L.OP_SPLIT_CONVERT, self.dtype,
+                                  p=[wf.data_ptr(), None, None, None, w_img.data_ptr(), maxima.data_ptr(), scales.data_ptr()],
+                                  i={0: nimg, 1: C, 3: C, 4: C, 5: 0, 6: 1, 13: C, 14: 0}))
+        self.keep += [wf, w_img, scales, maxima]
 
     @staticmethod
     def qk_group_rows(C: int):
```

Result: faster. 13.55, median of 6 (+1.5%).
